# bhansconnect/burn-ppo

Measured on AMD Instinct MI355X. Metric: env-steps/sec (rollout+GAE+PPO update) at 1/2/4/8 MI355X; steps-to-475-return CartPole, higher is better.
Workload: dtype f32

## Files before the change

burn-ppo_amd/bppo/_lib.py:

```python
import ctypes as C
import os

import numpy as np

HERE = os.path.dirname(os.path.abspath(__file__))
LIB_PATH = os.environ.get("BPPO_LIB_PATH") or os.path.join(HERE, "libbppo.so")

OK, ERR_ARG, ERR_NONFINITE, ERR_EMPTY_MASK, ERR_HIP, ERR_COMM, ERR_UNSUPPORTED = range(7)
ENV_CARTPOLE, ENV_CONNECT_FOUR, ENV_LIARS_DICE = 0, 1, 2
ENV_SKULL = 3
ENV_KINDS = {"cartpole": ENV_CARTPOLE, "connect_four": ENV_CONNECT_FOUR, "liars_dice": ENV_LIARS_DICE,
             "skull": ENV_SKULL}
MAX_PLAYERS = 6


class BppoError(RuntimeError):
    def __init__(self, status, msg):
        super().__init__(f"bppo status {status}: {msg}")
        self.status = status


class Config(C.Structure):
    _fields_ = [("env_kind", C.c_int32), ("num_envs", C.c_int32), ("num_steps", C.c_int32),
                ("hidden_size", C.c_int32), ("num_hidden", C.c_int32), ("relu", C.c_int32),
                ("ctde", C.c_int32), ("critic_hidden_size", C.c_int32), ("critic_num_hidden", C.c_int32),
                ("num_epochs", C.c_int32), ("num_minibatches", C.c_int32),
                ("normalize_obs", C.c_int32), ("normalize_returns", C.c_int32), ("clip_value", C.c_int32),
                ("gamma", C.c_double), ("gae_lambda", C.c_double), ("clip_epsilon", C.c_double),
                ("value_coef", C.c_double), ("max_grad_norm", C.c_double), ("adam_epsilon", C.c_double),
                ("target_kl", C.c_double), ("return_clip", C.c_double),
                ("reward_shaping_coef", C.c_double), ("seed", C.c_uint64), ("env_seed_base", C.c_uint64),
                ("rng_stream", C.c_uint64),
                ("cnn", C.c_int32), ("num_conv_layers", C.c_int32), ("conv_channels", C.c_int32 * 4),
                ("kernel_size", C.c_int32), ("cnn_fc_hidden_size", C.c_int32), ("cnn_num_fc_layers", C.c_int32),
                ("normalize_values", C.c_int32), ("player_count", C.c_int32), ("split_networks", C.c_int32),
                ("shuffle_windows", C.c_int32)]


class Episode(C.Structure):
    _fields_ = [("total_reward", C.c_float * MAX_PLAYERS), ("length", C.c_int32), ("env_index", C.c_int32),
                ("step", C.c_int32), ("pad", C.c_int32)]


class RolloutInfo(C.Structure):
    _fields_ = [("episodes", C.c_int32), ("mean_return", C.c_float), ("mean_length", C.c_float),
                ("pad", C.c_int32), ("rng_word_pos", C.c_uint64)]


METRIC_NAMES = ("policy_loss", "value_loss", "entropy", "entropy_scaled", "approx_kl", "clip_fraction",
                "explained_variance", "total_loss", "value_mean", "returns_mean", "adv_mean_raw",
                "adv_std_raw", "adv_min_raw", "adv_max_raw", "value_error_mean", "value_error_std",
                "value_error_max", "avg_valid_actions", "entropy_valid_pct")


POPART_METRICS = ("value_norm_target_mean", "value_norm_target_std", "value_norm_rescale_mag")


class UpdateMetrics(C.Structure):
    _fields_ = [(n, C.c_float) for n in METRIC_NAMES] + [("num_updates", C.c_int32),
                                                          ("epochs_run", C.c_int32)] + \
        [(n, C.c_float) for n in POPART_METRICS]


ALLREDUCE_FN = C.CFUNCTYPE(C.c_int, C.c_void_p, C.c_size_t, C.c_void_p)

EXPORTS = (
    "bppo_create", "bppo_destroy", "bppo_last_error", "bppo_version", "bppo_num_params",
    "bppo_params_set", "bppo_params_get", "bppo_forward", "bppo_rng_get", "bppo_rng_set",
    "bppo_vecenv_reset", "bppo_vecenv_observe", "bppo_vecenv_step", "bppo_vecenv_set_step", "bppo_set_reward_shaping_schedule",
    "bppo_obs_norm_get", "bppo_obs_norm_set", "bppo_ret_norm_get", "bppo_ret_norm_set",
    "bppo_collect_rollouts", "bppo_rollout_episodes", "bppo_compute_gae", "bppo_ppo_update", "bppo_train_step", "bppo_train_steps",
    "bppo_set_allreduce", "bppo_set_allreduce_async", "bppo_get_stream", "bppo_opponents_set", "bppo_opponents_get_envs", "bppo_buffer_get", "bppo_buffer_set", "bppo_gae_device", "bppo_gae_rows_device",
    "bppo_gae_mp_device", "bppo_last_kernel_ms", "bppo_debug_libm", "bppo_debug_shuffle_chain", "bppo_debug_chain_walk2", "bppo_minibatch_rows",
    "bppo_debug_fisher_yates", "bppo_debug_gemm", "bppo_debug_shuffle_engine", "bppo_debug_sample",
    "bppo_rng_fill_bytes", "bppo_rng_from_seed", "bppo_rng_key_get", "bppo_num_param_tensors",
    "bppo_optimizer_get", "bppo_optimizer_set", "bppo_popart_get", "bppo_popart_set",
    "bppo_config_size", "bppo_update_metrics_size", "bppo_episode_size", "bppo_rollout_info_size",
    "bppo_set_explained_variance_mode", "bppo_set_minibatch_kernel", "bppo_set_rank",
    "bppo_debug_record_params",
)

STRUCT_SIZES = {"bppo_config_size": Config, "bppo_update_metrics_size": UpdateMetrics,
                "bppo_episode_size": Episode, "bppo_rollout_info_size": RolloutInfo}

_lib = None


def lib():
    global _lib
    if _lib is not None:
        return _lib
    try:
        import torch
    except ImportError:
        pass
    if not os.path.exists(LIB_PATH):
        raise RuntimeError(f"{LIB_PATH} is missing; build it with `make -C burn-ppo_amd` "
                           f"(or __graft_entry__.build())")
    L = C.CDLL(LIB_PATH)
    vp, u64, sz, i32 = C.c_void_p, C.c_uint64, C.c_size_t, C.c_int32
    fp = C.POINTER(C.c_float)
    dp = C.POINTER(C.c_double)
    sig = {
        "bppo_create": (i32, [C.POINTER(Config), C.c_int, vp, C.POINTER(vp)]),
        "bppo_destroy": (None, [vp]),
        "bppo_last_error": (C.c_char_p, [vp]),
        "bppo_version": (C.c_char_p, []),
        "bppo_num_params": (sz, [vp]),
        "bppo_params_set": (i32, [vp, vp, sz]),
        "bppo_params_get": (i32, [vp, vp, sz]),
        "bppo_forward": (i32, [vp, vp, vp, i32, vp, vp]),
        "bppo_rng_get": (i32, [vp, C.POINTER(u64)]),
        "bppo_rng_set": (i32, [vp, u64]),
        "bppo_vecenv_reset": (i32, [vp]),
        "bppo_vecenv_observe": (i32, [vp, vp, vp, vp, vp]),
        "bppo_vecenv_step": (i32, [vp, vp, vp, vp, vp, vp, i32, C.POINTER(i32)]),
        "bppo_vecenv_set_step": (i32, [vp, u64]),
        "bppo_set_reward_shaping_schedule": (i32, [vp, vp, vp, i32]),
        "bppo_obs_norm_get": (i32, [vp, vp, vp, dp]),
        "bppo_obs_norm_set": (i32, [vp, vp, vp, C.c_double]),
        "bppo_ret_norm_get": (i32, [vp, vp, vp]),
        "bppo_ret_norm_set": (i32, [vp, vp, vp]),
        "bppo_collect_rollouts": (i32, [vp, C.POINTER(RolloutInfo)]),
        "bppo_rollout_episodes": (i32, [vp, vp, i32, C.POINTER(i32)]),
        "bppo_compute_gae": (i32, [vp]),
        "bppo_ppo_update": (i32, [vp, C.c_double, C.c_double, C.POINTER(UpdateMetrics)]),
        "bppo_train_step": (i32, [vp, C.c_double, C.c_double, C.POINTER(RolloutInfo), C.POINTER(UpdateMetrics)]),
        "bppo_train_steps": (i32, [vp, i32, vp, vp, C.c_uint64, vp, vp, vp, i32, vp]),
        "bppo_set_allreduce": (i32, [vp, ALLREDUCE_FN, vp, i32]),
        "bppo_set_allreduce_async": (i32, [vp, ALLREDUCE_FN, vp, i32]),
        "bppo_set_rank": (i32, [vp, i32]),
        "bppo_get_stream": (i32, [vp, C.POINTER(vp)]),
        "bppo_opponents_set": (i32, [vp, i32, vp, vp, vp, vp, i32, vp, vp, vp]),
        "bppo_opponents_get_envs": (i32, [vp, vp, vp]),
        "bppo_buffer_get": (i32, [vp, C.c_char_p, vp, sz]),
        "bppo_buffer_set": (i32, [vp, C.c_char_p, vp, sz]),
        "bppo_gae_device": (i32, [vp, vp, vp, vp, i32, i32, C.c_float, C.c_float, vp, vp, vp]),
        "bppo_gae_rows_device": (i32, [vp, vp, vp, vp, i32, i32, C.c_float, C.c_float, vp, vp, vp, vp]),
        "bppo_gae_mp_device": (i32, [vp, vp, vp, vp, vp, i32, i32, i32, C.c_float, C.c_float, vp, vp,
                                     vp]),
        "bppo_last_kernel_ms": (i32, [vp, C.c_char_p, fp]),
        "bppo_debug_libm": (i32, [i32, i32, vp, vp, sz]),
        "bppo_debug_shuffle_chain": (i32, [u64, u64, u64, C.c_uint32, vp, C.POINTER(u64)]),
        "bppo_minibatch_rows": (i32, [vp, vp, i32, C.POINTER(i32)]),
        "bppo_debug_chain_walk2": (i32, [u64, u64, u64, u64, C.c_uint32, C.c_uint32, C.POINTER(u64), C.POINTER(u64)]),
        "bppo_debug_fisher_yates": (i32, [i32, vp, C.c_uint32, vp]),
        "bppo_debug_gemm": (i32, [i32, i32, i32, i32, vp, vp, vp, i32, vp, vp]),
        "bppo_debug_shuffle_engine": (i32, [u64, u64, u64, C.c_uint32, i32, u64, i32, i32, vp, vp, vp]),
        "bppo_debug_sample": (i32, [i32, i32, vp, vp, u64, u64, u64, vp, vp]),
        "bppo_rng_fill_bytes": (i32, [vp, vp, sz]),
        "bppo_rng_from_seed": (i32, [vp, vp]),
        "bppo_rng_key_get": (i32, [vp, vp]),
        "bppo_num_param_tensors": (sz, [vp]),
        "bppo_optimizer_get": (i32, [vp, vp, vp, vp, sz]),
        "bppo_optimizer_set": (i32, [vp, vp, vp, vp, sz]),
        "bppo_popart_get": (i32, [vp, vp]),
        "bppo_popart_set": (i32, [vp, vp]),
        "bppo_set_explained_variance_mode": (i32, [vp, i32]),
        "bppo_set_minibatch_kernel": (i32, [vp, i32]),
        "bppo_debug_record_params": (i32, [vp, vp, i32]),
    }
    for name in STRUCT_SIZES:
        sig[name] = (sz, [])
    for name, (res, args) in sig.items():
        f = getattr(L, name)
        f.restype = res
        f.argtypes = args
    for name, struct in STRUCT_SIZES.items():
        if getattr(L, name)() != C.sizeof(struct):
            raise RuntimeError(f"{LIB_PATH}: {name}() = {getattr(L, name)()} but ctypes {struct.__name__} is "
                               f"{C.sizeof(struct)} bytes (binding out of date with include/bppo.h)")
    _lib = L
    return L


def check(status, ctx=None):
    if status != OK:
        msg = lib().bppo_last_error(ctx).decode() if ctx else ""
        raise BppoError(status, msg)


def ptr(a):
    if a is None:
        return None
    if isinstance(a, np.ndarray):
        assert a.flags["C_CONTIGUOUS"]
        return a.ctypes.data
    return a.data_ptr()
```

burn-ppo_amd/csrc/bppo_api.hip:

```cpp
#include <algorithm>
#include <pthread.h>
#include <chrono>
#include <cmath>
#include <cstdio>
#include <cstdlib>
#include <cstring>
#include <new>
#include <thread>
#include <sys/prctl.h>
#include <x86intrin.h>
#include "bppo_internal.h"
#include "shuffle_host.h"
#include "bppo_wide.h"

using namespace bppo;

namespace bppo {
static double tsc_per_ms() {
    static double v = 0.0;
    if (v == 0.0) {
        const auto t0 = std::chrono::steady_clock::now();
        const uint64_t c0 = __rdtsc();
        std::this_thread::sleep_for(std::chrono::milliseconds(20));
        const uint64_t c1 = __rdtsc();
// ... 4 lines not shown


NetLayout make_layout(const bppo_config &c, int obs_dim, int priv_dim, int act_dim) {
    NetLayout L;
    const bool split = c.split_networks && !c.ctde;
    L.ctde = c.ctde || split; L.relu = c.relu;
    auto add = [&](int in, int out) {
        int i = L.n_layers++;
        L.in[i] = in; L.out[i] = out;
        return i;
    };
    int in = obs_dim;
    if (c.cnn) {
        L.H = 6; L.W = 7; L.C = 2;
        L.E = obs_dim - L.H * L.W * L.C;
        L.ksize = c.kernel_size;
        int cin = L.C;
        for (int l = 0; l < c.num_conv_layers; l++) {
            const int co = c.conv_channels[l < 4 ? l : 3];
            L.conv_cin[l] = cin;
            add(cin * L.ksize * L.ksize, co);
            cin = co;
        }
        L.n_conv = c.num_conv_layers;
        L.fdim = L.H * L.W * cin + L.E;
        in = L.fdim;
        for (int l = 0; l < c.cnn_num_fc_layers; l++) { add(in, c.cnn_fc_hidden_size); in = c.cnn_fc_hidden_size; }
        L.n_actor_hidden = L.n_conv + c.cnn_num_fc_layers;
    } else {
        for (int l = 0; l < c.num_hidden; l++) { add(in, c.hidden_size); in = c.hidden_size; }
        L.n_actor_hidden = c.num_hidden;
    }
    L.policy = add(in, act_dim);
    if (L.ctde && c.cnn) {
        L.critic_first = L.n_layers;
        for (int l = 0; l < L.n_conv; l++) add(L.in[l], L.out[l]);
        L.critic_fc0 = L.n_layers;
        int cin = L.fdim;
        for (int l = 0; l < c.cnn_num_fc_layers; l++) { add(cin, c.cnn_fc_hidden_size); cin = c.cnn_fc_hidden_size; }
        L.value = add(cin, 1);
    } else if (L.ctde) {
        int cin = split ? obs_dim : priv_dim + obs_dim;
        const int nc = split ? c.num_hidden : c.critic_num_hidden, wc = split ? c.hidden_size : c.critic_hidden_size;
        L.critic_first = L.critic_fc0 = L.n_layers;
        for (int l = 0; l < nc; l++) { add(cin, wc); cin = wc; }
        L.value = add(cin, 1);
    } else {
        L.value = add(in, 1);
    }
    int order[16], no = 0;
    for (int l = 0; l < L.n_layers; l++)
        if (!split || l < L.n_actor_hidden || (l >= L.critic_first && l < L.value)) order[no++] = l;
    if (split) { order[no++] = L.policy; order[no++] = L.value; }
    size_t off = 0;
    for (int r = 0; r < L.n_layers; r++) {
        const int l = order[r];
        L.rec[l] = r;
        L.w[l] = off; off += (size_t)L.in[l] * L.out[l];
        L.b[l] = off; off += L.out[l];
    }
    L.n_params = off;
    return L;
}

__global__ void k_libm(int which, const float *x, float *y, size_t n) {
    size_t i = blockIdx.x * (size_t)blockDim.x + threadIdx.x;
    if (i >= n) return;
    float v = x[i];
    switch (which) {
    case 0: y[i] = bppo_math::logf_glibc(v); break;
    case 1: y[i] = bppo_math::sinf_glibc(v); break;
    case 2: y[i] = bppo_math::cosf_glibc(v); break;
    case 3: y[i] = -bppo_math::logf_glibc(-bppo_math::logf_glibc(v)); break;
    case 5: y[i] = bppo_math::tanhf_glibc_bf(v); break;
    default: y[i] = bppo_math::expf_glibc(v); break;
    }
}

bppo_status launch_libm(int which, const float *d_x, float *d_y, size_t n) {
    hipLaunchKernelGGL(k_libm, dim3((unsigned)((n + 255) / 256)), dim3(256), 0, 0, which, d_x, d_y, n);
    return hipGetLastError() == hipSuccess ? BPPO_OK : BPPO_ERR_HIP;
}

}

static float powi_f32(float a, int b) {
    int recip = b < 0;
    float r = 1.0f;
    for (;;) {
        if (b & 1) r *= a;
        b /= 2;
        if (b == 0) break;
        a *= a;
    }
    return recip ? 1.0f / r : r;
}

template <class T>
static bppo_status dalloc(bppo_ctx *c, T **p, size_t n) {
    *p = nullptr;
    if (n == 0) return BPPO_OK;
    BPPO_HIP(c, hipMalloc((void **)p, n * sizeof(T)));
    BPPO_HIP(c, hipMemsetAsync(*p, 0, n * sizeof(T), c->stream));
    return BPPO_OK;
}

extern "C" size_t bppo_config_size(void) { return sizeof(bppo_config); }
extern "C" size_t bppo_update_metrics_size(void) { return sizeof(bppo_update_metrics); }
extern "C" size_t bppo_episode_size(void) { return sizeof(bppo_episode); }
extern "C" size_t bppo_rollout_info_size(void) { return sizeof(bppo_rollout_info); }

extern "C" const char *bppo_version(void) { return "bppo-mi355x 0.1 (gfx950)"; }

extern "C" const char *bppo_last_error(const bppo_ctx *c) { return c ? c->err.c_str() : "null ctx"; }

static hipError_t wait_event(bppo_ctx *c, hipEvent_t ev) {
    const auto t0 = std::chrono::steady_clock::now();
    hipError_t e = event_query(ev);
    if (e == hipErrorNotReady) {
        if (c->wait_est_us > 200.0)
            std::this_thread::sleep_for(std::chrono::microseconds((long)(0.7 * c->wait_est_us)));
        while ((e = event_query(ev)) == hipErrorNotReady) std::this_thread::sleep_for(std::chrono::microseconds(20));
    }
    const double ms = std::chrono::duration<double, std::milli>(std::chrono::steady_clock::now() - t0).count();
    c->wait_est_us = c->wait_est_us > 0.0 ? 0.5 * c->wait_est_us + 500.0 * ms : 1000.0 * ms;
    c->sync_wait_ms += ms;
    return e;
}

static hipError_t sync_stream(bppo_ctx *c) {
    const auto t0 = std::chrono::steady_clock::now();
    hipError_t e;
    if (!c->ev_block) e = hipStreamSynchronize(c->stream);
    else {
        static thread_local bool slack = false;
        if (!slack) { (void)prctl(PR_SET_TIMERSLACK, 1000UL, 0, 0, 0); slack = true; }
        e = hipEventRecord(c->ev_block, c->stream);
        while (e == hipSuccess && (e = event_query(c->ev_block)) == hipErrorNotReady) {
            std::this_thread::sleep_for(std::chrono::microseconds(20));
            e = hipSuccess;
        }
    }
    c->sync_wait_ms += std::chrono::duration<double, std::milli>(std::chrono::steady_clock::now() - t0).count();
    return e;
}

static bool cartpole_fused_net(const bppo_config &c) {
    return !c.split_networks && !c.cnn && !c.ctde && (c.hidden_size == 16 || c.hidden_size == 32 || c.hidden_size == 64) &&
           (c.num_hidden == 1 || c.num_hidden == 2);
}

static bppo_status ctx_init(bppo_ctx *c, const bppo_config *cfg, int dev, void *stream) {
    c->cfg = *cfg;
    c->dev = dev;
    if (cfg->num_envs <= 0 || cfg->num_steps <= 0 || cfg->num_epochs <= 0 || cfg->num_minibatches <= 0) {
        c->err = "num_envs, num_steps, num_epochs, num_minibatches must be positive";
        return BPPO_ERR_ARG;
    }
    c->N = cfg->num_envs; c->T = cfg->num_steps;
    switch (cfg->env_kind) {
    case BPPO_ENV_CARTPOLE: c->D = 5; c->A = 2; c->P = 1; c->G = 0; break;
    case BPPO_ENV_CONNECT_FOUR: c->D = 86; c->A = 7; c->P = 2; c->G = 0; break;
    case BPPO_ENV_LIARS_DICE: c->D = 270; c->A = 49; c->P = 4; c->G = cfg->ctde ? 120 : 0; break;
    case BPPO_ENV_SKULL: c->D = 135; c->A = 33; c->P = 6; c->G = cfg->ctde ? 200 : 0; break;
    default: c->err = "unknown env_kind"; return BPPO_ERR_ARG;
    }
    c->Pa = c->P;
    if (cfg->env_kind == BPPO_ENV_SKULL) {
        c->Pa = cfg->player_count ? cfg->player_count : 4;
        if (c->Pa < 2 || c->Pa > 6) { c->err = "Skull supports 2-6 players"; return BPPO_ERR_ARG; }
    }
    c->wide = cfg->env_kind != BPPO_ENV_CARTPOLE || !cartpole_fused_net(*cfg);
    if (c->wide && !cfg->ctde) c->G = 0;
    if (!cfg->cnn && (cfg->hidden_size < 1 || cfg->num_hidden < 1 ||
                      (cfg->ctde && (cfg->critic_hidden_size < 1 || cfg->critic_num_hidden < 1)))) {
        c->err = "hidden_size / num_hidden (critic_*) must be positive";
        return BPPO_ERR_ARG;
    }
    if (!(cfg->reward_shaping_coef >= 0.0)) { c->err = "reward_shaping_coef must be >= 0"; return BPPO_ERR_ARG; }
    if (cfg->cnn) {
        if (cfg->env_kind != BPPO_ENV_CONNECT_FOUR || cfg->ctde) { c->err = "CNN requires OBSERVATION_SHAPE (Connect Four)"; return BPPO_ERR_ARG; }
        if (cfg->num_conv_layers < 1 || cfg->num_conv_layers > 4 || cfg->kernel_size < 1 || cfg->kernel_size > 7 ||
            !(cfg->kernel_size & 1) || cfg->cnn_num_fc_layers < 1 || cfg->cnn_fc_hidden_size < 1) {
            c->err = "CNN: 1-4 conv layers, odd kernel_size <= 7 (same padding), >= 1 FC layer";
            return BPPO_ERR_UNSUPPORTED;
        }
        for (int l = 0; l < cfg->num_conv_layers; l++)
            if (cfg->conv_channels[l < 4 ? l : 3] < 1) { c->err = "conv_channels must be positive"; return BPPO_ERR_ARG; }
    }
    {
        const int split = cfg->split_networks && !cfg->ctde ? 2 : 1;
        const int layers = cfg->cnn ? split * (cfg->num_conv_layers + cfg->cnn_num_fc_layers) + 2
                         : cfg->ctde ? cfg->num_hidden + cfg->critic_num_hidden + 2
                                     : split * cfg->num_hidden + 2;
        if (layers > NetLayout::MAX_LAYERS) {
            c->err = "network: at most 16 layers in all (hidden / conv / FC layers + heads)";
            return BPPO_ERR_UNSUPPORTED;
        }
    }
    BPPO_HIP(c, hipSetDevice(dev));
    if (stream) { c->stream = (hipStream_t)stream; c->own_stream = false; }
    else {
        int lo = 0, hi = 0;
        BPPO_HIP(c, hipDeviceGetStreamPriorityRange(&lo, &hi));
        BPPO_HIP(c, hipStreamCreateWithPriority(&c->stream, hipStreamNonBlocking, hi));
        c->own_stream = true;
    }
    c->net = make_layout(*cfg, c->D, c->G, c->A);
    const size_t np = c->net.n_params;
    const size_t TN = (size_t)c->T * c->N;
    c->adam_t.assign(2 * c->net.n_layers, 0);
    TRY(dalloc(c, &c->d_params, np));
    TRY(dalloc(c, &c->d_m1, np));
    TRY(dalloc(c, &c->d_m2, np));
    TRY(dalloc(c, &c->d_grad, np + 64));
    c->slab_rows = 256 * 8;
    c->relu_mfma = cfg->relu ? 1 : 0;
    if (!c->wide) TRY(dalloc(c, &c->d_slab, c->slab_rows * (np + 64)));
    TRY(dalloc(c, &c->d_cp, (size_t)4 * c->N));
    TRY(dalloc(c, &c->d_steps, (size_t)c->N));
    TRY(dalloc(c, &c->d_env_pos, (size_t)c->N));
    TRY(dalloc(c, &c->d_ep_ret, (size_t)c->N * c->P));
    TRY(dalloc(c, &c->d_ep_len, (size_t)c->N));
    if (!c->wide) TRY(dalloc(c, &c->d_obs, TN * c->D));
    TRY(dalloc(c, &c->d_rew, TN));
    TRY(dalloc(c, &c->d_rew_raw, TN));
    TRY(dalloc(c, &c->d_done, TN));
    TRY(dalloc(c, &c->d_val, TN));
    TRY(dalloc(c, &c->d_logp, TN));
    TRY(dalloc(c, &c->d_adv, TN));
    TRY(dalloc(c, &c->d_ret, TN));
    TRY(dalloc(c, &c->d_act, TN));
    if (!c->wide || cfg->normalize_returns) TRY(dalloc(c, &c->d_X, TN));
    if (!c->wide && cfg->hidden_size == 64 && cfg->num_hidden == 2 && cfg->relu)
    {
        TRY(dalloc(c, &c->d_gumbel, TN * 2));
        TRY(dalloc(c, &c->d_rpool, (size_t)RPOOL_K * c->N));
        TRY(dalloc(c, &c->d_rpos, (size_t)RPOOL_K * c->N));
    }
    TRY(dalloc(c, &c->d_on, (size_t)2 * c->D + 1));
    if (!c->wide) TRY(dalloc(c, &c->d_obs_part, (size_t)c->N * 2 * c->D));
    if (!c->wide) {
        TRY(dalloc(c, &c->d_act_in, (size_t)c->N));
        TRY(dalloc(c, &c->d_scr_r, (size_t)c->N));
        TRY(dalloc(c, &c->d_bxc, (size_t)c->N * c->D));
        BPPO_HIP(c, hipMalloc((void **)&c->d_scr_d, (size_t)c->N));
    }
    TRY(dalloc(c, &c->d_rn_returns, (size_t)c->N * c->P));
    TRY(dalloc(c, &c->d_rn_stats, 4));
    TRY(dalloc(c, &c->d_scan_agg, (TN + 4095) / 4096 + 1));
    TRY(dalloc(c, &c->d_last_v, (size_t)c->N));
    c->eps_cap = (int)std::min<size_t>((size_t)c->T * c->N + 4096, (size_t)INT32_MAX / 2);
    TRY(dalloc(c, &c->d_eps, (size_t)c->eps_cap));
    TRY(dalloc(c, &c->d_ep_count, 1));
    TRY(dalloc(c, &c->d_ep_sum, ROLL_HOST_WORDS));
    TRY(dalloc(c, &c->d_err, 1));
    TRY(dalloc(c, &c->d_perm_base, TN));
    c->d_perm = c->d_perm_base;
    TRY(dalloc(c, &c->d_perm_ep, TN * (size_t)cfg->num_epochs));
    TRY(dalloc(c, &c->d_inv_ep, TN * (size_t)cfg->num_epochs));
    TRY(dalloc(c, &c->d_advpart, (size_t)ADV_STREAM_BLOCKS * ADV_STREAM_MAXM * 4));
    {
        c->fy_shared = getenv("BPPO_FY_ON_COPY") && atoi(getenv("BPPO_FY_ON_COPY")) == 1;
        if (!c->fy_shared) BPPO_HIP(c, make_side_stream(dev, &c->fy_stream));
        for (int e = 0; e < cfg->num_epochs && e < SHUF_MAX_EPOCHS; e++)
            BPPO_HIP(c, hipEventCreateWithFlags(&c->fy_ev[e], hipEventDisableTiming));
        if (getenv("BPPO_PREP_SIDE") && atoi(getenv("BPPO_PREP_SIDE")) == 1) {
            BPPO_HIP(c, make_side_stream(dev, &c->prep_stream));
            BPPO_HIP(c, hipEventCreateWithFlags(&c->ev_prep, hipEventDisableTiming));
        }
        BPPO_HIP(c, hipEventCreateWithFlags(&c->ev_env, hipEventDisableTiming));
    }
    TRY(dalloc(c, &c->d_fy, 4 * TN));
    TRY(dalloc(c, &c->d_scan, TN / 8192 + 2));
    BPPO_HIP(c, fy_ranges_init(c->fyr, (uint32_t)TN));
    TRY(dalloc(c, &c->d_red, 4 * 1024 + 64));
    TRY(dalloc(c, &c->d_mb_stats, (size_t)4 * std::max(cfg->num_minibatches, 2)));
    c->d_mb_cur = c->d_mb_stats;
    TRY(dalloc(c, &c->d_rows, (size_t)cfg->num_epochs * cfg->num_minibatches * (WM_COUNT + 4)));
    BPPO_HIP(c, hipHostMalloc((void **)&c->h_rows,
                              sizeof(float) * (size_t)cfg->num_epochs * cfg->num_minibatches * (WM_COUNT + 4),
                              hipHostMallocDefault));
    if (!c->wide && cfg->hidden_size == 64 && cfg->num_hidden == 2 && cfg->relu && c->D == 5)
    {
        BPPO_HIP(c, hipMalloc((void **)&c->d_rowA, sizeof(float4) * 2 * TN));
        BPPO_HIP(c, hipMalloc((void **)&c->d_rowB, sizeof(float2) * TN));
    }
    BPPO_HIP(c, hipHostMalloc((void **)&c->h_red, sizeof(double) * (4 * 1024 + 64 + 2 * ROLL_HOST_WORDS),
                              hipHostMallocDefault));
    BPPO_HIP(c, hipHostGetDevicePointer((void **)&c->hd_red, c->h_red, 0));
    BPPO_HIP(c, hipEventCreateWithFlags(&c->ev_upd, hipEventDisableTiming));
    BPPO_HIP(c, hipEventRecord(c->ev_upd, c->stream));
    BPPO_HIP(c, hipEventCreateWithFlags(&c->ev_block, hipEventDisableTiming | hipEventBlockingSync));
    for (int i = 0; i < TM_SLOTS; i++) {
        BPPO_HIP(c, hipEventCreate(&c->ev[i][0]));
        BPPO_HIP(c, hipEventCreate(&c->ev[i][1]));
    }
    for (int i = 0; i < bppo_ctx::MB_EV; i++) {
        BPPO_HIP(c, hipEventCreate(&c->mb_ev[i][0]));
        BPPO_HIP(c, hipEventCreate(&c->mb_ev[i][1]));
    }
    c->rng_key = seed_key(cfg->seed);
    c->rng_pos = 0;
    c->shuf.gate = c->ev_upd;
    TRY(c->shuf.init(dev, c->rng_key, cfg->rng_stream, (uint32_t)TN, cfg->num_epochs, TN * (uint64_t)c->A, c->err,
                     cfg->shuffle_windows != 0));
    if (c->fy_shared) c->fy_stream = c->shuf.copy;
    c->on_mean.assign(c->D, 0.0); c->on_m2.assign(c->D, 0.0); c->on_count = 0;
    c->u_ret = c->d_ret; c->u_val = c->d_val;
    c->shaping_v.assign(1, cfg->reward_shaping_coef); c->shaping_s.assign(1, 0);
    if (cfg->normalize_values) TRY(popart_alloc(c));
    if (c->wide) {
        TRY(wide_init(c));
        TRY(wide_reset(c));
        TRY(wide_pack(c));
    } else {
        TRY(launch_cartpole_reset(c));
    }
    BPPO_HIP(c, sync_stream(c));
    return BPPO_OK;
}

extern "C" bppo_status bppo_create(const bppo_config *cfg, int hip_device, void *hip_stream,
                                   bppo_ctx **out) {
    if (!cfg || !out) return BPPO_ERR_ARG;
    bppo_ctx *c = new bppo_ctx();
    bppo_status s = ctx_init(c, cfg, hip_device, hip_stream);
    *out = c;
    return s;
}

extern "C" void bppo_destroy(bppo_ctx *c) {
    if (!c) return;
    if (c->ev_thread.joinable()) c->ev_thread.join();
    if (c->ev_stream) { (void)hipStreamSynchronize(c->ev_stream); (void)hipStreamDestroy(c->ev_stream); }
    if (c->ev_gae) (void)hipEventDestroy(c->ev_gae);
    if (c->ev_copied) (void)hipEventDestroy(c->ev_copied);
    for (float *h : {c->h_ev_v, c->h_ev_r, c->h_ev_valid}) if (h) (void)hipHostFree(h);
    if (c->fy_stream) (void)hipStreamSynchronize(c->fy_stream);
    if (c->prep_stream) (void)hipStreamSynchronize(c->prep_stream);
    c->shuf.shutdown();
    if (c->stream) (void)hipStreamSynchronize(c->stream);
    wide_free(c);
    popart_free(c);
    void *ptrs[] = {c->d_params, c->d_m1, c->d_m2, c->d_grad, c->d_slab, c->d_cp, c->d_steps,
                    c->d_env_pos, c->d_ep_ret, c->d_ep_len, c->d_obs, c->d_rew, c->d_rew_raw,
                    c->d_done, c->d_val, c->d_logp, c->d_adv, c->d_ret, c->d_act, c->d_X, c->d_on,
                    c->d_obs_part, c->d_rn_returns, c->d_rn_stats, c->d_scan_agg, c->d_last_v,
                    c->d_eps, c->d_ep_count, c->d_ep_sum, c->d_err, c->d_perm_base, c->d_perm_ep, c->d_inv_ep, c->d_advpart, c->d_fy, c->d_scan,
                    c->d_red, c->d_mb_stats, c->d_gumbel, c->d_rpool, c->d_rpos, c->d_rows, c->d_rowA, c->d_rowB};
    for (void *p : ptrs) if (p) (void)hipFree(p);
    fy_ranges_free(c->fyr);
    if (c->h_red) (void)hipHostFree(c->h_red);
    if (c->h_rows) (void)hipHostFree(c->h_rows);
    if (c->ev_block) (void)hipEventDestroy(c->ev_block);
    if (c->ev_upd) (void)hipEventDestroy(c->ev_upd);
    for (int i = 0; i < TM_SLOTS; i++) {
        if (c->ev[i][0]) (void)hipEventDestroy(c->ev[i][0]);
        if (c->ev[i][1]) (void)hipEventDestroy(c->ev[i][1]);
    }
    for (auto &pr : c->mb_ev)
        for (hipEvent_t e : pr) if (e) (void)hipEventDestroy(e);
    if (c->fy_stream && !c->fy_shared) { (void)hipStreamSynchronize(c->fy_stream); (void)hipStreamDestroy(c->fy_stream); }
    for (hipEvent_t e : c->fy_ev) if (e) (void)hipEventDestroy(e);
    if (c->prep_stream) (void)hipStreamDestroy(c->prep_stream);
    for (hipEvent_t e : {c->ev_env, c->ev_prep}) if (e) (void)hipEventDestroy(e);
    if (c->own_stream && c->stream) (void)hipStreamDestroy(c->stream);
    delete c;
}

extern "C" size_t bppo_num_params(const bppo_ctx *c) { return c ? c->net.n_params : 0; }

static void drop_prefetch(bppo_ctx *c) {
    if (!c->prefetched) return;
    c->prefetched = false;
    c->collected = 0;
    c->gae_done = 0;
}

extern "C" bppo_status bppo_params_set(bppo_ctx *c, const float *h, size_t n) {
    if (!c || !h || n != c->net.n_params) { if (c) c->err = "params_set: size mismatch"; return BPPO_ERR_ARG; }
    drop_prefetch(c);
    BPPO_HIP(c, hipMemcpyAsync(c->d_params, h, n * 4, hipMemcpyHostToDevice, c->stream));
    if (c->wide) TRY(wide_pack(c));
    BPPO_HIP(c, sync_stream(c));
    return BPPO_OK;
}

extern "C" bppo_status bppo_params_get(bppo_ctx *c, float *h, size_t n) {
    if (!c || !h || n != c->net.n_params) { if (c) c->err = "params_get: size mismatch"; return BPPO_ERR_ARG; }
    BPPO_HIP(c, hipMemcpyAsync(h, c->d_params, n * 4, hipMemcpyDeviceToHost, c->stream));
    BPPO_HIP(c, sync_stream(c));
    return BPPO_OK;
}

extern "C" bppo_status bppo_forward(bppo_ctx *c, const float *obs, const float *priv, int32_t B,
                                    float *logits, float *values) {
    if (!c || !obs || B <= 0) return BPPO_ERR_ARG;
    if (c->wide) return wide_forward_host(c, obs, priv, B, logits, values);
    struct Scratch { float *p[3] = {nullptr, nullptr, nullptr}; ~Scratch() { for (float *q : p) (void)hipFree(q); } } t;
    BPPO_HIP(c, hipMalloc((void **)&t.p[0], sizeof(float) * (size_t)B * c->D));
    BPPO_HIP(c, hipMalloc((void **)&t.p[1], sizeof(float) * (size_t)B * c->A));
    BPPO_HIP(c, hipMalloc((void **)&t.p[2], sizeof(float) * (size_t)B));
    float *d_o = t.p[0], *d_l = t.p[1], *d_v = t.p[2];
    BPPO_HIP(c, hipMemcpyAsync(d_o, obs, sizeof(float) * (size_t)B * c->D, hipMemcpyHostToDevice, c->stream));
    bppo_status s = launch_forward_rows(c, d_o, B, d_l, d_v);
    if (s == BPPO_OK) {
        if (logits) BPPO_HIP(c, hipMemcpyAsync(logits, d_l, sizeof(float) * (size_t)B * c->A, hipMemcpyDeviceToHost, c->stream));
        if (values) BPPO_HIP(c, hipMemcpyAsync(values, d_v, sizeof(float) * (size_t)B, hipMemcpyDeviceToHost, c->stream));
    }
    const bppo_status ss = sync_stream(c) == hipSuccess ? BPPO_OK : BPPO_ERR_HIP;
    return s != BPPO_OK ? s : ss;
}

extern "C" bppo_status bppo_rng_get(bppo_ctx *c, uint64_t *p) {
    if (!c || !p) return BPPO_ERR_ARG;
    *p = c->rng_pos;
    return BPPO_OK;
}
extern "C" bppo_status bppo_rng_set(bppo_ctx *c, uint64_t p) {
    if (!c) return BPPO_ERR_ARG;
    drop_prefetch(c);
    c->shuf_slot = -1;
    c->fy_slot = -1; c->fy_done = 0;
    c->rng_pos = p;
    return BPPO_OK;
}

extern "C" bppo_status bppo_rng_fill_bytes(bppo_ctx *c, uint8_t *dst, size_t n) {
    if (!c || (!dst && n)) return BPPO_ERR_ARG;
    const size_t nw = (n + 3) / 4;
    uint32_t blk[16];
    uint64_t cached = ~0ull;
    for (size_t i = 0; i < nw; i++) {
        const uint64_t pos = c->rng_pos + i;
        if ((pos >> 4) != cached) { chacha12_block(c->rng_key, pos >> 4, c->cfg.rng_stream, blk); cached = pos >> 4; }
        const uint32_t w = blk[pos & 15];
        for (int b = 0; b < 4 && 4 * i + b < n; b++) dst[4 * i + b] = (uint8_t)(w >> (8 * b));
    }
    c->rng_pos += nw;
    c->shuf_slot = -1;
    c->fy_slot = -1; c->fy_done = 0;
    return BPPO_OK;
}

extern "C" bppo_status bppo_rng_from_seed(bppo_ctx *c, const uint8_t *seed) {
    if (!c || !seed) return BPPO_ERR_ARG;
    drop_prefetch(c);
    Key8 k;
    for (int i = 0; i < 8; i++)
        k.k[i] = (uint32_t)seed[4 * i] | ((uint32_t)seed[4 * i + 1] << 8) | ((uint32_t)seed[4 * i + 2] << 16) |
                 ((uint32_t)seed[4 * i + 3] << 24);
    BPPO_HIP(c, sync_stream(c));
    BPPO_HIP(c, hipStreamSynchronize(c->fy_stream));
    c->fy_slot = -1; c->fy_done = 0;
    c->shuf.shutdown();
    c->shuf.~ShuffleEngine();
    new (&c->shuf) ShuffleEngine();
    c->rng_key = k;
    c->rng_pos = 0;
    c->shuf_slot = -1;
    const size_t TN = (size_t)c->T * c->N;
    c->shuf.gate = c->ev_upd;
    TRY(c->shuf.init(c->dev, c->rng_key, c->cfg.rng_stream, (uint32_t)TN, c->cfg.num_epochs, TN * (uint64_t)c->A, c->err,
                     c->cfg.shuffle_windows != 0));
    if (c->fy_shared) c->fy_stream = c->shuf.copy;
    return BPPO_OK;
}

extern "C" bppo_status bppo_rng_key_get(bppo_ctx *c, uint32_t *key) {
    if (!c || !key) return BPPO_ERR_ARG;
    for (int i = 0; i < 8; i++) key[i] = c->rng_key.k[i];
    return BPPO_OK;
}

extern "C" bppo_status bppo_optimizer_get(bppo_ctx *c, float *m1, float *m2, int32_t *steps, size_t n) {
    if (!c || n != c->net.n_params) { if (c) c->err = "optimizer_get: size mismatch"; return BPPO_ERR_ARG; }
    if (m1) BPPO_HIP(c, hipMemcpyAsync(m1, c->d_m1, n * 4, hipMemcpyDeviceToHost, c->stream));
    if (m2) BPPO_HIP(c, hipMemcpyAsync(m2, c->d_m2, n * 4, hipMemcpyDeviceToHost, c->stream));
    BPPO_HIP(c, sync_stream(c));
    if (steps)
        for (int l = 0; l < c->net.n_layers; l++)
            for (int k = 0; k < 2; k++) steps[2 * c->net.rec[l] + k] = c->adam_t[2 * l + k];
    return BPPO_OK;
}

extern "C" bppo_status bppo_optimizer_set(bppo_ctx *c, const float *m1, const float *m2, const int32_t *steps,
                                          size_t n) {
    if (!c || !m1 || !m2 || !steps || n != c->net.n_params) {
        if (c) c->err = "optimizer_set: size mismatch";
        return BPPO_ERR_ARG;
    }
    BPPO_HIP(c, hipMemcpyAsync(c->d_m1, m1, n * 4, hipMemcpyHostToDevice, c->stream));
    BPPO_HIP(c, hipMemcpyAsync(c->d_m2, m2, n * 4, hipMemcpyHostToDevice, c->stream));
    BPPO_HIP(c, sync_stream(c));
    for (int l = 0; l < c->net.n_layers; l++)
        for (int k = 0; k < 2; k++) c->adam_t[2 * l + k] = steps[2 * c->net.rec[l] + k];
    return BPPO_OK;
}

extern "C" size_t bppo_num_param_tensors(const bppo_ctx *c) { return c ? c->adam_t.size() : 0; }

extern "C" bppo_status bppo_vecenv_reset(bppo_ctx *c) {
    if (!c) return BPPO_ERR_ARG;
    drop_prefetch(c);
    TRY(c->wide ? wide_reset(c) : launch_cartpole_reset(c));
    BPPO_HIP(c, sync_stream(c));
    return BPPO_OK;
}

extern "C" bppo_status bppo_vecenv_observe(bppo_ctx *c, float *obs, int32_t *players, uint8_t *masks,
                                           float *priv) {
    (void)priv; (void)masks;
    if (!c) return BPPO_ERR_ARG;
    if (c->wide) return wide_observe_host(c, obs, players, masks, priv);
    if (obs) {
        TRY(launch_cartpole_observe(c, c->d_bxc));
        BPPO_HIP(c, hipMemcpyAsync(obs, c->d_bxc, sizeof(float) * (size_t)c->N * c->D, hipMemcpyDeviceToHost, c->stream));
        BPPO_HIP(c, sync_stream(c));
    }
    if (players) std::fill(players, players + c->N, 0);
    return BPPO_OK;
}

extern "C" bppo_status bppo_vecenv_step(bppo_ctx *c, const int32_t *actions, float *obs, float *rewards,
                                        uint8_t *dones, bppo_episode *eps, int32_t cap, int32_t *n_eps) {
    if (!c || !actions) return BPPO_ERR_ARG;
    const int N = c->N;
    if (c->wide) {
        BPPO_HIP(c, hipMemsetAsync(c->d_ep_count, 0, 4, c->stream));
        int32_t cnt = 0;
        TRY(wide_step_host(c, actions, obs, rewards, dones, &cnt));
        if (n_eps) *n_eps = cnt;
        if (eps && cap > 0 && cnt > 0) {
            std::vector<EpisodeRec> recs(std::min(cnt, c->eps_cap));
            BPPO_HIP(c, hipMemcpy(recs.data(), c->d_eps, sizeof(EpisodeRec) * recs.size(), hipMemcpyDeviceToHost));
            std::sort(recs.begin(), recs.end(), [](const EpisodeRec &a, const EpisodeRec &b) {
                return a.env_index < b.env_index; });
            for (int i = 0; i < (int)recs.size() && i < cap; i++) {
                std::memcpy(eps[i].total_reward, recs[i].total_reward, sizeof(float) * BPPO_MAX_PLAYERS);
                eps[i].length = recs[i].length; eps[i].env_index = recs[i].env_index;
                eps[i].step = recs[i].step; eps[i].pad = 0;
            }
        }
        return BPPO_OK;
    }
    int32_t *d_a = c->d_act_in; float *d_r = c->d_scr_r, *d_o = c->d_bxc; uint8_t *d_d = c->d_scr_d;
    BPPO_HIP(c, hipMemcpyAsync(d_a, actions, sizeof(int32_t) * N, hipMemcpyHostToDevice, c->stream));
    BPPO_HIP(c, hipMemsetAsync(c->d_ep_count, 0, 4, c->stream));
    TRY(launch_cartpole_vecenv_step(c, d_a, d_r, d_d, d_o));
    if (rewards) BPPO_HIP(c, hipMemcpyAsync(rewards, d_r, sizeof(float) * N, hipMemcpyDeviceToHost, c->stream));
    if (dones) BPPO_HIP(c, hipMemcpyAsync(dones, d_d, N, hipMemcpyDeviceToHost, c->stream));
    if (obs) BPPO_HIP(c, hipMemcpyAsync(obs, d_o, sizeof(float) * (size_t)N * c->D, hipMemcpyDeviceToHost, c->stream));
    int32_t cnt = 0;
    BPPO_HIP(c, hipMemcpyAsync(&cnt, c->d_ep_count, 4, hipMemcpyDeviceToHost, c->stream));
    BPPO_HIP(c, sync_stream(c));
    if (n_eps) *n_eps = cnt;
    if (eps && cap > 0 && cnt > 0) {
        std::vector<EpisodeRec> recs(std::min(cnt, c->eps_cap));
        BPPO_HIP(c, hipMemcpy(recs.data(), c->d_eps, sizeof(EpisodeRec) * recs.size(), hipMemcpyDeviceToHost));
        std::sort(recs.begin(), recs.end(), [](const EpisodeRec &a, const EpisodeRec &b) {
            return a.env_index < b.env_index; });
        for (int i = 0; i < (int)recs.size() && i < cap; i++) {
            std::memcpy(eps[i].total_reward, recs[i].total_reward, sizeof(float) * BPPO_MAX_PLAYERS);
            eps[i].length = recs[i].length; eps[i].env_index = recs[i].env_index;
            eps[i].step = recs[i].step; eps[i].pad = 0;
        }
    }
    return BPPO_OK;
}

extern "C" bppo_status bppo_vecenv_set_step(bppo_ctx *c, uint64_t s) {
    if (!c) return BPPO_ERR_ARG;
    c->env_step = s;
    return BPPO_OK;
}

extern "C" bppo_status bppo_set_reward_shaping_schedule(bppo_ctx *c, const double *values, const uint64_t *steps,
                                                        int32_t n) {
    if (!c || n < 0 || (n > 0 && (!values || !steps))) return BPPO_ERR_ARG;
    std::vector<double> v(values, values + n);
    std::vector<uint64_t> s(steps, steps + n);
    if (bppo::schedule_get(v, s, 0) < 0.0) { c->err = "reward_shaping_coef must be >= 0"; return BPPO_ERR_ARG; }
    c->shaping_v = std::move(v); c->shaping_s = std::move(s);
    return BPPO_OK;
}

extern "C" bppo_status bppo_obs_norm_get(bppo_ctx *c, double *mean, double *m2, double *count) {
    if (!c) return BPPO_ERR_ARG;
    std::vector<double> h(2 * c->D + 1);
    BPPO_HIP(c, hipMemcpyAsync(h.data(), c->d_on, sizeof(double) * h.size(), hipMemcpyDeviceToHost, c->stream));
    BPPO_HIP(c, sync_stream(c));
    if (mean) std::memcpy(mean, h.data(), sizeof(double) * c->D);
    if (m2) std::memcpy(m2, h.data() + c->D, sizeof(double) * c->D);
    if (count) *count = h[2 * c->D];
    return BPPO_OK;
}

extern "C" bppo_status bppo_obs_norm_set(bppo_ctx *c, const double *mean, const double *m2, double count) {
    if (!c || !mean || !m2) return BPPO_ERR_ARG;
    drop_prefetch(c);
    std::vector<double> h(2 * c->D + 1);
    std::memcpy(h.data(), mean, sizeof(double) * c->D);
    std::memcpy(h.data() + c->D, m2, sizeof(double) * c->D);
    h[2 * c->D] = count;
    BPPO_HIP(c, hipMemcpyAsync(c->d_on, h.data(), sizeof(double) * h.size(), hipMemcpyHostToDevice, c->stream));
    BPPO_HIP(c, sync_stream(c));
    return BPPO_OK;
}

extern "C" bppo_status bppo_ret_norm_get(bppo_ctx *c, double *mvc, double *returns) {
    if (!c) return BPPO_ERR_ARG;
    if (mvc) BPPO_HIP(c, hipMemcpyAsync(mvc, c->d_rn_stats, sizeof(double) * 3, hipMemcpyDeviceToHost, c->stream));
    if (returns) BPPO_HIP(c, hipMemcpyAsync(returns, c->d_rn_returns, sizeof(double) * (size_t)c->N * c->P, hipMemcpyDeviceToHost, c->stream));
    BPPO_HIP(c, sync_stream(c));
    return BPPO_OK;
}

extern "C" bppo_status bppo_ret_norm_set(bppo_ctx *c, const double *mvc, const double *returns) {
    if (!c) return BPPO_ERR_ARG;
    drop_prefetch(c);
    if (mvc) BPPO_HIP(c, hipMemcpyAsync(c->d_rn_stats, mvc, sizeof(double) * 3, hipMemcpyHostToDevice, c->stream));
    if (returns) BPPO_HIP(c, hipMemcpyAsync(c->d_rn_returns, returns, sizeof(double) * (size_t)c->N * c->P, hipMemcpyHostToDevice, c->stream));
    BPPO_HIP(c, sync_stream(c));
    return BPPO_OK;
}

extern "C" bppo_status bppo_popart_get(bppo_ctx *c, double *st) {
    if (!c || !st) return BPPO_ERR_ARG;
    st[0] = c->pa_mean; st[1] = c->pa_m2; st[2] = c->pa_count; st[3] = c->pa_eps;
    return BPPO_OK;
}

extern "C" bppo_status bppo_popart_set(bppo_ctx *c, const double *st) {
    if (!c || !st) return BPPO_ERR_ARG;
    drop_prefetch(c);
    c->pa_mean = st[0]; c->pa_m2 = st[1]; c->pa_count = st[2]; c->pa_eps = st[3];
    return BPPO_OK;
}

static bppo_status tm_begin(bppo_ctx *c, int slot) {
    BPPO_HIP(c, hipEventRecord(c->ev[slot][0], c->stream));
    return BPPO_OK;
}
static bppo_status tm_end(bppo_ctx *c, int slot) {
    BPPO_HIP(c, hipEventRecord(c->ev[slot][1], c->stream));
    return BPPO_OK;
}
static void tm_read(bppo_ctx *c, int slot) {
    float ms = 0;
    if (event_ms(c->ev[slot][0], c->ev[slot][1], &ms)) c->last_ms[slot] = ms;
}

static bppo_status fy_enqueue_ready(bppo_ctx *c, int slot) {
    const size_t B = (size_t)c->T * c->N;
    if (slot != c->fy_slot) {
        c->fy_slot = slot; c->fy_done = 0;
        BPPO_HIP(c, hipStreamWaitEvent(c->fy_stream, c->ev_upd, 0));
    }
    if (c->shuf.failed(c->err)) return BPPO_ERR_HIP;
    while (c->fy_done < c->cfg.num_epochs && c->shuf.epoch_ready(slot, c->fy_done)) {
        const int e = c->fy_done;
        if (c->shuf.failed(c->err)) return BPPO_ERR_HIP;
        BPPO_HIP(c, hipStreamWaitEvent(c->fy_stream, c->shuf.ev[slot][e], 0));
        if (e > 0) BPPO_HIP(c, hipStreamWaitEvent(c->fy_stream, c->fy_ev[e - 1], 0));
        BPPO_HIP(c, hipEventRecord(c->ev[TM_SHUFFLE][0], c->fy_stream));
        BPPO_HIP(c, fisher_yates_device(c->shuf.d_J[slot] + (size_t)e * B, (uint32_t)B, c->d_fy, c->d_scan,
                                        c->d_perm_ep + (size_t)e * B, c->fy_stream, &c->fyr,
                                        c->d_inv_ep + (size_t)e * B));
        BPPO_HIP(c, hipEventRecord(c->ev[TM_SHUFFLE][1], c->fy_stream));
        BPPO_HIP(c, hipEventRecord(c->fy_ev[e], c->fy_stream));
        c->fy_done++;
    }
    return BPPO_OK;
}

static double *roll_host(bppo_ctx *c, int slot) { return c->h_red + 4 * 1024 + 64 + (size_t)slot * ROLL_HOST_WORDS; }

static bppo_status collect_enqueue(bppo_ctx *c, bool summary) {
    const size_t TN = (size_t)c->T * c->N;
    c->coll_slot ^= 1;
    const int tro = c->coll_slot ? TM_ROLLOUT_B : TM_ROLLOUT, trn = c->coll_slot ? TM_RETNORM_B : TM_RETNORM;
    if (c->wide) {
        BPPO_HIP(c, hipMemsetAsync(c->d_ep_count, 0, 4, c->stream));
        BPPO_HIP(c, hipMemsetAsync(c->d_err, 0, 4, c->stream));
    }
    const uint64_t base = c->rng_pos;
    TRY(tm_begin(c, tro));
    if (c->wide) TRY(wide_collect(c, base));
    else {
        TRY(launch_cartpole_rollout(c, base, nullptr, nullptr, c->cfg.normalize_obs));
        TRY(popart_denorm(c, c->d_val, TN));
    }
    TRY(tm_end(c, tro));
    if (!opp_active(c)) {
        c->shuf_slot = c->shuf.ensure(base + TN * (uint64_t)c->A);
        TRY(fy_enqueue_ready(c, c->shuf_slot));
    }
    if (opp_active(c)) {
        TRY(opp_rollout_end(c));
    } else {
        c->rng_pos = base + TN * (uint64_t)c->A;
        c->shuf_slot = c->shuf.ensure(c->rng_pos);
    }
    if (c->cfg.normalize_obs) TRY(launch_obs_norm_merge(c));
    TRY(tm_begin(c, trn));
    if (c->cfg.normalize_returns) TRY(launch_return_norm(c));
    else if (!c->wide) BPPO_HIP(c, hipMemcpyAsync(c->d_rew, c->d_rew_raw, TN * 4, hipMemcpyDeviceToDevice, c->stream));
    TRY(tm_end(c, trn));
    int32_t *hv = reinterpret_cast<int32_t *>(roll_host(c, c->coll_slot));
    if (summary) {
        if (zero_copy()) {
            TRY(launch_episode_summary(c, c->hd_red + (roll_host(c, c->coll_slot) - c->h_red)));
        } else {
            TRY(launch_episode_summary(c, c->d_ep_sum));
            BPPO_HIP(c, hipMemcpyAsync(hv, c->d_ep_sum, sizeof(double) * ROLL_HOST_WORDS, hipMemcpyDeviceToHost, c->stream));
        }
    } else {
        BPPO_HIP(c, hipMemcpyAsync(&hv[0], c->d_ep_count, 4, hipMemcpyDeviceToHost, c->stream));
        BPPO_HIP(c, hipMemcpyAsync(&hv[1], c->d_err, 4, hipMemcpyDeviceToHost, c->stream));
    }
    c->collected = 1; c->gae_done = 0;
    c->rollout_rng_pos[c->coll_slot] = c->rng_pos;
    return BPPO_OK;
}

static bppo_status collect_finish(bppo_ctx *c, bppo_rollout_info *info, int slot) {
    float ms = 0;
    const int tro = slot ? TM_ROLLOUT_B : TM_ROLLOUT, trn = slot ? TM_RETNORM_B : TM_RETNORM;
    if (event_ms(c->ev[tro][0], c->ev[tro][1], &ms)) c->last_ms[TM_ROLLOUT] = ms;
    if (event_ms(c->ev[trn][0], c->ev[trn][1], &ms)) c->last_ms[TM_RETNORM] = ms;
    const int32_t *hv = reinterpret_cast<const int32_t *>(roll_host(c, slot));
    const double *part = roll_host(c, slot) + 2;
    if (hv[1] & 2) { c->err = "Empty action mask: an env has no valid action"; return BPPO_ERR_EMPTY_MASK; }
    if (hv[1] & 1) { c->err = "NaN/Inf in log probs — model producing corrupt logits"; return BPPO_ERR_NONFINITE; }
    if (hv[1] & 4) { c->err = "opponent pool: pos_to_opp names a model index outside [0, n_models)"; return BPPO_ERR_ARG; }
    if (hv[1] & 8) { c->err = "Invalid action: outside the env's action mask"; return BPPO_ERR_ARG; }
    if (hv[1]) { c->err = "collect_rollouts: unknown device error flag"; return BPPO_ERR_HIP; }
    if (info) {
        info->episodes = hv[0];
        info->rng_word_pos = c->rollout_rng_pos[slot];
        info->mean_return = 0; info->mean_length = 0;
        const int n = std::min(hv[0], c->eps_cap);
        if (n > 0) {
            double sr = 0, sl = 0;
            for (int b = 0; b < EP_SUMMARY_BLOCKS; b++) { sr += part[2 * b]; sl += part[2 * b + 1]; }
            info->mean_return = (float)(sr / n); info->mean_length = (float)(sl / n);
        }
    }
    return BPPO_OK;
}

extern "C" bppo_status bppo_collect_rollouts(bppo_ctx *c, bppo_rollout_info *info) {
    if (!c) return BPPO_ERR_ARG;
    if (c->prefetched) c->prefetched = false;
    else TRY(collect_enqueue(c, info != nullptr));
    BPPO_HIP(c, sync_stream(c));
    return collect_finish(c, info, c->coll_slot);
}

extern "C" bppo_status bppo_rollout_episodes(bppo_ctx *c, bppo_episode *eps, int32_t cap, int32_t *n) {
    if (!c) return BPPO_ERR_ARG;
    int32_t cnt = 0;
    BPPO_HIP(c, hipMemcpyAsync(&cnt, c->d_ep_count, 4, hipMemcpyDeviceToHost, c->stream));
    BPPO_HIP(c, sync_stream(c));
    int m = std::min(cnt, c->eps_cap);
// ... 727 lines not shown
```

burn-ppo_amd/csrc/bppo_internal.h:

```cpp
#pragma once
#include <hip/hip_runtime.h>
#include <stdint.h>
#include <stddef.h>
#include <string>
#include <vector>
#include <thread>
#include <mutex>
#include <condition_variable>
#include <atomic>
#include <memory>
#include "../../include/bppo.h"
#include "bppo_device.h"

namespace bppo {

struct NetLayout {
    static constexpr int MAX_LAYERS = 16;
    int n_layers = 0;
    int in[MAX_LAYERS], out[MAX_LAYERS];
    size_t w[MAX_LAYERS], b[MAX_LAYERS];
    int n_actor_hidden = 0;
    int policy = 0, value = 0;
    int critic_first = -1;
    int critic_fc0 = -1;
    int ctde = 0, relu = 1;
    int rec[MAX_LAYERS];
    size_t n_params = 0;
    int n_conv = 0, ksize = 3, H = 0, W = 0, C = 0, E = 0, fdim = 0;
    int conv_cin[4] = {0, 0, 0, 0};
    int conv_base(int s) const { return s ? critic_first : 0; }
    bool is_conv(int l) const {
        return n_conv && (l < n_conv || (critic_fc0 > critic_first && l >= critic_first && l < critic_fc0));
    }
};
NetLayout make_layout(const bppo_config &c, int obs_dim, int priv_dim, int act_dim);

constexpr int EP_SUMMARY_BLOCKS = 128;
constexpr int WIDE_SPLIT_MIN_ROWS = 32768;
constexpr int RPOOL_K = 16;
constexpr int TM_SLOTS = 10;
constexpr int ROLL_HOST_WORDS = 2 + 2 * EP_SUMMARY_BLOCKS;
constexpr int ADV_STREAM_BLOCKS = 512, ADV_STREAM_MAXM = 16;
constexpr int GRAD_METRIC_SLOTS = 14, GRAD_VEMAX = 9, GRAD_VEMAX_LOCAL = GRAD_METRIC_SLOTS;

struct EpisodeRec {
    float total_reward[BPPO_MAX_PLAYERS];
    int32_t length, env_index, step, pad;
};

struct Welford { double n, mean, m2; };

constexpr int SHUF_MAX_EPOCHS = 32;
constexpr int SHUF_MAX_SPEC = 64;
constexpr uint64_t SHUF_CK = 1024;
constexpr uint64_t SHUF_CHUNK = (uint64_t)1 << 20;
__host__ __device__ constexpr uint64_t shuffle_window(uint64_t n) { return 2 * n + ((uint64_t)1 << 20); }

struct SpecWalk {
    uint64_t start = 0, end = 0, ck_base = 0;
    int wbuf = 0;
    std::vector<uint32_t> ck;
    std::atomic<int64_t> progress{-1};
    std::atomic<int> done{1};
    std::atomic<bool> stop{false};
    std::atomic<int> merged_to{-1};
    uint64_t merge_q = 0;
    uint64_t gen = 0;
    uint64_t job = 0;
    bool running = false;
};

struct WordBuf {
    uint32_t *d = nullptr, *h = nullptr;
    uint64_t cap = 0;
    struct Region { uint64_t base = 0, len = 0, off = 0; } reg[SHUF_MAX_EPOCHS];
    int nreg = 0;
    std::vector<hipEvent_t> ev;
    std::unique_ptr<std::atomic<int>[]> ok;
    uint32_t *hd = nullptr;
    bool gpu = false;
    uint64_t made_for = ~0ull;
};

struct FyRanges {
    uint32_t *x = nullptr;
    uint32_t *cb = nullptr;
    uint32_t *cursor = nullptr;
    uint2 *P = nullptr;
    uint32_t *flag = nullptr;
    int nb = 0, ncb = 0;
    uint32_t n = 0;
};

struct EpochSplit { uint32_t B, base, rem, M; };
__device__ __forceinline__ uint32_t mb_of(uint32_t i, const EpochSplit &s) {
    const uint32_t big = s.rem * (s.base + 1);
    return i < big ? i / (s.base + 1) : s.rem + (i - big) / s.base;
}
struct ShuffleEngine {
    int dev = 0;
    uint32_t n = 0;
    int epochs = 0;
    Key8 key{};
    uint64_t stream = 0;
    uint64_t gap = 0;
    uint64_t win = 0;
    bool keep_guess = true;
    bool pair = false;
    bool win_producers = false;
    bool win_gpu_words = false;
    hipStream_t d2h = nullptr;
    hipEvent_t words_made = nullptr;
    double Ew = 0.0, sigma = 0.0;
    int K = 0;
    int host_cpus = 16;
    WordBuf wb[2];
    SpecWalk spec[SHUF_MAX_SPEC];
    int nspec = 0, ncur = 0;
    int C = 1;
    int fr_depth = 0;
    int cont0 = 0;
    bool cont_valid[2] = {false, false};
    int cont_src0 = -1, cont_dst0 = -1, cont_wb = 0;
    uint64_t cont_seq = 0;
    std::vector<std::thread> workers;
    std::vector<std::thread> gens;
    std::vector<std::pair<uint64_t, size_t>> gen_order;
    WordBuf *gen_buf = nullptr;
    std::atomic<size_t> gen_next{0};
    uint64_t gen_job = 0;
    int gen_active = 0;
    void generator();
    uint64_t seq = 0;
    bool carry_valid[2] = {false, false};
    std::thread th;
    std::mutex mu;
    std::condition_variable cv;
    bool quit = false;
    bool slot_valid[2] = {false, false};
    uint64_t slot_start[2] = {0, 0};
    int pending = -1, running = -1;
    int consumer = -1;
    int chain_from = -1;
    uint64_t chain_start = 0;
    int last_slot = 1;
    hipEvent_t consumed[2] = {nullptr, nullptr};
    bool consumed_used[2] = {false, false};
    std::atomic<bool> cancel{false};
    int ready[2] = {0, 0};
    uint64_t end_pos[2][SHUF_MAX_EPOCHS];
    struct Seg { uint64_t pos0, pos1; uint32_t r0, pad; };
    int maxseg = 0;
    Seg *seg_host[2] = {nullptr, nullptr};
    Seg *d_seg[2] = {nullptr, nullptr};
    uint32_t *d_J[2] = {nullptr, nullptr};
    hipEvent_t ev[2][SHUF_MAX_EPOCHS] = {};
    bool ev_used[2][SHUF_MAX_EPOCHS] = {};
    hipStream_t copy = nullptr;
    hipEvent_t gate = nullptr;
    double walk_ms[2][SHUF_MAX_EPOCHS] = {};
    int coalesced[2][SHUF_MAX_EPOCHS] = {};
    std::atomic<uint64_t> spec_words{0}, true_words{0};
    std::atomic<uint64_t> tsc_walk{0}, tsc_words{0};
    bppo_status init(int device, const Key8 &key, uint64_t stream, uint32_t n_, int epochs_, uint64_t gap_,
                     std::string &err, bool windows = false);
    bool run_windowed(int slot, uint64_t start);
    void xj_gate_wait(int e);
    uint64_t job_end(int slot) const { return win ? slot_start[slot] + (uint64_t)epochs * win : end_pos[slot][epochs - 1]; }
    std::atomic<bool> hip_bad{false};
    std::mutex hip_mu;
    std::string hip_msg;
    void hip_note(hipError_t e, const char *what);
    bool failed(std::string &msg) const;
    int ensure(uint64_t start);
    hipError_t release(int slot, hipStream_t st);
    void wait_epoch(int slot, int e);
    bool epoch_ready(int slot, int e);
    void shutdown();
    void run();
    void worker(int i);
    void launch_walk(int i, uint64_t start, int wbuf);
    void stop_walks(int lo, int hi);
    const uint32_t *words(int b, uint64_t pos, uint64_t len, std::vector<uint32_t> &scratch, bool true_walk = false);
    int alt_b = -1;
    WordBuf::Region alt_reg;
    struct WalkStats { uint64_t words = 0, tsc_walk = 0, tsc_words = 0; };
    void walk_pair(int i, WalkStats &st);
    uint64_t walk_piece(int b, uint64_t pos, uint32_t *r, std::vector<uint32_t> &scratch, WalkStats &st,
                        bool true_walk = false);
    void flush(WalkStats &st, std::atomic<uint64_t> &words_ctr);
    int peek(int i, uint64_t q, uint32_t *r);
};
uint64_t shuffle_walk_host(const Key8 &key, uint64_t stream, uint64_t pos, uint32_t n, uint32_t *J);
hipError_t make_side_stream(int device, hipStream_t *st);

struct Timers {
    hipEvent_t a = nullptr, b = nullptr;
};

}

struct bppo_ctx {
    bppo_config cfg;
    int dev = 0;
    hipStream_t stream = nullptr;
    bool own_stream = false;
    std::string err;
    int N = 0, T = 0, D = 0, A = 0, P = 1, G = 0;
    int Pa = 1;
    bppo::NetLayout net;
    float *d_params = nullptr, *d_m1 = nullptr, *d_m2 = nullptr;
    std::vector<int32_t> adam_t;
    float *d_grad = nullptr;
    double *d_grad64 = nullptr;
    float *d_slab = nullptr;
    size_t slab_rows = 0;
    int slab_used = 0;
    int relu_mfma = 1;
    int mb_kernel = 0;
    float *dbg_params = nullptr;
    int dbg_params_max = 0;
    float *d_cp = nullptr;
    int32_t *d_steps = nullptr;
    uint64_t *d_env_pos = nullptr;
    float *d_ep_ret = nullptr;
    int32_t *d_ep_len = nullptr;
    uint64_t env_step = 0;
    std::vector<double> shaping_v;
    std::vector<uint64_t> shaping_s;
    float *d_obs = nullptr, *d_rew = nullptr, *d_rew_raw = nullptr, *d_done = nullptr;
    float *d_val = nullptr, *d_logp = nullptr, *d_adv = nullptr, *d_ret = nullptr;
    int32_t *d_act = nullptr;
    double *d_X = nullptr;
    float *d_gumbel = nullptr;
    float4 *d_rpool = nullptr;
    uint64_t *d_rpos = nullptr;
    double *d_on = nullptr;
    std::vector<double> on_mean, on_m2;
    double on_count = 0;
    double *d_obs_part = nullptr;
    double *d_rn_returns = nullptr;
    double *d_rn_stats = nullptr;
    bppo::Welford *d_scan_agg = nullptr;
    float *d_last_v = nullptr;
    bppo::EpisodeRec *d_eps = nullptr;
    int32_t *d_ep_count = nullptr;
    int32_t eps_cap = 0;
    double *d_ep_sum = nullptr;
    int32_t *d_err = nullptr;
    bppo::Key8 rng_key{};
    uint64_t rng_pos = 0;
    bppo::ShuffleEngine shuf;
    uint32_t *d_perm = nullptr;
    uint32_t *d_perm_base = nullptr;
    uint32_t *d_perm_ep = nullptr;
    uint32_t *d_inv_ep = nullptr;
    double *d_advpart = nullptr;
    hipStream_t fy_stream = nullptr;
    bool fy_shared = false;
    hipEvent_t fy_ev[bppo::SHUF_MAX_EPOCHS] = {};
    hipStream_t prep_stream = nullptr;
    hipEvent_t ev_env = nullptr, ev_prep = nullptr;
    int fy_slot = -1, fy_done = 0;
    uint32_t *d_fy = nullptr;
    uint32_t *d_scan = nullptr;
    bppo::FyRanges fyr;
    int shuf_slot = -1;
    double *d_red = nullptr;
    double *h_red = nullptr;
    double *hd_red = nullptr;
    float *h_rows = nullptr;
    float *d_mb_stats = nullptr;
    float *d_mb_cur = nullptr;
    float *d_rows = nullptr;
    std::vector<float> last_rows;
    float4 *d_rowA = nullptr;
    float2 *d_rowB = nullptr;
    bppo_allreduce_fn allreduce = nullptr;
    void *allreduce_user = nullptr;
    int world = 1;
    int rank = -1;
    float *d_pa_gather = nullptr;
    int allreduce_async = 0;
    int wide = 0;
    int L = 0;
    int rows_max = 0;
    void *d_wstate = nullptr;
    float *d_xc = nullptr;
    float *d_obs_raw = nullptr;
    int opp_K = 0, n_opp = 0;
    float *d_opp_params = nullptr;
    double *d_opp_on = nullptr;
    std::vector<int> opp_has_norm;
    int32_t *d_lpos = nullptr, *d_p2o = nullptr, *d_curopp = nullptr;
    int32_t *d_group = nullptr, *d_gpos = nullptr;
    float *d_valid = nullptr;
    uint64_t *d_rngpos = nullptr;
    float *d_oraw = nullptr, *d_oxc = nullptr, *d_ologits = nullptr;
    uint32_t *d_vidx = nullptr, *d_Jopp = nullptr;
    uint32_t *d_nvalid = nullptr;
    uint32_t n_valid = 0;
    int32_t *d_gbase = nullptr, *h_gbase = nullptr;
    double *d_obsw_part = nullptr;
    size_t obsw_part_n = 0;
    uint8_t *d_mask = nullptr;
    int32_t *d_players = nullptr;
    float *d_allr = nullptr;
    float *d_lvpp = nullptr;
    float *d_hbuf = nullptr;
    size_t hoff[16] = {};
    float *d_logits = nullptr, *d_values = nullptr;
    float *d_xcg = nullptr;
    float *d_dout = nullptr;
    float *d_dz[2] = {nullptr, nullptr};
    float *d_heads = nullptr, *d_heads_b = nullptr;
    float *d_part = nullptr, *d_colsum = nullptr;
    double *d_mpart = nullptr;
    float *d_cnn_y[2][4] = {};
    float *d_cnn_f[2] = {nullptr, nullptr};
    float *d_cnn_dy[2] = {nullptr, nullptr};
    float *d_cnn_wt = nullptr, *d_cnn_wd = nullptr, *d_cnn_owt = nullptr, *d_cnn_dwt = nullptr;
    size_t cnn_wt_off[2][4] = {};
    size_t cnn_wd_off[2][4] = {};
    int cnn_stacks = 1;
    double pa_mean = 0.0, pa_m2 = 0.0, pa_count = 0.0, pa_eps = 1e-4;
    float pa_rescale_mag = 0.0f;
    double pa_tsum = 0.0, pa_tsq = 0.0, pa_tcount = 0.0;
    float *d_ret_n = nullptr, *d_val_n = nullptr;
    double *d_pa_part = nullptr;
    const float *u_ret = nullptr, *u_val = nullptr;
    float *d_bxc = nullptr;
    uint8_t *d_bmask = nullptr;
    int32_t *d_bplayers = nullptr;
    int32_t *d_act_in = nullptr;
    float *d_scr_r = nullptr;
    uint8_t *d_scr_d = nullptr;
    hipEvent_t ev[bppo::TM_SLOTS][2] = {};
    hipEvent_t ev_block = nullptr;
    float last_ms[8] = {0};
    double last_walk_ms = 0.0, last_wait_ms = 0.0;
    double sync_wait_ms = 0.0, last_host_ms = 0.0, last_sync_ms = 0.0;
    double wait_est_us = 0.0;
    static constexpr int MB_EV = 64;
    hipEvent_t mb_ev[MB_EV][2] = {};
    int mb_ev_n = 0;
    int mb_launch = 0;
    float mb_k_mean = 0.0f, mb_k_min = 0.0f, mb_k_max = 0.0f;
    bool mb_ev_split[MB_EV] = {};
    float mb_k_split = 0.0f, mb_k_exact = 0.0f;
    double last_spec_mwords = 0.0, last_true_mwords = 0.0;
    double last_walk_cpu_ms = 0.0, last_words_cpu_ms = 0.0;
    int last_met = 0;
    int collected = 0, gae_done = 0;
    hipEvent_t ev_upd = nullptr;
    int coll_slot = 1;
    uint64_t rollout_rng_pos[2] = {0, 0};
    bool prefetch_next = false, prefetched = false;
    bool rows_from_rollout = false, rows_packed = false;
    uint64_t prefetch_env_step = 0;
    int ev_mode = 0;
    hipStream_t ev_stream = nullptr;
    hipEvent_t ev_gae = nullptr, ev_copied = nullptr;
    float *h_ev_v = nullptr, *h_ev_r = nullptr, *h_ev_valid = nullptr;
    std::thread ev_thread;
    float ev_ref = 0.0f;
};

namespace bppo {
enum { TM_ROLLOUT = 0, TM_GAE = 1, TM_UPDATE = 2, TM_FWDBWD = 3, TM_RETNORM = 4, TM_SHUFFLE = 5,
       TM_ADAM = 6, TM_BOOT = 7 };
enum { TM_ROLLOUT_B = 8, TM_RETNORM_B = 9 };

bppo_status launch_cartpole_reset(bppo_ctx *c);
bppo_status launch_cartpole_rollout(bppo_ctx *c, uint64_t base_pos, const double *mean,
                                    const double *sd, int norm_on);
bppo_status launch_cartpole_vecenv_step(bppo_ctx *c, const int32_t *d_actions, float *d_rew,
                                        uint8_t *d_done, float *d_obs_out);
bppo_status launch_cartpole_observe(bppo_ctx *c, float *d_obs_out);
bppo_status launch_obs_norm_merge(bppo_ctx *c);
bppo_status launch_episode_summary(bppo_ctx *c, double *host_slot);
inline bool zero_copy() {
    static const bool z = getenv("BPPO_ZERO_COPY") && atoi(getenv("BPPO_ZERO_COPY")) == 1;
    return z;
}
bppo_status launch_obs_norm_rows(bppo_ctx *c, int rows, float *x, int ld, float *raw);
bppo_status launch_obs_norm_rows_on(bppo_ctx *c, int rows, float *x, int ld, float *raw, const double *on);
bppo_status launch_bootstrap(bppo_ctx *c, const double *mean, const double *sd, int norm_on);
bppo_status launch_forward_rows(bppo_ctx *c, const float *d_obs, int B, float *d_logits,
                                float *d_values);
bppo_status launch_gae_1p(const float *r, const float *d, const float *v, const float *lv, int T,
                          int N, float gamma, float lambda, float *adv, float *ret, hipStream_t s,
                          float2 *pairs = nullptr, bool *pairs_done = nullptr, hipError_t *herr = nullptr);
bppo_status launch_gae_mp(const float *ar, const int32_t *pl, const float *d, const float *v,
                          const float *lvpp, int T, int N, int P, float gamma, float lambda,
                          float *adv, float *ret, hipStream_t s, hipError_t *herr = nullptr);
bppo_status launch_return_norm(bppo_ctx *c);
bppo_status launch_fisher_yates(bppo_ctx *c, const uint32_t *d_J, uint32_t n);
hipError_t fisher_yates_device(const uint32_t *d_J, uint32_t n, uint32_t *scratch, uint32_t *scan, uint32_t *perm,
                               hipStream_t st, const FyRanges *rg, uint32_t *inv = nullptr);
hipError_t fy_ranges_init(FyRanges &r, uint32_t n);
void fy_ranges_free(FyRanges &r);
bppo_status launch_epoch_adv_stats(bppo_ctx *c, uint32_t B, int M, const uint32_t *inv = nullptr);
bppo_status launch_minibatch(bppo_ctx *c, uint32_t start, uint32_t n, float ent_coef, bool exact);
bppo_status launch_adam(bppo_ctx *c, float lr, const float *c1, const float *c2, float *metric_dst = nullptr,
                        int nm = 0);
bppo_status launch_metric_row(bppo_ctx *c, float *dst, int nm);
bppo_status launch_pack_rows(bppo_ctx *c);
bppo_status launch_explained_variance(bppo_ctx *c, const float *valid);
void explained_variance_sums(bppo_ctx *c, double *out4);
bppo_status wide_init(bppo_ctx *c);
void wide_free(bppo_ctx *c);
bppo_status wide_reset(bppo_ctx *c);
bppo_status wide_pack(bppo_ctx *c);
bppo_status wide_forward(bppo_ctx *c, int rows, const float *xc, int ldxc, float *logits, float *values,
                         int split = 0);
bppo_status wide_forward_actor(bppo_ctx *c, int rows, const float *xc, int ldxc, const float *params, float *logits);
bppo_status cnn_alloc(bppo_ctx *c);
void cnn_free(bppo_ctx *c);
bppo_status cnn_pack(bppo_ctx *c, const float *params, float *wt, float *wd);
bppo_status cnn_features(bppo_ctx *c, int s, int rows, const float *x, int ldx, const float *params, const float *wt);
bppo_status cnn_backward(bppo_ctx *c, int s, int rows, const float *x, int ldx, float *dF, float *grad, int exact);
inline int wide_exact_grad(const bppo_ctx *c) {
    if (c->mb_kernel == 1) return 2;
    return c->mb_kernel == 0 ? 1 : 0;
}
bool opp_active(const bppo_ctx *c);
bppo_status opp_alloc(bppo_ctx *c);
void opp_free(bppo_ctx *c);
bppo_status opp_rollout_begin(bppo_ctx *c, uint64_t base);
bppo_status opp_step_group(bppo_ctx *c, int t);
bppo_status opp_step_forwards(bppo_ctx *c);
bppo_status opp_step_seats(bppo_ctx *c, int t);
bppo_status opp_rollout_end(bppo_ctx *c);
bppo_status opp_compact_valid(bppo_ctx *c);
bppo_status opp_map_perm(bppo_ctx *c, uint32_t n);
bppo_status wide_collect(bppo_ctx *c, uint64_t base);
bppo_status wide_bootstrap_gae(bppo_ctx *c);
bppo_status wide_minibatch(bppo_ctx *c, uint32_t start, uint32_t n, double ent_coef, bool first);
bppo_status wide_observe_host(bppo_ctx *c, float *obs, int32_t *players, uint8_t *masks, float *priv);
bppo_status wide_step_host(bppo_ctx *c, const int32_t *actions, float *obs, float *rewards, uint8_t *dones,
                           int32_t *n_eps);
bppo_status wide_forward_host(bppo_ctx *c, const float *obs, const float *priv, int B, float *logits,
                              float *values);
bppo_status wide_buffer_get(bppo_ctx *c, const char *name, void *host, size_t bytes, bool *handled);
double popart_std(const bppo_ctx *c);

inline double schedule_get(const std::vector<double> &v, const std::vector<uint64_t> &s, uint64_t step) {
    const size_t n = v.size();
    if (n == 0) return 0.0;
    if (n == 1 || step <= s[0]) return v[0];
    for (size_t i = 0; i + 1 < n; i++)
        if (step >= s[i] && step < s[i + 1]) {
            const double t = (double)(step - s[i]) / (double)(s[i + 1] - s[i]);
            return v[i] + (v[i + 1] - v[i]) * t;
        }
    return v[n - 1];
}
inline float shaping_coef(const bppo_ctx *c) { return (float)schedule_get(c->shaping_v, c->shaping_s, c->env_step); }
bppo_status popart_alloc(bppo_ctx *c);
void popart_free(bppo_ctx *c);
bppo_status popart_denorm(bppo_ctx *c, float *v, size_t n);
bppo_status popart_update_begin(bppo_ctx *c, const float *valid);
bppo_status popart_target_stats(bppo_ctx *c, int full_epochs, size_t rows_done, const float *valid);
bppo_status launch_libm(int which, const float *d_x, float *d_y, size_t n);

inline bppo_status hip_fail(bppo_ctx *c, hipError_t e, const char *what) {
    if (c) c->err = std::string(what) + ": " + hipGetErrorString(e);
    return BPPO_ERR_HIP;
}
inline bppo_status launch_check(bppo_ctx *c, const char *kernel) {
    const hipError_t e = hipGetLastError();
    return e == hipSuccess ? BPPO_OK : hip_fail(c, e, kernel);
}
inline hipError_t event_query(hipEvent_t ev) {
    const hipError_t e = hipEventQuery(ev);
    if (e != hipSuccess) (void)hipGetLastError();
    return e;
}
inline bool event_ms(hipEvent_t a, hipEvent_t b, float *ms) {
    const hipError_t e = hipEventElapsedTime(ms, a, b);
    if (e != hipSuccess) (void)hipGetLastError();
    return e == hipSuccess;
}
}

#define TRY(x)                                 \
    do {                                       \
        bppo_status _s = (x);                  \
        if (_s != BPPO_OK) return _s;          \
    } while (0)

#define BPPO_HIP(c, expr)                                                   \
    do {                                                                    \
        hipError_t _e = (expr);                                             \
// ... 3 lines not shown
```

burn-ppo_amd/csrc/shuffle_engine.hip:

```cpp
#include <algorithm>
#include <chrono>
#include <cmath>
#include <cstdlib>
#include <cstdio>
#include <cstring>
#include <pthread.h>
#include <x86intrin.h>
#include <sys/mman.h>
#include <sys/prctl.h>
#include <sys/resource.h>
#include <sys/syscall.h>
#include <unistd.h>
#include "bppo_internal.h"
#include "shuffle_host.h"

namespace bppo {

static bool shuf_debug() {
    static int v = -1;
    if (v < 0) v = getenv("BPPO_SHUFFLE_DEBUG") ? 1 : 0;
    return v == 1;
}
static double shuf_t_ms() {
    static const auto t0 = std::chrono::steady_clock::now();
    return std::chrono::duration<double, std::milli>(std::chrono::steady_clock::now() - t0).count();
}
#define SHUF_LOG(...)                                        \
    do {                                                     \
        if (shuf_debug()) { fprintf(stderr, "%9.3f ", shuf_t_ms()); fprintf(stderr, __VA_ARGS__); fflush(stderr); } \
    } while (0)

__global__ void k_chacha_words(Key8 key, uint64_t stream, uint64_t base, uint64_t len, uint32_t *out) {
    const uint64_t b = blockIdx.x * (uint64_t)blockDim.x + threadIdx.x;
    if (b * 16 >= len) return;
    uint32_t blk[16];
    chacha12_block(key, (base >> 4) + b, stream, blk);
    uint4 *o = reinterpret_cast<uint4 *>(out + b * 16);
    o[0] = make_uint4(blk[0], blk[1], blk[2], blk[3]);
    o[1] = make_uint4(blk[4], blk[5], blk[6], blk[7]);
    o[2] = make_uint4(blk[8], blk[9], blk[10], blk[11]);
    o[3] = make_uint4(blk[12], blk[13], blk[14], blk[15]);
}

struct WordRegions {
    const uint32_t *ptr[4];
    uint64_t base[4], len[4];
    int n;
};
constexpr int XJ_WAVES = 4;
constexpr int XJ_H = 16;

__device__ __forceinline__ uint32_t xj_word(const Key8 &key, uint64_t stream, const WordRegions &wr, uint64_t q) {
    for (int k = 0; k < wr.n; k++)
        if (q >= wr.base[k] && q < wr.base[k] + wr.len[k]) return wr.ptr[k][q - wr.base[k]];
    uint32_t blk[16];
    chacha12_block(key, q >> 4, stream, blk);
    uint32_t v = blk[0];
#pragma unroll
    for (int i = 1; i < 16; i++) v = (int)(q & 15) == i ? blk[i] : v;
    return v;
}

__global__ void __launch_bounds__(64 * XJ_WAVES) k_expand_J(Key8 key, uint64_t stream, const ShuffleEngine::Seg *segs,
                                                          int ns, WordRegions wr, uint32_t *J) {
    const int lane = threadIdx.x & 63;
    const int si = blockIdx.x * XJ_WAVES + (threadIdx.x >> 6);
    if (si == 0 && lane == 0) J[0] = 0;
    if (si >= ns) return;
    const ShuffleEngine::Seg g = segs[si];
    uint32_t r = g.r0;
    uint64_t q = g.pos0;
    uint32_t avail = q < g.pos1 ? (uint32_t)min((uint64_t)64, g.pos1 - q) : 0u;
    uint32_t w = lane < (int)avail ? xj_word(key, stream, wr, q + lane) : 0u;
    while (q < g.pos1 && r >= 2) {
        const uint64_t qn = q + 64;
        const uint32_t availn = qn < g.pos1 ? (uint32_t)min((uint64_t)64, g.pos1 - qn) : 0u;
        const uint32_t wn = lane < (int)availn ? xj_word(key, stream, wr, qn + lane) : 0u;
        const int lz = __clz(r);
        const uint32_t lowr = 1u << (31 - lz);
        if (r >= lowr + 64 && r >= 66) {
            const uint32_t s = 1u << lz;
            const uint32_t rj = r - (uint32_t)lane;
            uint32_t lo = w * rj, z = (rj << lz) - 1u;
            const uint64_t valid = avail >= 64 ? ~0ull : ((1ull << avail) - 1ull);
            uint64_t rejm = 0;
            uint32_t b = avail;
            uint32_t nrej = 0;
            uint64_t from = 0;
            bool open = true;
#pragma unroll
            for (int h = 0; h < XJ_H; h++) {
                const uint64_t acc = __ballot(lo <= z);
                lo += w;
                z += s;
                if (open) {
                    const uint64_t rem = ~acc & valid & ~from;
                    if (rem == 0) { open = false; continue; }
                    const int jh = __builtin_ctzll(rem);
                    rejm |= 1ull << jh;
                    nrej++;
                    from = jh == 63 ? ~0ull : ((2ull << jh) - 1ull);
                    if (h == XJ_H - 1) b = (uint32_t)jh + 1;
                }
            }
            const uint32_t below = (uint32_t)__builtin_amdgcn_mbcnt_hi((uint32_t)(rejm >> 32),
                                                                      __builtin_amdgcn_mbcnt_lo((uint32_t)rejm, 0u));
            if ((uint32_t)lane < b && !((rejm >> lane) & 1ull)) {
                const uint32_t rr = r - (uint32_t)lane + below;
                J[rr - 1] = __umulhi(w, rr);
            }
            r -= b - nrej;
            q += b;
        } else {
            uint32_t rr = r, used = 0;
            if (lane == 0) {
                int lz1 = __clz(rr);
                uint32_t lowr1 = 1u << (31 - lz1), sh = 1u << lz1, z = (rr << lz1) - 1u;
                for (uint32_t j = 0; j < avail && rr >= 2; j++) {
                    const uint32_t wj = xj_word(key, stream, wr, q + j);
                    const uint64_t m = (uint64_t)wj * rr;
                    used = j + 1;
                    if ((uint32_t)m <= z) {
                        J[rr - 1] = (uint32_t)(m >> 32);
                        rr--;
                        z -= sh;
                        if (rr < lowr1 && rr >= 1) { lz1 = __clz(rr); lowr1 = 1u << (31 - lz1); sh = 1u << lz1; z = (rr << lz1) - 1u; }
                    }
                }
            }
            r = __shfl(rr, 0, 64);
            q += __shfl(used, 0, 64);
        }
        if (q == qn) {
            w = wn;
            avail = availn;
        } else if (q < g.pos1) {
            avail = (uint32_t)min((uint64_t)64, g.pos1 - q);
            w = lane < (int)avail ? xj_word(key, stream, wr, q + lane) : 0u;
        }
    }
}

void ShuffleEngine::xj_gate_wait(int e) {
    static const int mode = getenv("BPPO_XJ_GATE") ? atoi(getenv("BPPO_XJ_GATE")) : 0;
    if (gate && (mode == 1 || (mode == 2 && e > 0))) hip_note(hipStreamWaitEvent(copy, gate, 0), "hipStreamWaitEvent");
}

static void shuffle_word_stats(uint32_t n, double &mean, double &sd) {
    double m = 0.0, v = 0.0;
    for (uint32_t R = n; R >= 2; R--) {
        const double a = (double)(R << __builtin_clz(R)) / 4294967296.0;
        m += 1.0 / a;
        v += (1.0 - a) / (a * a);
    }
    mean = m;
    sd = std::sqrt(v);
}

static uint32_t *host_words_alloc(uint64_t words) {
    const size_t bytes = (size_t)words * 4;
    const size_t huge = (size_t)2 << 20, sz = (bytes + huge - 1) / huge * huge;
    void *p = mmap(nullptr, sz, PROT_READ | PROT_WRITE, MAP_PRIVATE | MAP_ANONYMOUS, -1, 0);
    if (p == MAP_FAILED) return nullptr;
    (void)madvise(p, sz, MADV_HUGEPAGE);
    memset(p, 0, sz);
    return static_cast<uint32_t *>(p);
}
static void host_words_free(uint32_t *h, uint64_t words) {
    const size_t huge = (size_t)2 << 20, bytes = (size_t)words * 4;
    (void)munmap(h, (bytes + huge - 1) / huge * huge);
}

bppo_status ShuffleEngine::init(int device, const Key8 &k, uint64_t strm, uint32_t n_, int epochs_, uint64_t gap_,
                                std::string &err, bool windows) {
    dev = device; n = n_; epochs = epochs_; key = k; stream = strm; gap = gap_;
    if (epochs > SHUF_MAX_EPOCHS) { err = "num_epochs > 32 not supported by the shuffle engine"; return BPPO_ERR_UNSUPPORTED; }
    shuffle_word_stats(n, Ew, sigma);
    win = windows ? shuffle_window(n) : 0;
    host_cpus = 16;
    if (const char *e = getenv("BPPO_HOST_THREADS")) host_cpus = std::max(1, atoi(e));
    K = std::max(1, std::min(6, (6 * host_cpus + 8) / 16));
    if (const char *e = getenv("BPPO_SHUFFLE_SPEC")) K = std::max(0, atoi(e));
    C = std::min(2, std::max(epochs, 1));
    fr_depth = getenv("BPPO_SHUFFLE_FRONTIER") ? atoi(getenv("BPPO_SHUFFLE_FRONTIER")) : (host_cpus >= 8 ? 2 : 1);
    if (fr_depth > 0 && epochs >= 3 && K > 0) {
        C = std::min(fr_depth + 1, epochs - 1);
        fr_depth = C - 1;
        if (!getenv("BPPO_SHUFFLE_SPEC")) K = std::max(1, std::min(fr_depth >= 2 ? 4 : 5, (5 * host_cpus + 8) / 16));
    } else {
        fr_depth = 0;
    }
    if (win) { K = 1; C = 0; fr_depth = 0; }
    keep_guess = !(getenv("BPPO_SHUFFLE_KEEP_GUESS") && atoi(getenv("BPPO_SHUFFLE_KEEP_GUESS")) == 0);
    pair = win && host_cpus < epochs;
    if (const char *e = getenv("BPPO_SHUFFLE_PAIR")) pair = win && atoi(e) != 0;
    win_producers = win && getenv("BPPO_SHUFFLE_WIN_PRODUCERS") && atoi(getenv("BPPO_SHUFFLE_WIN_PRODUCERS")) == 1;
    win_gpu_words = win && !win_producers && getenv("BPPO_SHUFFLE_GPU_WORDS") &&
                    atoi(getenv("BPPO_SHUFFLE_GPU_WORDS")) == 1;
    const bool cont_on = !win && epochs - 1 >= C;
    K = std::min(K, SHUF_MAX_SPEC / (std::max(epochs - C, 0) + 2 * C + (cont_on ? 2 : 0)));
    ncur = K * std::max(epochs - C, 0);
    nspec = ncur + 2 * C * K;
    if (cont_on && K > 0) {
        cont0 = nspec;
        nspec += 2 * K;
    }
    const size_t bytes = sizeof(uint32_t) * (size_t)n * epochs;
    maxseg = (int)((Ew + 48.0 * sigma) / SHUF_CK) + 16;
    const size_t sbytes = sizeof(Seg) * (size_t)maxseg * epochs;
    for (int s = 0; s < 2; s++) {
        if (hipHostMalloc((void **)&seg_host[s], sbytes, hipHostMallocDefault) != hipSuccess ||
            hipMalloc((void **)&d_seg[s], sbytes) != hipSuccess ||
            hipMalloc((void **)&d_J[s], bytes) != hipSuccess) {
            err = "shuffle buffers: allocation failed";
            return BPPO_ERR_HIP;
        }
        for (int e = 0; e < epochs; e++)
            if (hipEventCreateWithFlags(&ev[s][e], hipEventDisableTiming | hipEventBlockingSync) != hipSuccess) {
                err = "shuffle events: creation failed";
                return BPPO_ERR_HIP;
            }
    }
    for (int s = 0; s < 2; s++)
        if (hipEventCreateWithFlags(&consumed[s], hipEventDisableTiming | hipEventBlockingSync) != hipSuccess) {
            err = "shuffle events: creation failed";
            return BPPO_ERR_HIP;
        }
    if (win && getenv("BPPO_SHUFFLE_GPU_WORDS") && atoi(getenv("BPPO_SHUFFLE_GPU_WORDS")) == 1 &&
        (hipStreamCreateWithFlags(&d2h, hipStreamNonBlocking) != hipSuccess ||
         hipEventCreateWithFlags(&words_made, hipEventDisableTiming) != hipSuccess)) {
        err = "shuffle word copies: stream creation failed";
        return BPPO_ERR_HIP;
    }
    if (make_side_stream(dev, &copy) != hipSuccess) {
        err = "shuffle copy stream: creation failed";
        return BPPO_ERR_HIP;
    }
    auto chunks = [](double w) { return ((uint64_t)std::max(w, 1.0) + SHUF_CHUNK - 1) / SHUF_CHUNK * SHUF_CHUNK; };
    const double sE = sigma * std::sqrt((double)std::max(epochs, 1));
    const uint64_t cap0 = chunks(epochs * Ew + 12.0 * sE + 4.0 * SHUF_CK) + SHUF_CHUNK;
    const double sC = sigma * std::sqrt((double)(epochs + C));
    const uint64_t cap1 = K && !win ? chunks(C * Ew + 8.0 * sC + 12.0 * sigma + 8.0 * SHUF_CK) + SHUF_CHUNK : 0;
    const uint64_t capw = (uint64_t)epochs * chunks(Ew + 10.0 * sigma + 4.0 * SHUF_CK);
    for (int b = 0; b < 2; b++) {
        WordBuf &w = wb[b];
        w.cap = win ? capw : cap0 + cap1;
        if (hipMalloc((void **)&w.d, w.cap * 4) != hipSuccess ||
            !(w.h = host_words_alloc(w.cap))) {
            err = "shuffle word buffers: allocation failed";
            return BPPO_ERR_HIP;
        }
        if (win_gpu_words) {
            const size_t huge = (size_t)2 << 20, sz = ((size_t)w.cap * 4 + huge - 1) / huge * huge;
            if (hipHostRegister(w.h, sz, hipHostRegisterDefault) != hipSuccess) {
                (void)hipGetLastError();
                w.gpu = false;
            } else {
                w.hd = w.h;
                w.gpu = true;
            }
        }
        const size_t nch = w.cap / SHUF_CHUNK;
        w.ev.assign(nch, nullptr);
        w.ok.reset(new std::atomic<int>[nch]);
        for (size_t c = 0; c < nch; c++) {
            w.ok[c] = 0;
            if (hipEventCreateWithFlags(&w.ev[c], w.gpu ? hipEventDisableTiming
                                                         : hipEventDisableTiming | hipEventBlockingSync) != hipSuccess) {
                err = "shuffle chunk events: creation failed";
                return BPPO_ERR_HIP;
            }
        }
    }
    const uint64_t nck = (uint64_t)((Ew + 24.0 * sigma) / SHUF_CK) + 4;
    for (int i = 0; i < nspec; i++) spec[i].ck.assign(nck, 0xFFFFFFFFu);
    for (int i = 0; i < nspec; i++) workers.emplace_back([this, i]() { worker(i); });
    const int ngen = win && !win_producers ? 0 : std::max(1, std::min(4, host_cpus / 4));
    for (int i = 0; i < ngen; i++) gens.emplace_back([this]() { generator(); });
    th = std::thread([this]() { run(); });
    return BPPO_OK;
}

int ShuffleEngine::ensure(uint64_t start) {
    std::unique_lock<std::mutex> lk(mu);
    for (int sl = 0; sl < 2; sl++)
        if (slot_valid[sl] && slot_start[sl] == start) {
            consumer = sl;
            lk.unlock();
            cv.notify_all();
            return sl;
        }
    if (running >= 0 || pending >= 0) {
        cancel = true;
        pending = -1;
        cv.notify_all();
        cv.wait(lk, [&] { return running < 0; });
        cancel = false;
    }
    chain_from = -1;
    slot_valid[0] = slot_valid[1] = false;
    const int sl = last_slot ^ 1;
    last_slot = sl;
    slot_start[sl] = start;
    slot_valid[sl] = true;
    ready[sl] = 0;
    pending = sl;
    consumer = sl;
    lk.unlock();
    cv.notify_all();
    return sl;
}

void ShuffleEngine::wait_epoch(int slot, int e) {
    std::unique_lock<std::mutex> lk(mu);
    const bool had = ready[slot] > e;
    cv.wait(lk, [&] { return ready[slot] > e || !slot_valid[slot]; });
    SHUF_LOG("[shuf] consumer epoch %d %s\n", e, had ? "ready" : "waited");
}

bool ShuffleEngine::epoch_ready(int slot, int e) {
    std::lock_guard<std::mutex> lk(mu);
    return slot_valid[slot] && ready[slot] > e;
}

hipError_t ShuffleEngine::release(int slot, hipStream_t st) {
    const hipError_t e = hipEventRecord(consumed[slot], st);
    if (e != hipSuccess) return e;
    std::lock_guard<std::mutex> lk(mu);
    consumed_used[slot] = true;
    return hipSuccess;
}

void ShuffleEngine::hip_note(hipError_t e, const char *what) {
    if (e == hipSuccess) return;
    (void)hipGetLastError();
    std::lock_guard<std::mutex> lk(hip_mu);
    if (hip_bad.load(std::memory_order_relaxed)) return;
    hip_msg = std::string("shuffle engine: ") + what + ": " + hipGetErrorString(e);
    hip_bad.store(true, std::memory_order_release);
}

bool ShuffleEngine::failed(std::string &msg) const {
    if (!hip_bad.load(std::memory_order_acquire)) return false;
    msg = hip_msg;
    return true;
}


const uint32_t *ShuffleEngine::words(int b, uint64_t pos, uint64_t len, std::vector<uint32_t> &scratch, bool true_walk) {
    if (true_walk && alt_b >= 0 && pos >= alt_reg.base && pos + len <= alt_reg.base + alt_reg.len) {
        WordBuf &a = wb[alt_b];
        const uint64_t o = alt_reg.off + (pos - alt_reg.base);
        if (a.ok[(size_t)(o / SHUF_CHUNK)].load(std::memory_order_acquire)) return a.h + o;
    }
    WordBuf &w = wb[b];
    for (int g = 0; g < w.nreg; g++) {
        const WordBuf::Region &R = w.reg[g];
        if (pos >= R.base && pos + len <= R.base + R.len) {
            const uint64_t o = R.off + (pos - R.base);
            const size_t c = (size_t)(o / SHUF_CHUNK);
            if (w.ok[c].load(std::memory_order_acquire)) return w.h + o;
            if (w.gpu && event_query(w.ev[c]) == hipSuccess) {
                w.ok[c].store(1, std::memory_order_release);
                return w.h + o;
            }
            break;
        }
    }
    scratch.resize(len);
    bppo_host::chacha12_words(key.k, stream, pos, scratch.data(), len);
    return scratch.data();
}

uint64_t ShuffleEngine::walk_piece(int b, uint64_t pos, uint32_t *r, std::vector<uint32_t> &scratch, WalkStats &st,
                                   bool true_walk) {
    const uint64_t q = (pos / SHUF_CK + 1) * SHUF_CK;
    const uint64_t t0 = __rdtsc();
    const uint32_t *w = words(b, pos, q - pos, scratch, true_walk);
    const uint64_t t1 = __rdtsc();
    const uint64_t used = bppo_host::chain_walk_nj(w, (size_t)(q - pos), r);
    st.tsc_words += t1 - t0;
    st.tsc_walk += __rdtsc() - t1;
    st.words += used;
    return pos + used;
}
void ShuffleEngine::flush(WalkStats &st, std::atomic<uint64_t> &words_ctr) {
    words_ctr.fetch_add(st.words, std::memory_order_relaxed);
    tsc_walk.fetch_add(st.tsc_walk, std::memory_order_relaxed);
    tsc_words.fetch_add(st.tsc_words, std::memory_order_relaxed);
    st = WalkStats{};
}

void ShuffleEngine::launch_walk(int i, uint64_t start, int wbuf) {
    SpecWalk &s = spec[i];
    s.start = start;
    s.ck_base = start / SHUF_CK * SHUF_CK;
    s.wbuf = wbuf;
    s.end = 0;
    std::fill(s.ck.begin(), s.ck.end(), 0xFFFFFFFFu);
    s.progress.store(-1, std::memory_order_relaxed);
    s.stop.store(false, std::memory_order_relaxed);
    s.merged_to.store(-1, std::memory_order_relaxed);
    s.merge_q = 0;
    s.done.store(0, std::memory_order_release);
    s.running = true;
    s.job = seq;
    s.gen++;
}

void ShuffleEngine::stop_walks(int lo, int hi) {
    std::unique_lock<std::mutex> lk(mu);
    for (int i = lo; i < hi; i++) spec[i].stop.store(true, std::memory_order_relaxed);
    cv.notify_all();
    cv.wait(lk, [&] {
        if (quit) return true;
        for (int i = lo; i < hi; i++) if (spec[i].running) return false;
        return true;
    });
}

int ShuffleEngine::peek(int i, uint64_t q, uint32_t *r) {
    for (;;) {
        SpecWalk &t = spec[i];
        if (q <= t.start) return -1;
        const int mt = t.merged_to.load(std::memory_order_acquire);
        if (mt >= 0 && q >= t.merge_q) { i = mt; continue; }
        const int64_t c = (int64_t)((q - t.ck_base) / SHUF_CK);
        if (c >= (int64_t)t.ck.size()) return -1;
        if (t.progress.load(std::memory_order_acquire) >= c) { *r = t.ck[c]; return 1; }
        if (t.done.load(std::memory_order_acquire) && t.merged_to.load(std::memory_order_acquire) < 0) return -1;
        return 0;
    }
}

void ShuffleEngine::worker(int i) {
    (void)pthread_setname_np(pthread_self(), "bppo-spec");
    (void)hipSetDevice(dev);
    {
        const int g = i < ncur ? i / std::max(K, 1) : std::max(epochs - C, 0);
        const int nv = (fr_depth > 0 || win) ? 1 : 3 * g;
        if (nv > 0) (void)setpriority(PRIO_PROCESS, (id_t)syscall(SYS_gettid), std::min(19, nv));
    }
    std::vector<uint32_t> scratch;
    WalkStats wst;
    uint64_t seen = 0;
    SpecWalk &s = spec[i];
    for (;;) {
        {
            std::unique_lock<std::mutex> lk(mu);
            cv.wait(lk, [&] { return quit || s.gen != seen; });
            if (quit) { s.running = false; cv.notify_all(); return; }
            seen = s.gen;
        }
        if (pair && i < nspec - (nspec & 1)) {
            if (i & 1) continue;
            walk_pair(i, wst);
            continue;
        }
        uint64_t pos = s.start;
        uint32_t r = n;
        while (r >= 2 && !s.stop.load(std::memory_order_relaxed)) {
            const uint64_t q = (pos / SHUF_CK + 1) * SHUF_CK;
            pos = walk_piece(s.wbuf, pos, &r, scratch, wst);
            if (pos == q) {
                const int64_t c = (int64_t)((q - s.ck_base) / SHUF_CK);
                if (c < (int64_t)s.ck.size()) {
                    s.ck[c] = r;
                    s.progress.store(c, std::memory_order_release);
                }
                uint32_t rl;
                if (i % K != 0 && peek(i - 1, q, &rl) == 1 && rl == r) {
                    s.merge_q = q;
                    s.merged_to.store(i - 1, std::memory_order_release);
                    break;
                }
            }
        }
        s.end = pos;
        flush(wst, spec_words);
        {
            std::lock_guard<std::mutex> lk(mu);
            s.done.store(1, std::memory_order_release);
            s.running = false;
            if (cont_dst0 >= 0 && s.job == cont_seq && i >= cont_src0 && i < cont_src0 + K && r < 2 &&
                !s.stop.load(std::memory_order_relaxed) && s.merged_to.load(std::memory_order_relaxed) < 0 &&
                !quit && !cancel.load(std::memory_order_relaxed))
                launch_walk(cont_dst0 + (i - cont_src0), pos + gap, cont_wb);
        }
        cv.notify_all();
    }
}

void ShuffleEngine::walk_pair(int i, WalkStats &st) {
    struct Chain {
        SpecWalk *s;
        uint64_t pos;
        uint32_t r;
        const uint32_t *w;
        size_t left;
        std::vector<uint32_t> scratch;
        bool live;
    } ch[2];
    {
        std::unique_lock<std::mutex> lk(mu);
        cv.wait(lk, [&] { return quit || spec[i + 1].running; });
        if (quit) return;
    }
    auto refill = [&](Chain &c) {
        const uint64_t q = (c.pos / SHUF_CK + 1) * SHUF_CK;
        const uint64_t t0 = __rdtsc();
        c.w = words(c.s->wbuf, c.pos, q - c.pos, c.scratch);
        st.tsc_words += __rdtsc() - t0;
        c.left = (size_t)(q - c.pos);
    };
    auto finish = [&](Chain &c) {
        c.live = false;
        c.s->end = c.pos;
        std::lock_guard<std::mutex> lk(mu);
        c.s->done.store(1, std::memory_order_release);
        c.s->running = false;
    };
    auto advance = [&](Chain &c, size_t used) {
        c.w += used;
        c.left -= used;
        c.pos += used;
        st.words += used;
        if (c.r < 2) { finish(c); cv.notify_all(); return; }
        if (c.left == 0) {
            const int64_t k = (int64_t)((c.pos - c.s->ck_base) / SHUF_CK);
            if (k < (int64_t)c.s->ck.size()) {
                c.s->ck[k] = c.r;
                c.s->progress.store(k, std::memory_order_release);
            }
            if (c.s->stop.load(std::memory_order_relaxed)) { finish(c); cv.notify_all(); return; }
            refill(c);
        }
    };
    for (int k = 0; k < 2; k++) {
        Chain &c = ch[k];
        c.s = &spec[i + k];
        c.pos = c.s->start;
        c.r = n;
        c.live = n >= 2;
        if (c.live) refill(c);
        else finish(c);
    }
    while (ch[0].live && ch[1].live) {
        size_t u0 = 0, u1 = 0;
        const uint64_t t0 = __rdtsc();
        bppo_host::chain_walk2_nj(ch[0].w, ch[0].left, &ch[0].r, &u0, ch[1].w, ch[1].left, &ch[1].r, &u1);
        st.tsc_walk += __rdtsc() - t0;
        advance(ch[0], u0);
        advance(ch[1], u1);
    }
    for (int k = 0; k < 2; k++) {
        Chain &c = ch[k];
        while (c.live) {
            const uint64_t t0 = __rdtsc();
            const size_t u = bppo_host::chain_walk_nj(c.w, c.left, &c.r);
            st.tsc_walk += __rdtsc() - t0;
            advance(c, u);
        }
    }
    flush(st, spec_words);
    cv.notify_all();
}

void ShuffleEngine::generator() {
    (void)pthread_setname_np(pthread_self(), "bppo-words");
    uint64_t seen = 0;
    for (;;) {
        WordBuf *W;
        {
            std::unique_lock<std::mutex> lk(mu);
            cv.wait(lk, [&] { return quit || gen_job != seen; });
            if (quit) return;
            seen = gen_job;
            W = gen_buf;
            gen_active++;
        }
        for (;;) {
            const size_t k = gen_next.fetch_add(1, std::memory_order_relaxed);
            if (k >= gen_order.size()) break;
            const auto pc = gen_order[k];
            bppo_host::chacha12_words(key.k, stream, pc.first, W->h + pc.second * SHUF_CHUNK, SHUF_CHUNK);
            W->ok[pc.second].store(1, std::memory_order_release);
        }
        {
            std::lock_guard<std::mutex> lk(mu);
            gen_active--;
        }
        cv.notify_all();
    }
}

void ShuffleEngine::run() {
    (void)pthread_setname_np(pthread_self(), "bppo-true");
    (void)prctl(PR_SET_TIMERSLACK, 1000UL, 0, 0, 0);
    (void)hipSetDevice(dev);
    std::vector<uint32_t> scratch;
    for (;;) {
        uint64_t start;
        int slot;
        bool wait_consumed = false;
        {
            std::unique_lock<std::mutex> lk(mu);
            cv.wait(lk, [&] { return quit || pending >= 0 || (chain_from >= 0 && consumer == chain_from); });
            if (quit) return;
            if (pending < 0) {
                slot = chain_from ^ 1;
                chain_from = -1;
                last_slot = slot;
                slot_start[slot] = chain_start;
                slot_valid[slot] = true;
                ready[slot] = 0;
            } else {
                slot = pending;
                pending = -1;
            }
            running = slot;
            start = slot_start[slot];
            wait_consumed = consumed_used[slot];
        }
        if (wait_consumed) hip_note(hipStreamWaitEvent(copy, consumed[slot], 0), "hipStreamWaitEvent");
        seq++;
        if (win) {
            const bool ok = run_windowed(slot, start);
            if (!ok) stop_walks(0, nspec);
            {
                std::lock_guard<std::mutex> lk(mu);
                running = -1;
                if (!ok) {
                    slot_valid[slot] = false;
                } else {
                    chain_from = slot;
                    chain_start = job_end(slot) + gap;
                }
            }
            cv.notify_all();
            continue;
        }
        const int b = (int)(seq & 1);
        const int cs = 1 - b;
        const int cur0 = 0, cur1 = ncur;
        const int cn0 = ncur + b * C * K, cn1 = cn0 + C * K;
        const int cp0 = ncur + cs * C * K;
        SHUF_LOG("[shuf] job %llu start=%llu slot=%d carry=%d\n", (unsigned long long)seq, (unsigned long long)start,
                 slot, (int)carry_valid[cs]);
        stop_walks(cn0, cn1);
        const int ccn0 = cont0 ? cont0 + b * K : 0, ccp0 = cont0 ? cont0 + cs * K : 0;
        if (cont0) {
            stop_walks(ccn0, ccn0 + K);
            std::lock_guard<std::mutex> lk(mu);
            for (int i = ccn0; i < ccn0 + K; i++) {
                spec[i].start = ~0ull;
                spec[i].merged_to.store(-1, std::memory_order_relaxed);
            }
            cont_src0 = cur0 + (epochs - 1 - C) * K;
            cont_dst0 = ccn0;
            cont_wb = b;
            cont_seq = seq;
            cont_valid[b] = K > 0;
        }
        WordBuf &W = wb[b];
        const double sE = sigma * std::sqrt((double)std::max(epochs, 1));
        {
            auto chunks = [](double w) { return ((uint64_t)std::max(w, 1.0) + SHUF_CHUNK - 1) / SHUF_CHUNK * SHUF_CHUNK; };
            const uint64_t s0 = start / SHUF_CK * SHUF_CK;
            const uint64_t end0 = s0 + chunks((double)(start - s0) + epochs * Ew + 10.0 * sE + 4.0 * SHUF_CK);
            const WordBuf &Pv = wb[b ^ 1];
            alt_b = -1;
            uint64_t base0 = s0;
            static const bool reuse = !(getenv("BPPO_SHUFFLE_CARRY_REUSE") && atoi(getenv("BPPO_SHUFFLE_CARRY_REUSE")) == 0);
            if (reuse && seq > 1 && Pv.nreg == 2 && Pv.reg[1].len > 0 && Pv.reg[1].base <= s0 &&
                Pv.reg[1].base + Pv.reg[1].len > s0 && Pv.reg[1].base + Pv.reg[1].len < end0) {
                alt_b = b ^ 1;
                alt_reg = Pv.reg[1];
                base0 = alt_reg.base + alt_reg.len;
            }
            W.nreg = 1;
            W.reg[0].base = base0;
            W.reg[0].off = 0;
            W.reg[0].len = std::min(W.cap, chunks((double)(end0 - base0)));
            if (K > 0) {
                const double sC = sigma * std::sqrt((double)(epochs + C));
                const double lo = (double)start + epochs * Ew + (double)gap - 4.0 * sC - 4.0 * SHUF_CK;
                uint64_t b1 = (uint64_t)std::max(lo, 0.0) / SHUF_CK * SHUF_CK;
                b1 = std::max(b1, W.reg[0].base + W.reg[0].len);
                const uint64_t len1 = std::min(W.cap - W.reg[0].len, chunks(C * Ew + 8.0 * sC + 12.0 * sigma + 8.0 * SHUF_CK));
                if (len1 > 0) {
                    W.reg[1].base = b1; W.reg[1].off = W.reg[0].len; W.reg[1].len = len1;
                    W.nreg = 2;
                }
            }
        }
        std::vector<std::pair<double, size_t>> order;
        for (int g = 0; g < W.nreg; g++) {
            const WordBuf::Region &R = W.reg[g];
            hipLaunchKernelGGL(k_chacha_words, dim3((unsigned)((R.len / 16 + 255) / 256)), dim3(256), 0, copy, key,
                               stream, R.base, R.len, W.d + R.off);
            hip_note(hipGetLastError(), "k_chacha_words launch");
            for (uint64_t o = 0; o < R.len; o += SHUF_CHUNK) {
                const size_t c = (size_t)((R.off + o) / SHUF_CHUNK);
                W.ok[c] = 0;
                const double p = (double)(R.base + o);
                const double org = g == 0 ? (double)start : (double)start + epochs * Ew + (double)gap;
                const double key_t = std::fmod(std::max(0.0, p - org + 4.0 * sE), std::max(Ew, 1.0));
                order.push_back({key_t, c});
            }
        }
        std::sort(order.begin(), order.end());
        {
            std::unique_lock<std::mutex> lk(mu);
            cv.wait(lk, [&] { return gen_active == 0 || quit; });
            gen_order.clear();
            for (auto &oc : order) {
                const size_t c = oc.second;
                const WordBuf::Region *R = nullptr;
                for (int g = 0; g < W.nreg; g++)
                    if (c * SHUF_CHUNK >= W.reg[g].off && c * SHUF_CHUNK < W.reg[g].off + W.reg[g].len) R = &W.reg[g];
                if (R) gen_order.push_back({R->base + (c * SHUF_CHUNK - R->off), c});
            }
            gen_buf = &W;
            gen_next.store(0, std::memory_order_relaxed);
            gen_job++;
        }
        cv.notify_all();
        const double spread = 2.0;
        auto guess = [&](double centre, double sd, int k) {
            return (uint64_t)std::max((double)start, std::floor(centre + ((k + 0.5) / K - 0.5) * 2.0 * spread * sd));
        };
        if (fr_depth > 0) {
            std::lock_guard<std::mutex> lk(mu);
            for (int i = cur0; i < cur1; i++) { spec[i].start = ~0ull; spec[i].merged_to.store(-1, std::memory_order_relaxed); }
            for (int i = cn0; i < cn1; i++) { spec[i].start = ~0ull; spec[i].merged_to.store(-1, std::memory_order_relaxed); }
            carry_valid[b] = K > 0;
        } else {
            std::lock_guard<std::mutex> lk(mu);
            for (int e = C; e < epochs; e++)
                for (int k = 0; k < K; k++)
                    launch_walk(cur0 + (e - C) * K + k, guess((double)start + e * Ew, sigma * std::sqrt((double)e), k), b);
            for (int c = 0; c < C; c++)
                for (int k = 0; k < K; k++)
                    launch_walk(cn0 + c * K + k, guess((double)start + (epochs + c) * Ew + (double)gap,
                                                       sigma * std::sqrt((double)(epochs + c)), k), b);
            carry_valid[b] = K > 0;
        }
        cv.notify_all();
        uint64_t pos = start;
        bool cancelled = false;
        WalkStats tst;
        std::vector<std::pair<uint64_t, uint32_t>> tck;
        for (int e = 0; e < epochs && !cancelled; e++) {
            auto t0 = std::chrono::steady_clock::now();
            if (ev_used[slot][e]) hip_note(hipEventSynchronize(ev[slot][e]), "hipEventSynchronize");
            uint32_t r = n;
            int met = -1, walked = 0;
            int s0 = 0, s1 = 0;
            if (e < C) { if (carry_valid[cs]) { s0 = cp0 + e * K; s1 = s0 + K; } }
            else { s0 = cur0 + (e - C) * K; s1 = s0 + K; }
            int c0 = 0, c1 = 0;
            if (e == 0 && cont0 && cont_valid[cs]) { c0 = ccp0; c1 = ccp0 + K; }
            tck.clear();
            tck.push_back({pos, r});
            int fin = -1;
            uint64_t endp = 0, chain_front = 0;
            auto frontier = [&](int i) -> uint64_t {
                for (int mt; (mt = spec[i].merged_to.load(std::memory_order_acquire)) >= 0;) i = mt;
                const int64_t pr = spec[i].progress.load(std::memory_order_acquire);
                return pr < 0 ? 0 : spec[i].ck_base + (uint64_t)pr * SHUF_CK;
            };
            auto try_switch = [&](uint64_t q, uint32_t rq) -> bool {
                int best = met;
                uint64_t bf = met >= 0 ? frontier(met) : 0;
                for (int g = 0; g < 2; g++)
                    for (int i = g ? s0 : c0; i < (g ? s1 : c1); i++) {
                        uint32_t rs = 0;
                        if (i == met || peek(i, q, &rs) != 1 || rs != rq) continue;
                        const uint64_t f = frontier(i);
                        if (best < 0 || f > bf) { best = i; bf = f; }
                    }
                if (best == met) return false;
                met = best;
                const bool on_cont = met >= c0 && met < c1;
                bool keep[SHUF_MAX_SPEC] = {};
                for (int i = met; i >= 0; i = spec[i].merged_to.load(std::memory_order_acquire)) keep[i] = true;
                for (int g = 0; g < 2; g++)
                    for (int i = g ? s0 : c0; i < (g ? s1 : c1); i++)
                        if (!keep[i] && !(on_cont && g == 1 && keep_guess))
                            spec[i].stop.store(true, std::memory_order_relaxed);
                return true;
            };
            while (r >= 2) {
                if (met >= 0) {
                    if (cancel.load(std::memory_order_relaxed) || quit) { cancelled = true; break; }
                    int f = met;
                    for (int mt; (mt = spec[f].merged_to.load(std::memory_order_acquire)) >= 0;) f = mt;
                    const bool chain_done = spec[f].done.load(std::memory_order_acquire) != 0 &&
                                            spec[f].merged_to.load(std::memory_order_acquire) < 0;
                    uint32_t rr = 0;
                    const bool recheck = keep_guess && s1 > s0 && met >= c0 && met < c1;
                    for (uint64_t q = (pos / SHUF_CK + 1) * SHUF_CK; r >= 2 && peek(met, q, &rr) == 1; q += SHUF_CK) {
                        tck.push_back({q, rr});
                        pos = q;
                        r = rr;
                        if (recheck && try_switch(q, rr)) break;
                    }
                    if (r < 2) break;
                    if (chain_done && spec[f].end > pos && spec[f].end - pos <= SHUF_CK) {
                        fin = f;
                        endp = spec[f].end;
                        break;
                    }
                    if (fr_depth > 0 && !chain_done && pos > chain_front) {
                        chain_front = pos;
                        std::this_thread::sleep_for(std::chrono::microseconds(10));
                        continue;
                    }
                }
                const uint64_t q = (pos / SHUF_CK + 1) * SHUF_CK;
                pos = walk_piece(b, pos, &r, scratch, tst, true);
                if (cancel.load(std::memory_order_relaxed)) { cancelled = true; break; }
                if (pos != q || r < 2) continue;
                tck.push_back({q, r});
                if (s0 == s1 && c0 == c1) continue;
                if (met < 0) walked++;
                try_switch(q, r);
            }
            flush(tst, true_words);
            if (cancelled) break;
            Seg *S = seg_host[slot] + (size_t)e * maxseg;
            int ns = 0;
            bool overflow = false;
            auto add = [&](uint64_t p0, uint64_t p1, uint32_t r0) {
                if (p1 <= p0 || r0 < 2) return;
                if (ns >= maxseg) { overflow = true; return; }
                S[ns++] = Seg{p0, p1, r0, 0};
            };
            for (size_t i = 0; i + 1 < tck.size(); i++) add(tck[i].first, tck[i + 1].first, tck[i].second);
            if (fin >= 0) pos = endp;
            add(tck.back().first, pos, tck.back().second);
            coalesced[slot][e] = met >= 0 ? walked : -1;
            auto prune = [&](int g0, int g1, uint64_t x) {
                int lo = -1, hi = -1, exact = -1;
                for (int i = g0; i < g1; i++) {
                    const uint64_t st = spec[i].start;
                    if (st == ~0ull) continue;
                    if (st == x) exact = i;
                    if (st <= x && (lo < 0 || st > spec[lo].start)) lo = i;
                    if (st > x && (hi < 0 || st < spec[hi].start)) hi = i;
                }
                bool keep[SHUF_MAX_SPEC] = {};
                for (int k0 : {exact >= 0 ? exact : lo, exact >= 0 ? -1 : hi})
                    for (int i = k0; i >= 0; i = spec[i].merged_to.load(std::memory_order_acquire)) keep[i] = true;
                for (int i = g0; i < g1; i++)
                    if (!keep[i]) spec[i].stop.store(true, std::memory_order_relaxed);
                return exact;
            };
            if (K > 0 && !cancelled) {
                std::lock_guard<std::mutex> lk(mu);
                if (e + 1 < epochs) {
                    if (e + 1 < C) { if (carry_valid[cs]) prune(cp0 + (e + 1) * K, cp0 + (e + 2) * K, pos); }
                    else prune(cur0 + (e + 1 - C) * K, cur0 + (e + 2 - C) * K, pos);
                } else {
                    const uint64_t x = pos + gap;
                    const int ex = cont0 ? prune(ccn0, ccn0 + K, x) : -1;
                    if (ex >= 0 && !keep_guess) for (int i = cn0; i < cn0 + K; i++) spec[i].stop.store(true, std::memory_order_relaxed);
                    else prune(cn0, cn0 + K, x);
                }
            }
            if (fr_depth > 0 && !cancelled) {
                std::lock_guard<std::mutex> lk(mu);
                const int t = e + 1 + fr_depth;
                int g0 = -1;
                if (t < epochs) g0 = cur0 + (t - C) * K;
                else if (t - epochs < C) g0 = cn0 + (t - epochs) * K;
                if (g0 >= 0) {
                    const double centre = (double)pos + fr_depth * Ew + (t >= epochs ? (double)gap : 0.0);
                    const double sd = sigma * std::sqrt((double)fr_depth);
                    for (int k = 0; k < K; k++) launch_walk(g0 + k, guess(centre, sd, k), b);
                }
                cv.notify_all();
            }
            if (overflow) {
                std::vector<uint32_t> Jh(n);
                const uint64_t e0 = shuffle_walk_host(key, stream, tck.front().first, n, Jh.data());
                hip_note(hipMemcpyAsync(d_J[slot] + (size_t)e * n, Jh.data(), 4ull * n, hipMemcpyHostToDevice, copy), "hipMemcpyAsync");
                hip_note(hipStreamSynchronize(copy), "hipStreamSynchronize");
                pos = e0;
            } else {
                WordRegions wr{};
                for (int bb = 0; bb < 2; bb++)
                    for (int g = 0; g < wb[bb].nreg; g++) {
                        wr.ptr[wr.n] = wb[bb].d + wb[bb].reg[g].off;
                        wr.base[wr.n] = wb[bb].reg[g].base;
                        wr.len[wr.n] = wb[bb].reg[g].len;
                        wr.n++;
                    }
                Seg *dS = d_seg[slot] + (size_t)e * maxseg;
                hip_note(hipMemcpyAsync(dS, S, sizeof(Seg) * (size_t)std::max(ns, 1), hipMemcpyHostToDevice, copy), "hipMemcpyAsync");
                xj_gate_wait(e);
                hipLaunchKernelGGL(k_expand_J, dim3((unsigned)((std::max(ns, 1) + XJ_WAVES - 1) / XJ_WAVES)),
                                   dim3(64 * XJ_WAVES), 0, copy, key, stream, (const Seg *)dS, ns, wr,
                                   d_J[slot] + (size_t)e * n);
                hip_note(hipGetLastError(), "k_expand_J launch");
            }
            end_pos[slot][e] = pos;
            hip_note(hipEventRecord(ev[slot][e], copy), "hipEventRecord");
            ev_used[slot][e] = true;
            walk_ms[slot][e] = std::chrono::duration<double, std::milli>(std::chrono::steady_clock::now() - t0).count();
            SHUF_LOG("[shuf] epoch %d end=%llu met=%d segs=%d (%.2f ms)\n", e, (unsigned long long)pos,
                     coalesced[slot][e], ns, walk_ms[slot][e]);
            {
                std::lock_guard<std::mutex> lk(mu);
                ready[slot] = e + 1;
            }
            cv.notify_all();
            if (K > 0) stop_walks(s0, s1);
            if (c1 > c0) { stop_walks(c0, c1); cont_valid[cs] = false; }
            if (e == C - 1) carry_valid[cs] = false;
        }
        SHUF_LOG("[shuf] job done cancelled=%d\n", (int)cancelled);
        stop_walks(cur0, cur1);
        if (cancelled) {
            stop_walks(0, nspec);
            carry_valid[0] = carry_valid[1] = false;
            cont_valid[0] = cont_valid[1] = false;
        }
        {
            std::lock_guard<std::mutex> lk(mu);
            running = -1;
            if (cancelled) {
                slot_valid[slot] = false;
            } else {
                chain_from = slot;
                chain_start = end_pos[slot][epochs - 1] + gap;
            }
        }
        cv.notify_all();
    }
}

bool ShuffleEngine::run_windowed(int slot, uint64_t start) {
    const int b = (int)(seq & 1);
    WordBuf &W = wb[b];
    auto chunks = [](double w) { return ((uint64_t)std::max(w, 1.0) + SHUF_CHUNK - 1) / SHUF_CHUNK * SHUF_CHUNK; };
    const uint64_t rlen = std::min(W.cap / (uint64_t)epochs, chunks(Ew + 10.0 * sigma + 4.0 * SHUF_CK));
    auto regions = [&](WordBuf &B, uint64_t s0, std::vector<size_t> &order) {
        std::vector<std::pair<double, size_t>> ord;
        B.nreg = epochs;
        for (int e = 0; e < epochs; e++) {
            WordBuf::Region &R = B.reg[e];
            R.base = (s0 + (uint64_t)e * win) / SHUF_CK * SHUF_CK;
            R.off = (uint64_t)e * rlen;
            R.len = rlen;
            for (uint64_t o = 0; o < R.len; o += SHUF_CHUNK) {
                const size_t c = (size_t)((R.off + o) / SHUF_CHUNK);
                B.ok[c] = 0;
                ord.push_back({(double)o + 0.25 * e, c});
            }
        }
        std::sort(ord.begin(), ord.end());
        order.clear();
        for (auto &oc : ord) order.push_back(oc.second);
    };
    auto make_words = [&](WordBuf &B, uint64_t s0, std::vector<size_t> &order) {
        regions(B, s0, order);
        for (int e = 0; e < epochs; e++)
            hipLaunchKernelGGL(k_chacha_words, dim3((unsigned)((B.reg[e].len / 16 + 255) / 256)), dim3(256), 0, copy,
                               key, stream, B.reg[e].base, B.reg[e].len, B.d + B.reg[e].off);
        hip_note(hipGetLastError(), "k_chacha_words launch");
        if (B.gpu) {
            hip_note(hipEventRecord(words_made, copy), "hipEventRecord");
            hip_note(hipStreamWaitEvent(d2h, words_made, 0), "hipStreamWaitEvent");
            for (size_t c : order) {
                const uint64_t o = c * SHUF_CHUNK;
                hip_note(hipMemcpyAsync(B.h + o, B.d + o, SHUF_CHUNK * 4, hipMemcpyDeviceToHost, d2h), "hipMemcpyAsync");
                hip_note(hipEventRecord(B.ev[c], d2h), "hipEventRecord");
            }
        }
        B.made_for = s0;
    };
    std::vector<size_t> order, next_order;
    if (!(W.gpu && W.made_for == start)) make_words(W, start, order);
    else regions(W, start, order);
    if (W.gpu) make_words(wb[b ^ 1], start + (uint64_t)epochs * win + gap, next_order);
    {
        std::unique_lock<std::mutex> lk(mu);
        cv.wait(lk, [&] { return gen_active == 0 || quit; });
        gen_order.clear();
        if (win_producers)
            for (size_t c : order) {
                const WordBuf::Region &R = W.reg[c * SHUF_CHUNK / rlen];
                gen_order.push_back({R.base + (c * SHUF_CHUNK - R.off), c});
            }
        gen_buf = &W;
        gen_next.store(0, std::memory_order_relaxed);
        gen_job++;
        for (int e = 0; e < epochs; e++) launch_walk(e, start + (uint64_t)e * win, b);
    }
    cv.notify_all();
    for (int e = 0; e < epochs; e++) {
        const auto t0 = std::chrono::steady_clock::now();
        if (ev_used[slot][e]) hip_note(hipEventSynchronize(ev[slot][e]), "hipEventSynchronize");
        SpecWalk &w = spec[e];
        {
            std::unique_lock<std::mutex> lk(mu);
            cv.wait(lk, [&] { return quit || cancel.load(std::memory_order_relaxed) ||
                                     (!w.running && w.done.load(std::memory_order_acquire)); });
            if (quit || cancel.load(std::memory_order_relaxed)) return false;
        }
        const uint64_t p0 = start + (uint64_t)e * win, pend = w.end;
        Seg *S = seg_host[slot] + (size_t)e * maxseg;
        int ns = 0;
        bool overflow = false;
        auto add = [&](uint64_t a, uint64_t z, uint32_t r0) {
            if (z <= a || r0 < 2) return;
            if (ns >= maxseg) { overflow = true; return; }
            S[ns++] = Seg{a, z, r0, 0};
        };
        uint64_t q = w.ck_base + SHUF_CK;
        add(p0, std::min(q, pend), n);
        for (size_t c = 1; q < pend; c++, q += SHUF_CK) {
            if (c >= w.ck.size()) { overflow = true; break; }
            add(q, std::min(q + SHUF_CK, pend), w.ck[c]);
        }
        if (overflow) {
            std::vector<uint32_t> Jh(n);
            (void)shuffle_walk_host(key, stream, p0, n, Jh.data());
            hip_note(hipMemcpyAsync(d_J[slot] + (size_t)e * n, Jh.data(), 4ull * n, hipMemcpyHostToDevice, copy), "hipMemcpyAsync");
            hip_note(hipStreamSynchronize(copy), "hipStreamSynchronize");
        } else {
            WordRegions wr{};
            wr.ptr[0] = W.d + W.reg[e].off; wr.base[0] = W.reg[e].base; wr.len[0] = W.reg[e].len; wr.n = 1;
            Seg *dS = d_seg[slot] + (size_t)e * maxseg;
            hip_note(hipMemcpyAsync(dS, S, sizeof(Seg) * (size_t)std::max(ns, 1), hipMemcpyHostToDevice, copy), "hipMemcpyAsync");
            xj_gate_wait(e);
            hipLaunchKernelGGL(k_expand_J, dim3((unsigned)((std::max(ns, 1) + XJ_WAVES - 1) / XJ_WAVES)),
                               dim3(64 * XJ_WAVES), 0, copy, key, stream, (const Seg *)dS, ns, wr,
                               d_J[slot] + (size_t)e * n);
            hip_note(hipGetLastError(), "k_expand_J launch");
        }
        end_pos[slot][e] = pend;
        coalesced[slot][e] = -1;
        hip_note(hipEventRecord(ev[slot][e], copy), "hipEventRecord");
        ev_used[slot][e] = true;
        walk_ms[slot][e] = std::chrono::duration<double, std::milli>(std::chrono::steady_clock::now() - t0).count();
        {
            std::lock_guard<std::mutex> lk(mu);
            ready[slot] = e + 1;
        }
        cv.notify_all();
    }
    return true;
}

void ShuffleEngine::shutdown() {
    if (th.joinable()) {
        {
            std::lock_guard<std::mutex> lk(mu);
            quit = true;
            cancel = true;
            for (int i = 0; i < nspec; i++) spec[i].stop = true;
        }
        cv.notify_all();
        th.join();
        for (auto &w : workers) w.join();
        workers.clear();
        for (auto &g : gens) g.join();
        gens.clear();
    }
    if (copy) { (void)hipStreamSynchronize(copy); (void)hipStreamDestroy(copy); copy = nullptr; }
    if (d2h) { (void)hipStreamSynchronize(d2h); (void)hipStreamDestroy(d2h); d2h = nullptr; }
    if (words_made) { (void)hipEventDestroy(words_made); words_made = nullptr; }
    for (int s = 0; s < 2; s++) {
        if (consumed[s]) { (void)hipEventDestroy(consumed[s]); consumed[s] = nullptr; }
        for (int e = 0; e < epochs; e++) if (ev[s][e]) { (void)hipEventDestroy(ev[s][e]); ev[s][e] = nullptr; }
        if (seg_host[s]) { (void)hipHostFree(seg_host[s]); seg_host[s] = nullptr; }
        if (d_seg[s]) { (void)hipFree(d_seg[s]); d_seg[s] = nullptr; }
        if (d_J[s]) { (void)hipFree(d_J[s]); d_J[s] = nullptr; }
    }
    for (int b = 0; b < 2; b++) {
        for (auto &e : wb[b].ev) if (e) (void)hipEventDestroy(e);
        wb[b].ev.clear();
        if (wb[b].d) { (void)hipFree(wb[b].d); wb[b].d = nullptr; }
        if (wb[b].h && wb[b].hd) (void)hipHostUnregister(wb[b].h);
        wb[b].hd = nullptr;
        if (wb[b].h) { host_words_free(wb[b].h, wb[b].cap); wb[b].h = nullptr; }
    }
}

hipError_t make_side_stream(int device, hipStream_t *st) {
    (void)device;
    int lo = 0, hi = 0;
    (void)hipDeviceGetStreamPriorityRange(&lo, &hi);
    static const bool normal = getenv("BPPO_SIDE_PRIO") && std::string(getenv("BPPO_SIDE_PRIO")) == "normal";
    if (normal) return hipStreamCreateWithFlags(st, hipStreamNonBlocking);
    return hipStreamCreateWithPriority(st, hipStreamNonBlocking, lo);
}

uint64_t shuffle_walk_host(const Key8 &key, uint64_t stream, uint64_t pos, uint32_t n, uint32_t *J) {
    const size_t C = (size_t)1 << 18;
    std::vector<uint32_t> w(C);
    uint32_t r = n;
    while (r >= 2) {
        bppo_host::chacha12_words(key.k, stream, pos, w.data(), C);
        pos += bppo_host::chain_walk(w.data(), C, &r, J);
    }
    if (n) J[0] = 0;
    return pos;
}

}
```

burn-ppo_amd/csrc/shuffle_host.cpp:

```cpp
#include "shuffle_host.h"

#include <immintrin.h>
#include <cstdlib>
#include <string.h>

namespace bppo_host {

typedef uint32_t u32;
typedef uint64_t u64;

static inline u32 rotl(u32 v, int n) { return (v << n) | (v >> (32 - n)); }

static void chacha12_block_scalar(const u32 key[8], u64 ctr, u64 stream, u32 out[16]) {
    u32 x[16] = {0x61707865u, 0x3320646eu, 0x79622d32u, 0x6b206574u, key[0], key[1], key[2], key[3],
                 key[4], key[5], key[6], key[7], (u32)ctr, (u32)(ctr >> 32), (u32)stream,
                 (u32)(stream >> 32)};
    u32 s[16];
    memcpy(s, x, sizeof s);
#define QR(a, b, c, d)                              \
    x[a] += x[b]; x[d] = rotl(x[d] ^ x[a], 16);     \
    x[c] += x[d]; x[b] = rotl(x[b] ^ x[c], 12);     \
    x[a] += x[b]; x[d] = rotl(x[d] ^ x[a], 8);      \
    x[c] += x[d]; x[b] = rotl(x[b] ^ x[c], 7);
    for (int r = 0; r < 6; r++) {
        QR(0, 4, 8, 12) QR(1, 5, 9, 13) QR(2, 6, 10, 14) QR(3, 7, 11, 15)
        QR(0, 5, 10, 15) QR(1, 6, 11, 12) QR(2, 7, 8, 13) QR(3, 4, 9, 14)
    }
#undef QR
    for (int i = 0; i < 16; i++) out[i] = x[i] + s[i];
}

__attribute__((target("avx2"))) static void chacha12_8blocks_avx2(const u32 key[8], u64 ctr, u64 stream,
                                                                  u32 *out) {
    __m256i x[16], s[16];
    x[0] = _mm256_set1_epi32(0x61707865); x[1] = _mm256_set1_epi32(0x3320646e);
    x[2] = _mm256_set1_epi32(0x79622d32); x[3] = _mm256_set1_epi32(0x6b206574);
    for (int i = 0; i < 8; i++) x[4 + i] = _mm256_set1_epi32((int)key[i]);
    u32 lo[8], hi[8];
    for (int l = 0; l < 8; l++) { u64 c = ctr + (u64)l; lo[l] = (u32)c; hi[l] = (u32)(c >> 32); }
    x[12] = _mm256_loadu_si256((const __m256i *)lo);
    x[13] = _mm256_loadu_si256((const __m256i *)hi);
    x[14] = _mm256_set1_epi32((int)(u32)stream);
    x[15] = _mm256_set1_epi32((int)(u32)(stream >> 32));
    for (int i = 0; i < 16; i++) s[i] = x[i];
    const __m256i r16 = _mm256_setr_epi8(2, 3, 0, 1, 6, 7, 4, 5, 10, 11, 8, 9, 14, 15, 12, 13,
                                         2, 3, 0, 1, 6, 7, 4, 5, 10, 11, 8, 9, 14, 15, 12, 13);
    const __m256i r8 = _mm256_setr_epi8(3, 0, 1, 2, 7, 4, 5, 6, 11, 8, 9, 10, 15, 12, 13, 14,
                                        3, 0, 1, 2, 7, 4, 5, 6, 11, 8, 9, 10, 15, 12, 13, 14);
#define ROTV(v, n) _mm256_or_si256(_mm256_slli_epi32(v, n), _mm256_srli_epi32(v, 32 - n))
#define QRV(a, b, c, d)                                                                   \
    x[a] = _mm256_add_epi32(x[a], x[b]); x[d] = _mm256_shuffle_epi8(_mm256_xor_si256(x[d], x[a]), r16); \
    x[c] = _mm256_add_epi32(x[c], x[d]); x[b] = ROTV(_mm256_xor_si256(x[b], x[c]), 12);              \
    x[a] = _mm256_add_epi32(x[a], x[b]); x[d] = _mm256_shuffle_epi8(_mm256_xor_si256(x[d], x[a]), r8);  \
    x[c] = _mm256_add_epi32(x[c], x[d]); x[b] = ROTV(_mm256_xor_si256(x[b], x[c]), 7);
    for (int r = 0; r < 6; r++) {
        QRV(0, 4, 8, 12) QRV(1, 5, 9, 13) QRV(2, 6, 10, 14) QRV(3, 7, 11, 15)
        QRV(0, 5, 10, 15) QRV(1, 6, 11, 12) QRV(2, 7, 8, 13) QRV(3, 4, 9, 14)
    }
#undef QRV
#undef ROTV
    for (int i = 0; i < 16; i++) x[i] = _mm256_add_epi32(x[i], s[i]);
    alignas(32) u32 t[16][8];
    for (int i = 0; i < 16; i++) _mm256_store_si256((__m256i *)t[i], x[i]);
    for (int l = 0; l < 8; l++)
        for (int i = 0; i < 16; i++) out[l * 16 + i] = t[i][l];
}

__attribute__((target("avx512f"))) static void chacha12_16blocks_avx512(const u32 key[8], u64 ctr, u64 stream,
                                                                       u32 *out) {
    __m512i x[16], s[16];
    x[0] = _mm512_set1_epi32(0x61707865); x[1] = _mm512_set1_epi32(0x3320646e);
    x[2] = _mm512_set1_epi32(0x79622d32); x[3] = _mm512_set1_epi32(0x6b206574);
    for (int i = 0; i < 8; i++) x[4 + i] = _mm512_set1_epi32((int)key[i]);
    u32 lo[16], hi[16];
    for (int l = 0; l < 16; l++) { u64 c = ctr + (u64)l; lo[l] = (u32)c; hi[l] = (u32)(c >> 32); }
    x[12] = _mm512_loadu_si512((const void *)lo);
    x[13] = _mm512_loadu_si512((const void *)hi);
    x[14] = _mm512_set1_epi32((int)(u32)stream);
    x[15] = _mm512_set1_epi32((int)(u32)(stream >> 32));
    for (int i = 0; i < 16; i++) s[i] = x[i];
#define QRZ(a, b, c, d)                                                                     \
    x[a] = _mm512_add_epi32(x[a], x[b]); x[d] = _mm512_rol_epi32(_mm512_xor_si512(x[d], x[a]), 16); \
    x[c] = _mm512_add_epi32(x[c], x[d]); x[b] = _mm512_rol_epi32(_mm512_xor_si512(x[b], x[c]), 12); \
    x[a] = _mm512_add_epi32(x[a], x[b]); x[d] = _mm512_rol_epi32(_mm512_xor_si512(x[d], x[a]), 8);  \
    x[c] = _mm512_add_epi32(x[c], x[d]); x[b] = _mm512_rol_epi32(_mm512_xor_si512(x[b], x[c]), 7);
    for (int r = 0; r < 6; r++) {
        QRZ(0, 4, 8, 12) QRZ(1, 5, 9, 13) QRZ(2, 6, 10, 14) QRZ(3, 7, 11, 15)
        QRZ(0, 5, 10, 15) QRZ(1, 6, 11, 12) QRZ(2, 7, 8, 13) QRZ(3, 4, 9, 14)
    }
#undef QRZ
    alignas(64) u32 t[16][16];
    for (int i = 0; i < 16; i++) _mm512_store_si512((void *)t[i], _mm512_add_epi32(x[i], s[i]));
    for (int l = 0; l < 16; l++)
        for (int i = 0; i < 16; i++) out[l * 16 + i] = t[i][l];
}

static bool have_avx512() {
    static int v = -1;
    if (v < 0) { __builtin_cpu_init(); v = __builtin_cpu_supports("avx512f") ? 1 : 0; }
    return v == 1;
}

static bool have_avx2() {
    static int v = -1;
    if (v < 0) { __builtin_cpu_init(); v = __builtin_cpu_supports("avx2") ? 1 : 0; }
    return v == 1;
}

void chacha12_words(const u32 key[8], u64 stream, u64 pos, u32 *out, size_t n) {
    size_t o = 0;
    u32 blk[128];
    if (pos & 15) {
        chacha12_block_scalar(key, pos >> 4, stream, blk);
        for (u64 w = pos & 15; w < 16 && o < n; w++) out[o++] = blk[w];
    }
    u64 b = (pos + o) >> 4;
    if (have_avx512()) {
        while (n - o >= 256) {
            chacha12_16blocks_avx512(key, b, stream, out + o);
            o += 256; b += 16;
        }
    }
    const bool v8 = have_avx2();
    while (n - o >= 128 && v8) {
        chacha12_8blocks_avx2(key, b, stream, out + o);
        o += 128; b += 8;
    }
    while (o < n) {
        chacha12_block_scalar(key, b, stream, blk);
        for (int w = 0; w < 16 && o < n; w++) out[o++] = blk[w];
        b++;
    }
}

static inline size_t walk_scalar(const u32 *w, size_t nw, u32 *rp, u32 *J) {
    u32 r = *rp;
    size_t p = 0;
    while (r >= 2 && p < nw) {
        const int lz = __builtin_clz(r);
        const u32 lowr = 1u << (31 - lz), s = 1u << lz;
        u32 z = (r << lz) - 1u;
        while (r >= lowr && r >= 2 && p < nw) {
            const u64 m = (u64)w[p++] * r;
            J[r - 1] = (u32)(m >> 32);
            const u32 acc = (u32)m <= z;
            r -= acc;
            z -= acc ? s : 0u;
        }
    }
    *rp = r;
    return p;
}

__attribute__((target("avx512f,avx512bw,avx512vl,avx512dq,bmi,bmi2,popcnt")))
static size_t walk_avx512(const u32 *w, size_t nw, u32 *rp, u32 *J) {
    u32 r = *rp;
    size_t p = 0;
    const __m512i kidx = _mm512_setr_epi32(0, 1, 2, 3, 4, 5, 6, 7, 8, 9, 10, 11, 12, 13, 14, 15);
    const __m512i rev = _mm512_setr_epi32(15, 14, 13, 12, 11, 10, 9, 8, 7, 6, 5, 4, 3, 2, 1, 0);
    while (r >= 2 && p < nw) {
        const int lz = __builtin_clz(r);
        const u32 lowr = 1u << (31 - lz), s = 1u << lz;
        while (r >= lowr + 24 && p + 16 <= nw) {
            const u32 z = (r << lz) - 1u;
            const __m512i wv = _mm512_loadu_si512((const void *)(w + p));
            const __m512i rk = _mm512_sub_epi32(_mm512_set1_epi32((int)r), kidx);
            __m512i lo = _mm512_mullo_epi32(wv, rk);
            __m512i zz = _mm512_sub_epi32(_mm512_set1_epi32((int)z), _mm512_slli_epi32(kidx, lz));
            const __m512i sv = _mm512_set1_epi32((int)s);
            u64 M[8];
            for (int j = 0; j < 8; j++) {
                M[j] = (u64)_mm512_cmple_epu32_mask(lo, zz);
                lo = _mm512_add_epi32(lo, wv);
                zz = _mm512_add_epi32(zz, sv);
            }
            u64 k = 0, rejmask = 0;
            for (int j = 0; j < 8; j++) {
                const u64 rej = ((~M[j]) & 0xFFFFull & (~0ull << k)) | (1ull << 16);
                const u64 kz = (u64)__builtin_ctzll(rej);
                rejmask |= 1ull << kz;
                k = kz + 1;
            }
            const u32 stop = k > 16 ? 16u : (u32)k;
            const u32 valid = (u32)((1u << stop) - 1u);
            const u32 am = (~(u32)rejmask) & valid;
            const u32 acc = (u32)__builtin_popcount(am);
            const __m512i wc = _mm512_maskz_compress_epi32((__mmask16)am, wv);
            const __m512i pe = _mm512_mul_epu32(wc, rk);
            const __m512i po = _mm512_mul_epu32(_mm512_srli_epi64(wc, 32), _mm512_srli_epi64(rk, 32));
            const __m512i hi = _mm512_mask_blend_epi32((__mmask16)0xAAAA, _mm512_srli_epi64(pe, 32), po);
            const __m512i hr = _mm512_permutexvar_epi32(rev, hi);
            const __mmask16 sm = (__mmask16)(0xFFFFu & ~((1u << (16 - acc)) - 1u));
            _mm512_mask_storeu_epi32((void *)(J + r - 16), sm, hr);
            r -= acc;
            p += stop;
        }
        u32 z = (r << lz) - 1u;
        while (r >= lowr && r >= 2 && p < nw) {
            const u64 m = (u64)w[p++] * r;
            J[r - 1] = (u32)(m >> 32);
            const u32 a = (u32)m <= z;
            r -= a;
            z -= a ? s : 0u;
            if (r >= lowr + 24 && p + 16 <= nw) break;
        }
    }
    *rp = r;
    return p;
}

static inline size_t walk_scalar_nj(const u32 *w, size_t nw, u32 *rp) {
    u32 r = *rp;
    size_t p = 0;
    while (r >= 2 && p < nw) {
        const int lz = __builtin_clz(r);
        const u32 lowr = 1u << (31 - lz), s = 1u << lz;
        u32 z = (r << lz) - 1u;
        while (r >= lowr && r >= 2 && p < nw) {
            const u32 lo = w[p++] * r;
            const u32 acc = lo <= z;
            r -= acc;
            z -= acc ? s : 0u;
        }
    }
    *rp = r;
    return p;
}

template <int NH>
__attribute__((target("avx512f,avx512bw,avx512vl,avx512dq,bmi,bmi2,popcnt")))
static size_t walk_avx512_nj_t(const u32 *w, size_t nw, u32 *rp) {
    u32 r = *rp;
    size_t p = 0;
    const __m512i kidx = _mm512_setr_epi32(0, 1, 2, 3, 4, 5, 6, 7, 8, 9, 10, 11, 12, 13, 14, 15);
    const __m512i kidx16 = _mm512_add_epi32(kidx, _mm512_set1_epi32(16));
    while (r >= 2 && p < nw) {
        const int lz = __builtin_clz(r);
        const u32 lowr = 1u << (31 - lz), s = 1u << lz;
        const __m512i sv = _mm512_set1_epi32((int)s);
        const __m512i kz = _mm512_slli_epi32(kidx, lz), kz16 = _mm512_slli_epi32(kidx16, lz);
        while (r >= lowr + 48 && p + 32 <= nw) {
            const u32 z = (r << lz) - 1u;
            const __m512i w0 = _mm512_loadu_si512((const void *)(w + p));
            const __m512i w1 = _mm512_loadu_si512((const void *)(w + p + 16));
            const __m512i rv = _mm512_set1_epi32((int)r), zv = _mm512_set1_epi32((int)z);
            __m512i lo0 = _mm512_mullo_epi32(w0, _mm512_sub_epi32(rv, kidx));
            __m512i lo1 = _mm512_mullo_epi32(w1, _mm512_sub_epi32(rv, kidx16));
            __m512i zz0 = _mm512_sub_epi32(zv, kz), zz1 = _mm512_sub_epi32(zv, kz16);
            u64 Z[NH];
            for (int j = 0; j < NH; j++) {
                const __mmask32 m = _mm512_kunpackw(_mm512_cmple_epu32_mask(lo1, zz1), _mm512_cmple_epu32_mask(lo0, zz0));
                Z[j] = (u64)(u32)~_cvtmask32_u32(m) | 0xFFFFFFFF00000000ull;
                lo0 = _mm512_add_epi32(lo0, w0); lo1 = _mm512_add_epi32(lo1, w1);
                zz0 = _mm512_add_epi32(zz0, sv); zz1 = _mm512_add_epi32(zz1, sv);
            }
            u64 L = 0;
            for (int j = 0; j < NH; j++) L = _blsmsk_u64(Z[j] & ~L);
            const u32 P = (u32)__builtin_popcountll(L);
            r -= P - NH;
            p += P < 32 ? P : 32;
        }
        u32 z = (r << lz) - 1u;
        while (r >= lowr && r >= 2 && p < nw) {
            const u32 lo = w[p++] * r;
            const u32 a = lo <= z;
            r -= a;
            z -= a ? s : 0u;
            if (r >= lowr + 48 && p + 32 <= nw) break;
        }
    }
    *rp = r;
    return p;
}
static size_t walk_avx512_nj(const u32 *w, size_t nw, u32 *rp) { return walk_avx512_nj_t<10>(w, nw, rp); }

template <int NH>
__attribute__((target("avx512f,avx512bw,avx512vl,avx512dq,bmi,bmi2,popcnt"), always_inline))
static inline u32 block32(const u32 *w, u32 &r) {
    const int lz = __builtin_clz(r);
    const u32 z = (r << lz) - 1u;
    const __m512i kidx = _mm512_setr_epi32(0, 1, 2, 3, 4, 5, 6, 7, 8, 9, 10, 11, 12, 13, 14, 15);
    const __m512i kidx16 = _mm512_add_epi32(kidx, _mm512_set1_epi32(16));
    const __m512i sv = _mm512_set1_epi32((int)(1u << lz));
    const __m512i w0 = _mm512_loadu_si512((const void *)w);
    const __m512i w1 = _mm512_loadu_si512((const void *)(w + 16));
    const __m512i rv = _mm512_set1_epi32((int)r), zv = _mm512_set1_epi32((int)z);
    __m512i lo0 = _mm512_mullo_epi32(w0, _mm512_sub_epi32(rv, kidx));
    __m512i lo1 = _mm512_mullo_epi32(w1, _mm512_sub_epi32(rv, kidx16));
    __m512i zz0 = _mm512_sub_epi32(zv, _mm512_slli_epi32(kidx, lz));
    __m512i zz1 = _mm512_sub_epi32(zv, _mm512_slli_epi32(kidx16, lz));
    u64 Z[NH];
    for (int j = 0; j < NH; j++) {
        const __mmask32 m = _mm512_kunpackw(_mm512_cmple_epu32_mask(lo1, zz1), _mm512_cmple_epu32_mask(lo0, zz0));
        Z[j] = (u64)(u32)~_cvtmask32_u32(m) | 0xFFFFFFFF00000000ull;
        lo0 = _mm512_add_epi32(lo0, w0); lo1 = _mm512_add_epi32(lo1, w1);
        zz0 = _mm512_add_epi32(zz0, sv); zz1 = _mm512_add_epi32(zz1, sv);
    }
    u64 L = 0;
    for (int j = 0; j < NH; j++) L = _blsmsk_u64(Z[j] & ~L);
    const u32 P = (u32)__builtin_popcountll(L);
    r -= P - NH;
    return P < 32 ? P : 32;
}

static inline bool block_ok(u32 r, size_t p, size_t nw) {
    const u32 lowr = 1u << (31 - __builtin_clz(r));
    return r >= lowr + 48 && p + 32 <= nw;
}

static inline void steps_until_block(const u32 *w, size_t nw, size_t &p, u32 &r) {
    while (r >= 2 && p < nw) {
        if (r >= 2 && block_ok(r, p, nw)) return;
        const int lz = __builtin_clz(r);
        const u32 lo = w[p++] * r;
        r -= lo <= (r << lz) - 1u;
    }
}

__attribute__((target("avx512f,avx512bw,avx512vl,avx512dq,bmi,bmi2,popcnt")))
static void walk2_avx512_nj(const u32 *wa, size_t na, u32 *rap, size_t *ua, const u32 *wb, size_t nb, u32 *rbp,
                            size_t *ub) {
    u32 ra = *rap, rb = *rbp;
    size_t pa = 0, pb = 0;
    for (;;) {
        while (block_ok(ra, pa, na) && block_ok(rb, pb, nb)) {
            pa += block32<10>(wa + pa, ra);
            pb += block32<10>(wb + pb, rb);
        }
        steps_until_block(wa, na, pa, ra);
        steps_until_block(wb, nb, pb, rb);
        const bool da = ra < 2 || pa >= na || !block_ok(ra, pa, na);
        const bool db = rb < 2 || pb >= nb || !block_ok(rb, pb, nb);
        if (da || db) break;
    }
    *rap = ra; *rbp = rb; *ua = pa; *ub = pb;
}

static int isa_level() {
    static int v = -1;
    if (v < 0) {
        __builtin_cpu_init();
        v = (__builtin_cpu_supports("avx512f") && __builtin_cpu_supports("avx512bw") &&
             __builtin_cpu_supports("avx512vl") && __builtin_cpu_supports("avx512dq")) ? 2 : 1;
    }
    return v;
}

int chain_walk_isa() { return isa_level(); }

size_t chain_walk_nj(const u32 *w, size_t nw, u32 *r) {
    if (isa_level() == 2) return walk_avx512_nj(w, nw, r);
    return walk_scalar_nj(w, nw, r);
}

void chain_walk2_nj(const u32 *wa, size_t na, u32 *ra, size_t *ua, const u32 *wb, size_t nb, u32 *rb, size_t *ub) {
    if (isa_level() == 2) return walk2_avx512_nj(wa, na, ra, ua, wb, nb, rb, ub);
    *ua = walk_scalar_nj(wa, na, ra);
    *ub = walk_scalar_nj(wb, nb, rb);
}

size_t chain_walk(const u32 *w, size_t nw, u32 *r, u32 *J) {
    if (isa_level() == 2) return walk_avx512(w, nw, r, J);
    return walk_scalar(w, nw, r, J);
}

}
```

burn-ppo_amd/csrc/shuffle_host.h:

```cpp
#pragma once
#include <stddef.h>
#include <stdint.h>

namespace bppo_host {

void chacha12_words(const uint32_t key[8], uint64_t stream, uint64_t pos, uint32_t *out, size_t n);

size_t chain_walk(const uint32_t *w, size_t nw, uint32_t *r, uint32_t *J);

size_t chain_walk_nj(const uint32_t *w, size_t nw, uint32_t *r);

void chain_walk2_nj(const uint32_t *wa, size_t na, uint32_t *ra, size_t *ua,
                    const uint32_t *wb, size_t nb, uint32_t *rb, size_t *ub);

int chain_walk_isa();

}
```

include/bppo.h:

```cpp
#ifndef BPPO_H
#define BPPO_H

#include <stddef.h>
#include <stdint.h>

#ifdef __cplusplus
extern "C" {
#endif

typedef enum {
    BPPO_OK = 0,
    BPPO_ERR_ARG = 1,
    BPPO_ERR_NONFINITE = 2,
    BPPO_ERR_EMPTY_MASK = 3,
    BPPO_ERR_HIP = 4,
    BPPO_ERR_COMM = 5,
    BPPO_ERR_UNSUPPORTED = 6
} bppo_status;

typedef enum { BPPO_ENV_CARTPOLE = 0, BPPO_ENV_CONNECT_FOUR = 1, BPPO_ENV_LIARS_DICE = 2, BPPO_ENV_SKULL = 3 } bppo_env_kind;
#define BPPO_MAX_PLAYERS 6

typedef struct {
    int32_t env_kind;
    int32_t num_envs;
    int32_t num_steps;
    int32_t hidden_size, num_hidden, relu;
    int32_t ctde, critic_hidden_size, critic_num_hidden;
    int32_t num_epochs, num_minibatches;
    int32_t normalize_obs, normalize_returns, clip_value;
    double gamma, gae_lambda, clip_epsilon, value_coef, max_grad_norm, adam_epsilon;
    double target_kl;
    double return_clip;
    double reward_shaping_coef;
    uint64_t seed;
    uint64_t env_seed_base;
    uint64_t rng_stream;
    int32_t cnn, num_conv_layers, conv_channels[4], kernel_size, cnn_fc_hidden_size, cnn_num_fc_layers;
    int32_t normalize_values;
    int32_t player_count;
    int32_t split_networks;
    int32_t shuffle_windows;
} bppo_config;

typedef struct {
    float total_reward[BPPO_MAX_PLAYERS];
    int32_t length;
    int32_t env_index;
    int32_t step;
    int32_t pad;
} bppo_episode;

typedef struct {
    int32_t episodes;
    float mean_return;
    float mean_length;
    int32_t pad;
    uint64_t rng_word_pos;
} bppo_rollout_info;

typedef struct {
    float policy_loss, value_loss, entropy, entropy_scaled, approx_kl, clip_fraction;
    float explained_variance, total_loss, value_mean, returns_mean;
    float adv_mean_raw, adv_std_raw, adv_min_raw, adv_max_raw;
    float value_error_mean, value_error_std, value_error_max;
    float avg_valid_actions, entropy_valid_pct;
    int32_t num_updates, epochs_run;
    float value_norm_target_mean, value_norm_target_std, value_norm_rescale_mag;
} bppo_update_metrics;

typedef struct bppo_ctx bppo_ctx;

bppo_status bppo_create(const bppo_config *cfg, int hip_device, void *hip_stream, bppo_ctx **out);
void bppo_destroy(bppo_ctx *ctx);
const char *bppo_last_error(const bppo_ctx *ctx);
const char *bppo_version(void);
size_t bppo_config_size(void);
size_t bppo_update_metrics_size(void);
size_t bppo_episode_size(void);
size_t bppo_rollout_info_size(void);

size_t bppo_num_params(const bppo_ctx *ctx);
bppo_status bppo_params_set(bppo_ctx *ctx, const float *host, size_t n);
bppo_status bppo_params_get(bppo_ctx *ctx, float *host, size_t n);
bppo_status bppo_forward(bppo_ctx *ctx, const float *obs, const float *priv, int32_t B,
                         float *logits, float *values);

bppo_status bppo_rng_get(bppo_ctx *ctx, uint64_t *word_pos);
bppo_status bppo_rng_set(bppo_ctx *ctx, uint64_t word_pos);
bppo_status bppo_rng_fill_bytes(bppo_ctx *ctx, uint8_t *dst, size_t n);
bppo_status bppo_rng_from_seed(bppo_ctx *ctx, const uint8_t *seed);
bppo_status bppo_rng_key_get(bppo_ctx *ctx, uint32_t key[8]);

size_t bppo_num_param_tensors(const bppo_ctx *ctx);
bppo_status bppo_optimizer_get(bppo_ctx *ctx, float *m1, float *m2, int32_t *steps, size_t n);
bppo_status bppo_optimizer_set(bppo_ctx *ctx, const float *m1, const float *m2, const int32_t *steps, size_t n);

bppo_status bppo_vecenv_reset(bppo_ctx *ctx);
bppo_status bppo_vecenv_observe(bppo_ctx *ctx, float *obs, int32_t *players, uint8_t *masks,
                                float *priv);
bppo_status bppo_vecenv_step(bppo_ctx *ctx, const int32_t *actions, float *obs, float *rewards,
                             uint8_t *dones, bppo_episode *eps, int32_t cap, int32_t *n_eps);
bppo_status bppo_vecenv_set_step(bppo_ctx *ctx, uint64_t global_step);
bppo_status bppo_set_reward_shaping_schedule(bppo_ctx *ctx, const double *values, const uint64_t *steps,
                                             int32_t n);

bppo_status bppo_obs_norm_get(bppo_ctx *ctx, double *mean, double *m2, double *count);
bppo_status bppo_obs_norm_set(bppo_ctx *ctx, const double *mean, const double *m2, double count);
bppo_status bppo_ret_norm_get(bppo_ctx *ctx, double *mvc, double *returns);
bppo_status bppo_ret_norm_set(bppo_ctx *ctx, const double *mvc, const double *returns);
bppo_status bppo_popart_get(bppo_ctx *ctx, double *state4);
bppo_status bppo_popart_set(bppo_ctx *ctx, const double *state4);

bppo_status bppo_collect_rollouts(bppo_ctx *ctx, bppo_rollout_info *info);
bppo_status bppo_rollout_episodes(bppo_ctx *ctx, bppo_episode *eps, int32_t cap, int32_t *n);
bppo_status bppo_compute_gae(bppo_ctx *ctx);
bppo_status bppo_ppo_update(bppo_ctx *ctx, double lr, double ent_coef, bppo_update_metrics *m);
bppo_status bppo_train_step(bppo_ctx *ctx, double lr, double ent_coef, bppo_rollout_info *info,
                            bppo_update_metrics *m);
bppo_status bppo_train_steps(bppo_ctx *ctx, int32_t n, const double *lr, const double *ent_coef,
                             uint64_t global_step0, bppo_rollout_info *infos, bppo_update_metrics *ms,
                             const char *const *phase_keys, int32_t nkeys, float *phase_sums);

typedef int (*bppo_allreduce_fn)(float *device_buf, size_t n, void *user);
bppo_status bppo_set_allreduce(bppo_ctx *ctx, bppo_allreduce_fn fn, void *user, int32_t world_size);
bppo_status bppo_set_rank(bppo_ctx *ctx, int32_t rank);

bppo_status bppo_set_allreduce_async(bppo_ctx *ctx, bppo_allreduce_fn fn, void *user, int32_t world_size);
bppo_status bppo_get_stream(bppo_ctx *ctx, void **hip_stream);

bppo_status bppo_opponents_set(bppo_ctx *ctx, int32_t n_models, const float *params, const double *norm_mean,
                               const double *norm_m2, const double *norm_count, int32_t num_opponent_envs,
                               const int32_t *learner_pos, const int32_t *pos_to_opp, const int32_t *current_opp);
bppo_status bppo_opponents_get_envs(bppo_ctx *ctx, int32_t *learner_pos, int32_t *pos_to_opp);

int32_t bppo_minibatch_rows(bppo_ctx *ctx, float *out, int32_t max_rows, int32_t *row_width);
bppo_status bppo_buffer_get(bppo_ctx *ctx, const char *name, void *host, size_t bytes);
bppo_status bppo_buffer_set(bppo_ctx *ctx, const char *name, const void *host, size_t bytes);

bppo_status bppo_gae_device(const float *rewards, const float *dones, const float *values,
                            const float *last_values, int32_t T, int32_t N, float gamma,
                            float lambda, float *advantages, float *returns, void *hip_stream);
bppo_status bppo_gae_rows_device(const float *rewards, const float *dones, const float *values,
                                 const float *last_values, int32_t T, int32_t N, float gamma,
                                 float lambda, float *advantages, float *returns, float *pairs,
                                 void *hip_stream);
bppo_status bppo_gae_mp_device(const float *all_rewards, const int32_t *players,
                               const float *dones, const float *values, const float *last_v_pp,
                               int32_t T, int32_t N, int32_t P, float gamma, float lambda,
                               float *advantages, float *returns, void *hip_stream);

bppo_status bppo_set_explained_variance_mode(bppo_ctx *ctx, int32_t mode);

bppo_status bppo_set_minibatch_kernel(bppo_ctx *ctx, int32_t mode);

bppo_status bppo_debug_record_params(bppo_ctx *ctx, float *host, int32_t max_minibatches);

bppo_status bppo_last_kernel_ms(bppo_ctx *ctx, const char *kernel, float *ms);

bppo_status bppo_debug_libm(int32_t which, int32_t device, const float *x, float *y, size_t n);

bppo_status bppo_debug_shuffle_chain(uint64_t seed, uint64_t stream, uint64_t word_pos, uint32_t n,
                                     uint32_t *J, uint64_t *end_pos);
bppo_status bppo_debug_fisher_yates(int32_t device, const uint32_t *J, uint32_t n, uint32_t *perm);
bppo_status bppo_debug_chain_walk2(uint64_t seed, uint64_t stream, uint64_t pos_a, uint64_t pos_b, uint32_t n,
                                   uint32_t piece, uint64_t *end_a, uint64_t *end_b);
bppo_status bppo_debug_shuffle_engine(uint64_t seed, uint64_t stream, uint64_t start, uint32_t n, int32_t epochs,
                                      uint64_t gap, int32_t jobs, int32_t windows, uint32_t *J, uint64_t *ends,
                                      int32_t *met);

bppo_status bppo_debug_sample(int32_t A, int32_t B, const float *logits, const uint8_t *masks, uint64_t seed,
                              uint64_t stream, uint64_t word_pos, int32_t *actions, float *log_probs);

bppo_status bppo_debug_gemm(int32_t mode, int32_t M, int32_t N, int32_t K, const float *A, const float *B,
                            const float *bias_or_H, int32_t act, float *out, float *out2);

#ifdef __cplusplus
}
#endif
#endif
```

Before: 654.5 million.

## Record rejection bitmasks during host chain walk to simplify GPU J expansion

The host-side shuffle chain walk now records, per chunk, a bitmask of which random words were accepted. The GPU expand kernel then uses these masks to place each accepted word directly, instead of re-running the rejection-sampling walk with wave ballots. This is meant to cut GPU expand cost and serial per-segment work. In exchange it adds host bit bookkeeping, extra pinned and device buffers and copies, and it removes the optional event gate on the copy stream.

```diff
diff --git a/burn-ppo_amd/bppo/_lib.py b/burn-ppo_amd/bppo/_lib.py
--- a/burn-ppo_amd/bppo/_lib.py
+++ b/burn-ppo_amd/bppo/_lib.py
@@ -77,7 +77,7 @@
     "bppo_optimizer_get", "bppo_optimizer_set", "bppo_popart_get", "bppo_popart_set",
     "bppo_config_size", "bppo_update_metrics_size", "bppo_episode_size", "bppo_rollout_info_size",
     "bppo_set_explained_variance_mode", "bppo_set_minibatch_kernel", "bppo_set_rank",
-    "bppo_debug_record_params",
+    "bppo_debug_record_params", "bppo_debug_walk_bits", "bppo_debug_walk2_bits", "bppo_debug_expand_bits",
 )
 
 STRUCT_SIZES = {"bppo_config_size": Config, "bppo_update_metrics_size": UpdateMetrics,
@@ -159,6 +159,9 @@
         "bppo_set_explained_variance_mode": (i32, [vp, i32]),
         "bppo_set_minibatch_kernel": (i32, [vp, i32]),
         "bppo_debug_record_params": (i32, [vp, vp, i32]),
+        "bppo_debug_walk_bits": (i32, [vp, sz, vp, vp, u64, i32, C.POINTER(sz)]),
+        "bppo_debug_walk2_bits": (i32, [vp, sz, vp, vp, u64, C.POINTER(sz), vp, sz, vp, vp, u64, C.POINTER(sz), i32]),
+        "bppo_debug_expand_bits": (i32, [i32, vp, u64, sz, vp, vp, vp, vp, i32, C.c_uint32, vp]),
     }
     for name in STRUCT_SIZES:
         sig[name] = (sz, [])
diff --git a/burn-ppo_amd/csrc/bppo_api.hip b/burn-ppo_amd/csrc/bppo_api.hip
--- a/burn-ppo_amd/csrc/bppo_api.hip
+++ b/burn-ppo_amd/csrc/bppo_api.hip
@@ -330,7 +330,6 @@
     }
     c->rng_key = seed_key(cfg->seed);
     c->rng_pos = 0;
-    c->shuf.gate = c->ev_upd;
     TRY(c->shuf.init(dev, c->rng_key, cfg->rng_stream, (uint32_t)TN, cfg->num_epochs, TN * (uint64_t)c->A, c->err,
                      cfg->shuffle_windows != 0));
     if (c->fy_shared) c->fy_stream = c->shuf.copy;
@@ -489,7 +488,6 @@
     c->rng_pos = 0;
     c->shuf_slot = -1;
     const size_t TN = (size_t)c->T * c->N;
-    c->shuf.gate = c->ev_upd;
     TRY(c->shuf.init(c->dev, c->rng_key, c->cfg.rng_stream, (uint32_t)TN, c->cfg.num_epochs, TN * (uint64_t)c->A, c->err,
                      c->cfg.shuffle_windows != 0));
     if (c->fy_shared) c->fy_stream = c->shuf.copy;
diff --git a/burn-ppo_amd/csrc/bppo_internal.h b/burn-ppo_amd/csrc/bppo_internal.h
--- a/burn-ppo_amd/csrc/bppo_internal.h
+++ b/burn-ppo_amd/csrc/bppo_internal.h
@@ -60,6 +60,11 @@
     uint64_t start = 0, end = 0, ck_base = 0;
     int wbuf = 0;
     std::vector<uint32_t> ck;
+    uint64_t *bits = nullptr;
+    uint64_t bits_cap = 0;
+    uint64_t *bits_own = nullptr;
+    uint64_t bits_own_cap = 0;
+    hipEvent_t bits_ev = nullptr;
     std::atomic<int64_t> progress{-1};
     std::atomic<int> done{1};
     std::atomic<bool> stop{false};
@@ -150,14 +155,17 @@
     int ready[2] = {0, 0};
     uint64_t end_pos[2][SHUF_MAX_EPOCHS];
     struct Seg { uint64_t pos0, pos1; uint32_t r0, pad; };
+    static constexpr int SEG_BITW = (int)(SHUF_CK / 64);
     int maxseg = 0;
     Seg *seg_host[2] = {nullptr, nullptr};
     Seg *d_seg[2] = {nullptr, nullptr};
+    uint64_t *bits_host[2] = {nullptr, nullptr};
+    uint64_t *spec_bits = nullptr;
+    uint64_t *d_bits[2] = {nullptr, nullptr};
     uint32_t *d_J[2] = {nullptr, nullptr};
     hipEvent_t ev[2][SHUF_MAX_EPOCHS] = {};
     bool ev_used[2][SHUF_MAX_EPOCHS] = {};
     hipStream_t copy = nullptr;
-    hipEvent_t gate = nullptr;
     double walk_ms[2][SHUF_MAX_EPOCHS] = {};
     int coalesced[2][SHUF_MAX_EPOCHS] = {};
     std::atomic<uint64_t> spec_words{0}, true_words{0};
@@ -165,7 +173,6 @@
     bppo_status init(int device, const Key8 &key, uint64_t stream, uint32_t n_, int epochs_, uint64_t gap_,
                      std::string &err, bool windows = false);
     bool run_windowed(int slot, uint64_t start);
-    void xj_gate_wait(int e);
     uint64_t job_end(int slot) const { return win ? slot_start[slot] + (uint64_t)epochs * win : end_pos[slot][epochs - 1]; }
     std::atomic<bool> hip_bad{false};
     std::mutex hip_mu;
@@ -179,7 +186,7 @@
     void shutdown();
     void run();
     void worker(int i);
-    void launch_walk(int i, uint64_t start, int wbuf);
+    void launch_walk(int i, uint64_t start, int wbuf, uint64_t *bits = nullptr, uint64_t bits_cap = 0);
     void stop_walks(int lo, int hi);
     const uint32_t *words(int b, uint64_t pos, uint64_t len, std::vector<uint32_t> &scratch, bool true_walk = false);
     int alt_b = -1;
@@ -187,9 +194,9 @@
     struct WalkStats { uint64_t words = 0, tsc_walk = 0, tsc_words = 0; };
     void walk_pair(int i, WalkStats &st);
     uint64_t walk_piece(int b, uint64_t pos, uint32_t *r, std::vector<uint32_t> &scratch, WalkStats &st,
-                        bool true_walk = false);
+                        bool true_walk, uint64_t *bits, uint64_t bits_base, uint64_t bits_cap);
     void flush(WalkStats &st, std::atomic<uint64_t> &words_ctr);
-    int peek(int i, uint64_t q, uint32_t *r);
+    int peek(int i, uint64_t q, uint32_t *r, int *src = nullptr);
 };
 uint64_t shuffle_walk_host(const Key8 &key, uint64_t stream, uint64_t pos, uint32_t n, uint32_t *J);
 hipError_t make_side_stream(int device, hipStream_t *st);
diff --git a/burn-ppo_amd/csrc/shuffle_engine.hip b/burn-ppo_amd/csrc/shuffle_engine.hip
--- a/burn-ppo_amd/csrc/shuffle_engine.hip
+++ b/burn-ppo_amd/csrc/shuffle_engine.hip
@@ -48,7 +48,6 @@
     int n;
 };
 constexpr int XJ_WAVES = 4;
-constexpr int XJ_H = 16;
 
 __device__ __forceinline__ uint32_t xj_word(const Key8 &key, uint64_t stream, const WordRegions &wr, uint64_t q) {
     for (int k = 0; k < wr.n; k++)
@@ -61,89 +60,39 @@
     return v;
 }
 
-__global__ void __launch_bounds__(64 * XJ_WAVES) k_expand_J(Key8 key, uint64_t stream, const ShuffleEngine::Seg *segs,
-                                                          int ns, WordRegions wr, uint32_t *J) {
+__global__ void __launch_bounds__(64 * XJ_WAVES) k_expand_bits(Key8 key, uint64_t stream, const ShuffleEngine::Seg *segs,
+                                                             const uint64_t *bits, int ns, WordRegions wr, uint32_t n,
+                                                             uint32_t *J) {
+    constexpr int BW = ShuffleEngine::SEG_BITW;
     const int lane = threadIdx.x & 63;
     const int si = blockIdx.x * XJ_WAVES + (threadIdx.x >> 6);
-    if (si == 0 && lane == 0) J[0] = 0;
+    if (si == 0 && lane == 0 && n) J[0] = 0;
     if (si >= ns) return;
     const ShuffleEngine::Seg g = segs[si];
-    uint32_t r = g.r0;
-    uint64_t q = g.pos0;
-    uint32_t avail = q < g.pos1 ? (uint32_t)min((uint64_t)64, g.pos1 - q) : 0u;
-    uint32_t w = lane < (int)avail ? xj_word(key, stream, wr, q + lane) : 0u;
-    while (q < g.pos1 && r >= 2) {
-        const uint64_t qn = q + 64;
-        const uint32_t availn = qn < g.pos1 ? (uint32_t)min((uint64_t)64, g.pos1 - qn) : 0u;
-        const uint32_t wn = lane < (int)availn ? xj_word(key, stream, wr, qn + lane) : 0u;
-        const int lz = __clz(r);
-        const uint32_t lowr = 1u << (31 - lz);
-        if (r >= lowr + 64 && r >= 66) {
-            const uint32_t s = 1u << lz;
-            const uint32_t rj = r - (uint32_t)lane;
-            uint32_t lo = w * rj, z = (rj << lz) - 1u;
-            const uint64_t valid = avail >= 64 ? ~0ull : ((1ull << avail) - 1ull);
-            uint64_t rejm = 0;
-            uint32_t b = avail;
-            uint32_t nrej = 0;
-            uint64_t from = 0;
-            bool open = true;
-#pragma unroll
-            for (int h = 0; h < XJ_H; h++) {
-                const uint64_t acc = __ballot(lo <= z);
-                lo += w;
-                z += s;
-                if (open) {
-                    const uint64_t rem = ~acc & valid & ~from;
-                    if (rem == 0) { open = false; continue; }
-                    const int jh = __builtin_ctzll(rem);
-                    rejm |= 1ull << jh;
-                    nrej++;
-                    from = jh == 63 ? ~0ull : ((2ull << jh) - 1ull);
-                    if (h == XJ_H - 1) b = (uint32_t)jh + 1;
-                }
-            }
-            const uint32_t below = (uint32_t)__builtin_amdgcn_mbcnt_hi((uint32_t)(rejm >> 32),
-                                                                      __builtin_amdgcn_mbcnt_lo((uint32_t)rejm, 0u));
-            if ((uint32_t)lane < b && !((rejm >> lane) & 1ull)) {
-                const uint32_t rr = r - (uint32_t)lane + below;
-                J[rr - 1] = __umulhi(w, rr);
-            }
-            r -= b - nrej;
-            q += b;
-        } else {
-            uint32_t rr = r, used = 0;
-            if (lane == 0) {
-                int lz1 = __clz(rr);
-                uint32_t lowr1 = 1u << (31 - lz1), sh = 1u << lz1, z = (rr << lz1) - 1u;
-                for (uint32_t j = 0; j < avail && rr >= 2; j++) {
-                    const uint32_t wj = xj_word(key, stream, wr, q + j);
-                    const uint64_t m = (uint64_t)wj * rr;
-                    used = j + 1;
-                    if ((uint32_t)m <= z) {
-                        J[rr - 1] = (uint32_t)(m >> 32);
-                        rr--;
-                        z -= sh;
-                        if (rr < lowr1 && rr >= 1) { lz1 = __clz(rr); lowr1 = 1u << (31 - lz1); sh = 1u << lz1; z = (rr << lz1) - 1u; }
-                    }
-                }
-            }
-            r = __shfl(rr, 0, 64);
-            q += __shfl(used, 0, 64);
-        }
-        if (q == qn) {
-            w = wn;
-            avail = availn;
-        } else if (q < g.pos1) {
-            avail = (uint32_t)min((uint64_t)64, g.pos1 - q);
-            w = lane < (int)avail ? xj_word(key, stream, wr, q + lane) : 0u;
-        }
-    }
-}
-
-void ShuffleEngine::xj_gate_wait(int e) {
-    static const int mode = getenv("BPPO_XJ_GATE") ? atoi(getenv("BPPO_XJ_GATE")) : 0;
-    if (gate && (mode == 1 || (mode == 2 && e > 0))) hip_note(hipStreamWaitEvent(copy, gate, 0), "hipStreamWaitEvent");
+    const uint64_t base = g.pos0 & ~(SHUF_CK - 1);
+    if (g.pos1 <= g.pos0 || g.pos1 > base + SHUF_CK) return;
+    const int a = (int)(g.pos0 - base), b = (int)(g.pos1 - base);
+    uint64_t m = 0;
+    if (lane < BW) {
+        const int f = min(max(a - 64 * lane, 0), 64), t = min(max(b - 64 * lane, 0), 64);
+        const uint64_t below_t = t >= 64 ? ~0ull : ((1ull << t) - 1ull);
+        const uint64_t below_f = f >= 64 ? ~0ull : ((1ull << f) - 1ull);
+        m = bits[(size_t)si * BW + lane] & below_t & ~below_f;
+    }
+    uint32_t before = 0;
+#pragma unroll 4
+    for (int s = 0; s < BW; s++) {
+        const uint32_t mlo = (uint32_t)__shfl((int)(uint32_t)m, s, 64);
+        const uint32_t mhi = (uint32_t)__shfl((int)(uint32_t)(m >> 32), s, 64);
+        const uint64_t ms = ((uint64_t)mhi << 32) | mlo;
+        if ((ms >> lane) & 1ull) {
+            const uint32_t below = (uint32_t)__builtin_amdgcn_mbcnt_hi(mhi, __builtin_amdgcn_mbcnt_lo(mlo, 0u));
+            const uint32_t rr = g.r0 - before - below;
+            const uint32_t w = xj_word(key, stream, wr, base + (uint64_t)(64 * s + lane));
+            if (rr >= 2 && rr <= g.r0 && rr <= n) J[rr - 1] = __umulhi(w, rr);
+        }
+        before += (uint32_t)__popcll(ms);
+    }
 }
 
 static void shuffle_word_stats(uint32_t n, double &mean, double &sd) {
@@ -208,9 +157,12 @@
     const size_t bytes = sizeof(uint32_t) * (size_t)n * epochs;
     maxseg = (int)((Ew + 48.0 * sigma) / SHUF_CK) + 16;
     const size_t sbytes = sizeof(Seg) * (size_t)maxseg * epochs;
+    const size_t bbytes = sizeof(uint64_t) * SEG_BITW * (size_t)maxseg * epochs;
     for (int s = 0; s < 2; s++) {
         if (hipHostMalloc((void **)&seg_host[s], sbytes, hipHostMallocDefault) != hipSuccess ||
             hipMalloc((void **)&d_seg[s], sbytes) != hipSuccess ||
+            hipHostMalloc((void **)&bits_host[s], bbytes, hipHostMallocDefault) != hipSuccess ||
+            hipMalloc((void **)&d_bits[s], bbytes) != hipSuccess ||
             hipMalloc((void **)&d_J[s], bytes) != hipSuccess) {
             err = "shuffle buffers: allocation failed";
             return BPPO_ERR_HIP;
@@ -274,6 +226,13 @@
     }
     const uint64_t nck = (uint64_t)((Ew + 24.0 * sigma) / SHUF_CK) + 4;
     for (int i = 0; i < nspec; i++) spec[i].ck.assign(nck, 0xFFFFFFFFu);
+    if (!win && nspec > 0) {
+        if (hipHostMalloc((void **)&spec_bits, sizeof(uint64_t) * SEG_BITW * nck * (size_t)nspec, hipHostMallocDefault) != hipSuccess) {
+            err = "shuffle bit buffers: allocation failed";
+            return BPPO_ERR_HIP;
+        }
+        for (int i = 0; i < nspec; i++) { spec[i].bits_own = spec_bits + (size_t)i * nck * SEG_BITW; spec[i].bits_own_cap = nck; }
+    }
     for (int i = 0; i < nspec; i++) workers.emplace_back([this, i]() { worker(i); });
     const int ngen = win && !win_producers ? 0 : std::max(1, std::min(4, host_cpus / 4));
     for (int i = 0; i < ngen; i++) gens.emplace_back([this]() { generator(); });
@@ -373,12 +332,14 @@
 }
 
 uint64_t ShuffleEngine::walk_piece(int b, uint64_t pos, uint32_t *r, std::vector<uint32_t> &scratch, WalkStats &st,
-                                   bool true_walk) {
+                                   bool true_walk, uint64_t *bits, uint64_t bits_base, uint64_t bits_cap) {
     const uint64_t q = (pos / SHUF_CK + 1) * SHUF_CK;
     const uint64_t t0 = __rdtsc();
     const uint32_t *w = words(b, pos, q - pos, scratch, true_walk);
     const uint64_t t1 = __rdtsc();
-    const uint64_t used = bppo_host::chain_walk_nj(w, (size_t)(q - pos), r);
+    const bool rec = bits && pos >= bits_base && (pos - bits_base) / SHUF_CK < bits_cap;
+    const uint64_t used = rec ? bppo_host::chain_walk_bits(w, (size_t)(q - pos), r, bits, pos - bits_base)
+                              : bppo_host::chain_walk_nj(w, (size_t)(q - pos), r);
     st.tsc_words += t1 - t0;
     st.tsc_walk += __rdtsc() - t1;
     st.words += used;
@@ -391,11 +352,14 @@
     st = WalkStats{};
 }
 
-void ShuffleEngine::launch_walk(int i, uint64_t start, int wbuf) {
+void ShuffleEngine::launch_walk(int i, uint64_t start, int wbuf, uint64_t *bits, uint64_t bits_cap) {
     SpecWalk &s = spec[i];
     s.start = start;
     s.ck_base = start / SHUF_CK * SHUF_CK;
     s.wbuf = wbuf;
+    if (s.bits_ev) { hip_note(hipEventSynchronize(s.bits_ev), "hipEventSynchronize"); s.bits_ev = nullptr; }
+    s.bits = bits ? bits : s.bits_own;
+    s.bits_cap = bits ? bits_cap : s.bits_own_cap;
     s.end = 0;
     std::fill(s.ck.begin(), s.ck.end(), 0xFFFFFFFFu);
     s.progress.store(-1, std::memory_order_relaxed);
@@ -419,15 +383,15 @@
     });
 }
 
-int ShuffleEngine::peek(int i, uint64_t q, uint32_t *r) {
+int ShuffleEngine::peek(int i, uint64_t q, uint32_t *r, int *src) {
     for (;;) {
         SpecWalk &t = spec[i];
         if (q <= t.start) return -1;
         const int mt = t.merged_to.load(std::memory_order_acquire);
-        if (mt >= 0 && q >= t.merge_q) { i = mt; continue; }
+        if (mt >= 0 && q > t.merge_q) { i = mt; continue; }
         const int64_t c = (int64_t)((q - t.ck_base) / SHUF_CK);
         if (c >= (int64_t)t.ck.size()) return -1;
-        if (t.progress.load(std::memory_order_acquire) >= c) { *r = t.ck[c]; return 1; }
+        if (t.progress.load(std::memory_order_acquire) >= c) { *r = t.ck[c]; if (src) *src = i; return 1; }
         if (t.done.load(std::memory_order_acquire) && t.merged_to.load(std::memory_order_acquire) < 0) return -1;
         return 0;
     }
@@ -461,7 +425,7 @@
         uint32_t r = n;
         while (r >= 2 && !s.stop.load(std::memory_order_relaxed)) {
             const uint64_t q = (pos / SHUF_CK + 1) * SHUF_CK;
-            pos = walk_piece(s.wbuf, pos, &r, scratch, wst);
+            pos = walk_piece(s.wbuf, pos, &r, scratch, wst, false, s.bits, s.ck_base, s.bits_cap);
             if (pos == q) {
                 const int64_t c = (int64_t)((q - s.ck_base) / SHUF_CK);
                 if (c < (int64_t)s.ck.size()) {
@@ -513,6 +477,7 @@
         st.tsc_words += __rdtsc() - t0;
         c.left = (size_t)(q - c.pos);
     };
+    auto rec = [&](const Chain &c) { return c.s->bits && (c.pos - c.s->ck_base) / SHUF_CK < c.s->bits_cap; };
     auto finish = [&](Chain &c) {
         c.live = false;
         c.s->end = c.pos;
@@ -548,7 +513,11 @@
     while (ch[0].live && ch[1].live) {
         size_t u0 = 0, u1 = 0;
         const uint64_t t0 = __rdtsc();
-        bppo_host::chain_walk2_nj(ch[0].w, ch[0].left, &ch[0].r, &u0, ch[1].w, ch[1].left, &ch[1].r, &u1);
+        if (rec(ch[0]) && rec(ch[1]))
+            bppo_host::chain_walk2_bits(ch[0].w, ch[0].left, &ch[0].r, &u0, ch[0].s->bits, ch[0].pos - ch[0].s->ck_base,
+                                        ch[1].w, ch[1].left, &ch[1].r, &u1, ch[1].s->bits, ch[1].pos - ch[1].s->ck_base);
+        else
+            bppo_host::chain_walk2_nj(ch[0].w, ch[0].left, &ch[0].r, &u0, ch[1].w, ch[1].left, &ch[1].r, &u1);
         st.tsc_walk += __rdtsc() - t0;
         advance(ch[0], u0);
         advance(ch[1], u1);
@@ -557,7 +526,8 @@
         Chain &c = ch[k];
         while (c.live) {
             const uint64_t t0 = __rdtsc();
-            const size_t u = bppo_host::chain_walk_nj(c.w, c.left, &c.r);
+            const size_t u = rec(c) ? bppo_host::chain_walk_bits(c.w, c.left, &c.r, c.s->bits, c.pos - c.s->ck_base)
+                                    : bppo_host::chain_walk_nj(c.w, c.left, &c.r);
             st.tsc_walk += __rdtsc() - t0;
             advance(c, u);
         }
@@ -751,6 +721,9 @@
         bool cancelled = false;
         WalkStats tst;
         std::vector<std::pair<uint64_t, uint32_t>> tck;
+        struct BitRun { const uint64_t *src; size_t si0, cnt; };
+        std::vector<BitRun> runs;
+        std::vector<int> used_walks;
         for (int e = 0; e < epochs && !cancelled; e++) {
             auto t0 = std::chrono::steady_clock::now();
             if (ev_used[slot][e]) hip_note(hipEventSynchronize(ev[slot][e]), "hipEventSynchronize");
@@ -763,6 +736,33 @@
             if (e == 0 && cont0 && cont_valid[cs]) { c0 = ccp0; c1 = ccp0 + K; }
             tck.clear();
             tck.push_back({pos, r});
+            uint64_t *SB = bits_host[slot] + (size_t)e * maxseg * SEG_BITW;
+            bool bits_missing = false;
+            runs.clear();
+            used_walks.clear();
+            auto own_row = [&]() -> uint64_t * {
+                return tck.size() - 1 < (size_t)maxseg ? SB + (tck.size() - 1) * SEG_BITW : nullptr;
+            };
+            auto stage = [&](int src) {
+                const size_t si = tck.size() - 1;
+                if (si >= (size_t)maxseg) return;
+                const uint64_t p0 = tck.back().first / SHUF_CK * SHUF_CK;
+                const uint64_t *from = SB + si * SEG_BITW;
+                if (src >= 0) {
+                    const SpecWalk &t = spec[src];
+                    if (!t.bits || p0 < t.ck_base || (p0 - t.ck_base) / SHUF_CK >= t.bits_cap) { bits_missing = true; return; }
+                    from = t.bits + (p0 - t.ck_base) / SHUF_CK * SEG_BITW;
+                    if (used_walks.empty() || used_walks.back() != src) used_walks.push_back(src);
+                }
+                if (!runs.empty() && runs.back().si0 + runs.back().cnt == si && runs.back().src + runs.back().cnt * SEG_BITW == from)
+                    runs.back().cnt++;
+                else
+                    runs.push_back(BitRun{from, si, 1});
+            };
+            auto push = [&](uint64_t q, uint32_t rq, int src) {
+                stage(src);
+                tck.push_back({q, rq});
+            };
             int fin = -1;
             uint64_t endp = 0, chain_front = 0;
             auto frontier = [&](int i) -> uint64_t {
@@ -799,9 +799,10 @@
                     const bool chain_done = spec[f].done.load(std::memory_order_acquire) != 0 &&
                                             spec[f].merged_to.load(std::memory_order_acquire) < 0;
                     uint32_t rr = 0;
+                    int src = -1;
                     const bool recheck = keep_guess && s1 > s0 && met >= c0 && met < c1;
-                    for (uint64_t q = (pos / SHUF_CK + 1) * SHUF_CK; r >= 2 && peek(met, q, &rr) == 1; q += SHUF_CK) {
-                        tck.push_back({q, rr});
+                    for (uint64_t q = (pos / SHUF_CK + 1) * SHUF_CK; r >= 2 && peek(met, q, &rr, &src) == 1; q += SHUF_CK) {
+                        push(q, rr, src);
                         pos = q;
                         r = rr;
                         if (recheck && try_switch(q, rr)) break;
@@ -819,10 +820,10 @@
                     }
                 }
                 const uint64_t q = (pos / SHUF_CK + 1) * SHUF_CK;
-                pos = walk_piece(b, pos, &r, scratch, tst, true);
+                pos = walk_piece(b, pos, &r, scratch, tst, true, own_row(), pos / SHUF_CK * SHUF_CK, 1);
                 if (cancel.load(std::memory_order_relaxed)) { cancelled = true; break; }
                 if (pos != q || r < 2) continue;
-                tck.push_back({q, r});
+                push(q, r, -1);
                 if (s0 == s1 && c0 == c1) continue;
                 if (met < 0) walked++;
                 try_switch(q, r);
@@ -839,7 +840,9 @@
             };
             for (size_t i = 0; i + 1 < tck.size(); i++) add(tck[i].first, tck[i + 1].first, tck[i].second);
             if (fin >= 0) pos = endp;
+            if (pos > tck.back().first && tck.back().second >= 2) stage(fin);
             add(tck.back().first, pos, tck.back().second);
+            overflow = overflow || bits_missing;
             coalesced[slot][e] = met >= 0 ? walked : -1;
             auto prune = [&](int g0, int g1, uint64_t x) {
                 int lo = -1, hi = -1, exact = -1;
@@ -898,16 +901,24 @@
                         wr.n++;
                     }
                 Seg *dS = d_seg[slot] + (size_t)e * maxseg;
+                uint64_t *dB = d_bits[slot] + (size_t)e * maxseg * SEG_BITW;
                 hip_note(hipMemcpyAsync(dS, S, sizeof(Seg) * (size_t)std::max(ns, 1), hipMemcpyHostToDevice, copy), "hipMemcpyAsync");
-                xj_gate_wait(e);
-                hipLaunchKernelGGL(k_expand_J, dim3((unsigned)((std::max(ns, 1) + XJ_WAVES - 1) / XJ_WAVES)),
-                                   dim3(64 * XJ_WAVES), 0, copy, key, stream, (const Seg *)dS, ns, wr,
-                                   d_J[slot] + (size_t)e * n);
-                hip_note(hipGetLastError(), "k_expand_J launch");
+                for (const BitRun &rn : runs)
+                    if (rn.si0 + rn.cnt <= (size_t)ns)
+                        hip_note(hipMemcpyAsync(dB + rn.si0 * SEG_BITW, rn.src, sizeof(uint64_t) * SEG_BITW * rn.cnt,
+                                                hipMemcpyHostToDevice, copy), "hipMemcpyAsync");
+                hipLaunchKernelGGL(k_expand_bits, dim3((unsigned)((std::max(ns, 1) + XJ_WAVES - 1) / XJ_WAVES)),
+                                   dim3(64 * XJ_WAVES), 0, copy, key, stream, (const Seg *)dS, (const uint64_t *)dB, ns, wr,
+                                   n, d_J[slot] + (size_t)e * n);
+                hip_note(hipGetLastError(), "k_expand_bits launch");
             }
             end_pos[slot][e] = pos;
             hip_note(hipEventRecord(ev[slot][e], copy), "hipEventRecord");
             ev_used[slot][e] = true;
+            if (!used_walks.empty()) {
+                std::lock_guard<std::mutex> lk(mu);
+                for (int i : used_walks) spec[i].bits_ev = ev[slot][e];
+            }
             walk_ms[slot][e] = std::chrono::duration<double, std::milli>(std::chrono::steady_clock::now() - t0).count();
             SHUF_LOG("[shuf] epoch %d end=%llu met=%d segs=%d (%.2f ms)\n", e, (unsigned long long)pos,
                      coalesced[slot][e], ns, walk_ms[slot][e]);
@@ -985,6 +996,8 @@
     if (!(W.gpu && W.made_for == start)) make_words(W, start, order);
     else regions(W, start, order);
     if (W.gpu) make_words(wb[b ^ 1], start + (uint64_t)epochs * win + gap, next_order);
+    for (int e = 0; e < epochs; e++)
+        if (ev_used[slot][e]) hip_note(hipEventSynchronize(ev[slot][e]), "hipEventSynchronize");
     {
         std::unique_lock<std::mutex> lk(mu);
         cv.wait(lk, [&] { return gen_active == 0 || quit; });
@@ -997,7 +1010,9 @@
         gen_buf = &W;
         gen_next.store(0, std::memory_order_relaxed);
         gen_job++;
-        for (int e = 0; e < epochs; e++) launch_walk(e, start + (uint64_t)e * win, b);
+        for (int e = 0; e < epochs; e++)
+            launch_walk(e, start + (uint64_t)e * win, b, bits_host[slot] + (size_t)e * maxseg * SEG_BITW,
+                        std::min<uint64_t>((uint64_t)maxseg, spec[e].ck.size()));
     }
     cv.notify_all();
     for (int e = 0; e < epochs; e++) {
@@ -1034,12 +1049,14 @@
             WordRegions wr{};
             wr.ptr[0] = W.d + W.reg[e].off; wr.base[0] = W.reg[e].base; wr.len[0] = W.reg[e].len; wr.n = 1;
             Seg *dS = d_seg[slot] + (size_t)e * maxseg;
+            const size_t bo = (size_t)e * maxseg * SEG_BITW;
             hip_note(hipMemcpyAsync(dS, S, sizeof(Seg) * (size_t)std::max(ns, 1), hipMemcpyHostToDevice, copy), "hipMemcpyAsync");
-            xj_gate_wait(e);
-            hipLaunchKernelGGL(k_expand_J, dim3((unsigned)((std::max(ns, 1) + XJ_WAVES - 1) / XJ_WAVES)),
-                               dim3(64 * XJ_WAVES), 0, copy, key, stream, (const Seg *)dS, ns, wr,
-                               d_J[slot] + (size_t)e * n);
-            hip_note(hipGetLastError(), "k_expand_J launch");
+            hip_note(hipMemcpyAsync(d_bits[slot] + bo, bits_host[slot] + bo, sizeof(uint64_t) * SEG_BITW * (size_t)std::max(ns, 1),
+                                    hipMemcpyHostToDevice, copy), "hipMemcpyAsync");
+            hipLaunchKernelGGL(k_expand_bits, dim3((unsigned)((std::max(ns, 1) + XJ_WAVES - 1) / XJ_WAVES)),
+                               dim3(64 * XJ_WAVES), 0, copy, key, stream, (const Seg *)dS, (const uint64_t *)(d_bits[slot] + bo),
+                               ns, wr, n, d_J[slot] + (size_t)e * n);
+            hip_note(hipGetLastError(), "k_expand_bits launch");
         }
         end_pos[slot][e] = pend;
         coalesced[slot][e] = -1;
@@ -1073,11 +1090,14 @@
     if (copy) { (void)hipStreamSynchronize(copy); (void)hipStreamDestroy(copy); copy = nullptr; }
     if (d2h) { (void)hipStreamSynchronize(d2h); (void)hipStreamDestroy(d2h); d2h = nullptr; }
     if (words_made) { (void)hipEventDestroy(words_made); words_made = nullptr; }
+    if (spec_bits) { (void)hipHostFree(spec_bits); spec_bits = nullptr; }
     for (int s = 0; s < 2; s++) {
         if (consumed[s]) { (void)hipEventDestroy(consumed[s]); consumed[s] = nullptr; }
         for (int e = 0; e < epochs; e++) if (ev[s][e]) { (void)hipEventDestroy(ev[s][e]); ev[s][e] = nullptr; }
         if (seg_host[s]) { (void)hipHostFree(seg_host[s]); seg_host[s] = nullptr; }
         if (d_seg[s]) { (void)hipFree(d_seg[s]); d_seg[s] = nullptr; }
+        if (bits_host[s]) { (void)hipHostFree(bits_host[s]); bits_host[s] = nullptr; }
+        if (d_bits[s]) { (void)hipFree(d_bits[s]); d_bits[s] = nullptr; }
         if (d_J[s]) { (void)hipFree(d_J[s]); d_J[s] = nullptr; }
     }
     for (int b = 0; b < 2; b++) {
@@ -1112,3 +1132,58 @@
 }
 
 }
+
+extern "C" bppo_status bppo_debug_walk_bits(const uint32_t *words, size_t nw, uint32_t *r_inout, uint64_t *bits,
+                                            uint64_t bit0, int32_t isa, size_t *used) {
+    if (!words || !r_inout || !bits || !used || (isa != 1 && isa != 2)) return BPPO_ERR_ARG;
+    *used = bppo_host::chain_walk_bits_isa(isa, words, nw, r_inout, bits, bit0);
+    return BPPO_OK;
+}
+
+extern "C" bppo_status bppo_debug_walk2_bits(const uint32_t *words_a, size_t na, uint32_t *ra_inout, uint64_t *bits_a,
+                                             uint64_t bit0_a, size_t *used_a, const uint32_t *words_b, size_t nb,
+                                             uint32_t *rb_inout, uint64_t *bits_b, uint64_t bit0_b, size_t *used_b,
+                                             int32_t isa) {
+    if (!words_a || !words_b || !ra_inout || !rb_inout || !bits_a || !bits_b || !used_a || !used_b ||
+        (isa != 1 && isa != 2))
+        return BPPO_ERR_ARG;
+    bppo_host::chain_walk2_bits_isa(isa, words_a, na, ra_inout, used_a, bits_a, bit0_a, words_b, nb, rb_inout, used_b,
+                                    bits_b, bit0_b);
+    return BPPO_OK;
+}
+
+extern "C" bppo_status bppo_debug_expand_bits(int32_t device, const uint32_t *words, uint64_t word_base, size_t nw,
+                                              const uint64_t *pos0, const uint64_t *pos1, const uint32_t *r0,
+                                              const uint64_t *bits, int32_t ns, uint32_t n, uint32_t *J) {
+    using namespace bppo;
+    if (!words || !pos0 || !pos1 || !r0 || !bits || !J || ns < 1 || n < 1 || nw < 1) return BPPO_ERR_ARG;
+    std::vector<ShuffleEngine::Seg> segs((size_t)ns);
+    for (int i = 0; i < ns; i++) {
+        if (pos1[i] <= pos0[i] || pos1[i] > (pos0[i] & ~(SHUF_CK - 1)) + SHUF_CK || pos0[i] < word_base ||
+            pos1[i] > word_base + nw || r0[i] < 2 || r0[i] > n)
+            return BPPO_ERR_ARG;
+        segs[(size_t)i] = ShuffleEngine::Seg{pos0[i], pos1[i], r0[i], 0};
+    }
+    if (hipSetDevice(device) != hipSuccess) return BPPO_ERR_HIP;
+    uint32_t *dW = nullptr, *dJ = nullptr;
+    uint64_t *dB = nullptr;
+    ShuffleEngine::Seg *dS = nullptr;
+    const size_t bb = sizeof(uint64_t) * ShuffleEngine::SEG_BITW * (size_t)ns;
+    bppo_status s = BPPO_ERR_HIP;
+    if (hipMalloc((void **)&dW, 4 * nw) == hipSuccess && hipMalloc((void **)&dJ, 4ull * n) == hipSuccess &&
+        hipMalloc((void **)&dB, bb) == hipSuccess && hipMalloc((void **)&dS, sizeof(ShuffleEngine::Seg) * (size_t)ns) == hipSuccess &&
+        hipMemcpy(dW, words, 4 * nw, hipMemcpyHostToDevice) == hipSuccess &&
+        hipMemcpy(dJ, J, 4ull * n, hipMemcpyHostToDevice) == hipSuccess &&
+        hipMemcpy(dB, bits, bb, hipMemcpyHostToDevice) == hipSuccess &&
+        hipMemcpy(dS, segs.data(), sizeof(ShuffleEngine::Seg) * (size_t)ns, hipMemcpyHostToDevice) == hipSuccess) {
+        WordRegions wr{};
+        wr.ptr[0] = dW; wr.base[0] = word_base; wr.len[0] = nw; wr.n = 1;
+        hipLaunchKernelGGL(k_expand_bits, dim3((unsigned)((ns + XJ_WAVES - 1) / XJ_WAVES)), dim3(64 * XJ_WAVES), 0, 0,
+                           Key8{}, 0ull, (const ShuffleEngine::Seg *)dS, (const uint64_t *)dB, (int)ns, wr, n, dJ);
+        if (hipGetLastError() == hipSuccess && hipDeviceSynchronize() == hipSuccess &&
+            hipMemcpy(J, dJ, 4ull * n, hipMemcpyDeviceToHost) == hipSuccess)
+            s = BPPO_OK;
+    }
+    (void)hipFree(dW); (void)hipFree(dJ); (void)hipFree(dB); (void)hipFree(dS);
+    return s;
+}
diff --git a/burn-ppo_amd/csrc/shuffle_host.cpp b/burn-ppo_amd/csrc/shuffle_host.cpp
--- a/burn-ppo_amd/csrc/shuffle_host.cpp
+++ b/burn-ppo_amd/csrc/shuffle_host.cpp
@@ -209,9 +209,53 @@
     return p;
 }
 
-static inline size_t walk_scalar_nj(const u32 *w, size_t nw, u32 *rp) {
+template <bool BITS>
+struct BitAcc {
+    u64 *p = nullptr;
+    u64 acc = 0;
+    u32 n = 0;
+    inline void open(u64 *bits, u64 bit0) {
+        if (!BITS) return;
+        p = bits + (bit0 >> 6);
+        n = (u32)(bit0 & 63);
+        acc = n ? *p & ((1ull << n) - 1ull) : 0ull;
+    }
+    inline void put(u64 v, u32 k) {
+        if (!BITS) return;
+        acc |= v << n;
+        *p = acc;
+        const u32 m = n + k;
+        const u64 spill = (v >> 1) >> (63 - n);
+        acc = m >= 64 ? spill : acc;
+        p += m >> 6;
+        n = m & 63;
+    }
+    u64 one_v = 0;
+    u32 one_k = 0;
+    inline void one(u32 a) {
+        if (!BITS) return;
+        one_v |= (u64)a << one_k;
+        if (++one_k == 32) ones();
+    }
+    inline void ones() {
+        if (!BITS || !one_k) return;
+        put(one_v, one_k);
+        one_v = 0;
+        one_k = 0;
+    }
+    inline void flush() {
+        if (!BITS) return;
+        ones();
+        if (n) *p = acc;
+    }
+};
+
+template <bool BITS>
+static inline size_t walk_scalar_nj(const u32 *w, size_t nw, u32 *rp, u64 *bits, u64 bit0) {
     u32 r = *rp;
     size_t p = 0;
+    BitAcc<BITS> ba;
+    ba.open(bits, bit0);
     while (r >= 2 && p < nw) {
         const int lz = __builtin_clz(r);
         const u32 lowr = 1u << (31 - lz), s = 1u << lz;
@@ -219,19 +263,23 @@
         while (r >= lowr && r >= 2 && p < nw) {
             const u32 lo = w[p++] * r;
             const u32 acc = lo <= z;
+            ba.one(acc);
             r -= acc;
             z -= acc ? s : 0u;
         }
     }
+    ba.flush();
     *rp = r;
     return p;
 }
 
-template <int NH>
+template <int NH, bool BITS>
 __attribute__((target("avx512f,avx512bw,avx512vl,avx512dq,bmi,bmi2,popcnt")))
-static size_t walk_avx512_nj_t(const u32 *w, size_t nw, u32 *rp) {
+static size_t walk_avx512_nj_t(const u32 *w, size_t nw, u32 *rp, u64 *bits, u64 bit0) {
     u32 r = *rp;
     size_t p = 0;
+    BitAcc<BITS> ba;
+    ba.open(bits, bit0);
     const __m512i kidx = _mm512_setr_epi32(0, 1, 2, 3, 4, 5, 6, 7, 8, 9, 10, 11, 12, 13, 14, 15);
     const __m512i kidx16 = _mm512_add_epi32(kidx, _mm512_set1_epi32(16));
     while (r >= 2 && p < nw) {
@@ -239,6 +287,7 @@
         const u32 lowr = 1u << (31 - lz), s = 1u << lz;
         const __m512i sv = _mm512_set1_epi32((int)s);
         const __m512i kz = _mm512_slli_epi32(kidx, lz), kz16 = _mm512_slli_epi32(kidx16, lz);
+        ba.ones();
         while (r >= lowr + 48 && p + 32 <= nw) {
             const u32 z = (r << lz) - 1u;
             const __m512i w0 = _mm512_loadu_si512((const void *)(w + p));
@@ -254,29 +303,36 @@
                 lo0 = _mm512_add_epi32(lo0, w0); lo1 = _mm512_add_epi32(lo1, w1);
                 zz0 = _mm512_add_epi32(zz0, sv); zz1 = _mm512_add_epi32(zz1, sv);
             }
-            u64 L = 0;
-            for (int j = 0; j < NH; j++) L = _blsmsk_u64(Z[j] & ~L);
+            u64 L = 0, R = 0;
+            for (int j = 0; j < NH; j++) {
+                L = _blsmsk_u64(Z[j] & ~L);
+                if (BITS) R += L;
+            }
+            if (BITS) R = (R + NH) >> 1;
             const u32 P = (u32)__builtin_popcountll(L);
+            const u32 used = P < 32 ? P : 32;
+            ba.put(_bzhi_u64(~R, used), used);
             r -= P - NH;
-            p += P < 32 ? P : 32;
+            p += used;
         }
         u32 z = (r << lz) - 1u;
         while (r >= lowr && r >= 2 && p < nw) {
             const u32 lo = w[p++] * r;
             const u32 a = lo <= z;
+            ba.one(a);
             r -= a;
             z -= a ? s : 0u;
             if (r >= lowr + 48 && p + 32 <= nw) break;
         }
     }
+    ba.flush();
     *rp = r;
     return p;
 }
-static size_t walk_avx512_nj(const u32 *w, size_t nw, u32 *rp) { return walk_avx512_nj_t<10>(w, nw, rp); }
-
-template <int NH>
+
+template <int NH, bool BITS>
 __attribute__((target("avx512f,avx512bw,avx512vl,avx512dq,bmi,bmi2,popcnt"), always_inline))
-static inline u32 block32(const u32 *w, u32 &r) {
+static inline u32 block32(const u32 *w, u32 &r, BitAcc<BITS> &ba) {
     const int lz = __builtin_clz(r);
     const u32 z = (r << lz) - 1u;
     const __m512i kidx = _mm512_setr_epi32(0, 1, 2, 3, 4, 5, 6, 7, 8, 9, 10, 11, 12, 13, 14, 15);
@@ -296,11 +352,17 @@
         lo0 = _mm512_add_epi32(lo0, w0); lo1 = _mm512_add_epi32(lo1, w1);
         zz0 = _mm512_add_epi32(zz0, sv); zz1 = _mm512_add_epi32(zz1, sv);
     }
-    u64 L = 0;
-    for (int j = 0; j < NH; j++) L = _blsmsk_u64(Z[j] & ~L);
+    u64 L = 0, R = 0;
+    for (int j = 0; j < NH; j++) {
+        L = _blsmsk_u64(Z[j] & ~L);
+        if (BITS) R += L;
+    }
+    if (BITS) R = (R + NH) >> 1;
     const u32 P = (u32)__builtin_popcountll(L);
+    const u32 used = P < 32 ? P : 32;
+    ba.put(_bzhi_u64(~R, used), used);
     r -= P - NH;
-    return P < 32 ? P : 32;
+    return used;
 }
 
 static inline bool block_ok(u32 r, size_t p, size_t nw) {
@@ -308,31 +370,42 @@
     return r >= lowr + 48 && p + 32 <= nw;
 }
 
-static inline void steps_until_block(const u32 *w, size_t nw, size_t &p, u32 &r) {
+template <bool BITS>
+static inline void steps_until_block(const u32 *w, size_t nw, size_t &p, u32 &r, BitAcc<BITS> &ba) {
     while (r >= 2 && p < nw) {
         if (r >= 2 && block_ok(r, p, nw)) return;
         const int lz = __builtin_clz(r);
         const u32 lo = w[p++] * r;
-        r -= lo <= (r << lz) - 1u;
-    }
-}
-
+        const u32 a = lo <= (r << lz) - 1u;
+        ba.one(a);
+        r -= a;
+    }
+}
+
+template <bool BITS>
 __attribute__((target("avx512f,avx512bw,avx512vl,avx512dq,bmi,bmi2,popcnt")))
 static void walk2_avx512_nj(const u32 *wa, size_t na, u32 *rap, size_t *ua, const u32 *wb, size_t nb, u32 *rbp,
-                            size_t *ub) {
+                            size_t *ub, u64 *bits_a, u64 bit0_a, u64 *bits_b, u64 bit0_b) {
     u32 ra = *rap, rb = *rbp;
     size_t pa = 0, pb = 0;
+    BitAcc<BITS> ba, bb;
+    ba.open(bits_a, bit0_a);
+    bb.open(bits_b, bit0_b);
     for (;;) {
+        ba.ones();
+        bb.ones();
         while (block_ok(ra, pa, na) && block_ok(rb, pb, nb)) {
-            pa += block32<10>(wa + pa, ra);
-            pb += block32<10>(wb + pb, rb);
-        }
-        steps_until_block(wa, na, pa, ra);
-        steps_until_block(wb, nb, pb, rb);
+            pa += block32<10, BITS>(wa + pa, ra, ba);
+            pb += block32<10, BITS>(wb + pb, rb, bb);
+        }
+        steps_until_block<BITS>(wa, na, pa, ra, ba);
+        steps_until_block<BITS>(wb, nb, pb, rb, bb);
         const bool da = ra < 2 || pa >= na || !block_ok(ra, pa, na);
         const bool db = rb < 2 || pb >= nb || !block_ok(rb, pb, nb);
         if (da || db) break;
     }
+    ba.flush();
+    bb.flush();
     *rap = ra; *rbp = rb; *ua = pa; *ub = pb;
 }
 
@@ -349,14 +422,39 @@
 int chain_walk_isa() { return isa_level(); }
 
 size_t chain_walk_nj(const u32 *w, size_t nw, u32 *r) {
-    if (isa_level() == 2) return walk_avx512_nj(w, nw, r);
-    return walk_scalar_nj(w, nw, r);
+    if (isa_level() == 2) return walk_avx512_nj_t<10, false>(w, nw, r, nullptr, 0);
+    return walk_scalar_nj<false>(w, nw, r, nullptr, 0);
 }
 
 void chain_walk2_nj(const u32 *wa, size_t na, u32 *ra, size_t *ua, const u32 *wb, size_t nb, u32 *rb, size_t *ub) {
-    if (isa_level() == 2) return walk2_avx512_nj(wa, na, ra, ua, wb, nb, rb, ub);
-    *ua = walk_scalar_nj(wa, na, ra);
-    *ub = walk_scalar_nj(wb, nb, rb);
+    if (isa_level() == 2) return walk2_avx512_nj<false>(wa, na, ra, ua, wb, nb, rb, ub, nullptr, 0, nullptr, 0);
+    *ua = walk_scalar_nj<false>(wa, na, ra, nullptr, 0);
+    *ub = walk_scalar_nj<false>(wb, nb, rb, nullptr, 0);
+}
+
+size_t chain_walk_bits(const u32 *w, size_t nw, u32 *r, u64 *bits, u64 bit0) {
+    if (isa_level() == 2) return walk_avx512_nj_t<10, true>(w, nw, r, bits, bit0);
+    return walk_scalar_nj<true>(w, nw, r, bits, bit0);
+}
+
+void chain_walk2_bits(const u32 *wa, size_t na, u32 *ra, size_t *ua, u64 *bits_a, u64 bit0_a,
+                      const u32 *wb, size_t nb, u32 *rb, size_t *ub, u64 *bits_b, u64 bit0_b) {
+    if (isa_level() == 2) return walk2_avx512_nj<true>(wa, na, ra, ua, wb, nb, rb, ub, bits_a, bit0_a, bits_b, bit0_b);
+    *ua = walk_scalar_nj<true>(wa, na, ra, bits_a, bit0_a);
+    *ub = walk_scalar_nj<true>(wb, nb, rb, bits_b, bit0_b);
+}
+
+size_t chain_walk_bits_isa(int isa, const u32 *w, size_t nw, u32 *r, u64 *bits, u64 bit0) {
+    if (isa == 2 && isa_level() == 2) return walk_avx512_nj_t<10, true>(w, nw, r, bits, bit0);
+    return walk_scalar_nj<true>(w, nw, r, bits, bit0);
+}
+
+void chain_walk2_bits_isa(int isa, const u32 *wa, size_t na, u32 *ra, size_t *ua, u64 *bits_a, u64 bit0_a,
+                          const u32 *wb, size_t nb, u32 *rb, size_t *ub, u64 *bits_b, u64 bit0_b) {
+    if (isa == 2 && isa_level() == 2)
+        return walk2_avx512_nj<true>(wa, na, ra, ua, wb, nb, rb, ub, bits_a, bit0_a, bits_b, bit0_b);
+    *ua = walk_scalar_nj<true>(wa, na, ra, bits_a, bit0_a);
+    *ub = walk_scalar_nj<true>(wb, nb, rb, bits_b, bit0_b);
 }
 
 size_t chain_walk(const u32 *w, size_t nw, u32 *r, u32 *J) {
diff --git a/burn-ppo_amd/csrc/shuffle_host.h b/burn-ppo_amd/csrc/shuffle_host.h
--- a/burn-ppo_amd/csrc/shuffle_host.h
+++ b/burn-ppo_amd/csrc/shuffle_host.h
@@ -13,6 +13,14 @@
 void chain_walk2_nj(const uint32_t *wa, size_t na, uint32_t *ra, size_t *ua,
                     const uint32_t *wb, size_t nb, uint32_t *rb, size_t *ub);
 
+size_t chain_walk_bits(const uint32_t *w, size_t nw, uint32_t *r, uint64_t *bits, uint64_t bit0);
+void chain_walk2_bits(const uint32_t *wa, size_t na, uint32_t *ra, size_t *ua, uint64_t *bits_a, uint64_t bit0_a,
+                      const uint32_t *wb, size_t nb, uint32_t *rb, size_t *ub, uint64_t *bits_b, uint64_t bit0_b);
+size_t chain_walk_bits_isa(int isa, const uint32_t *w, size_t nw, uint32_t *r, uint64_t *bits, uint64_t bit0);
+void chain_walk2_bits_isa(int isa, const uint32_t *wa, size_t na, uint32_t *ra, size_t *ua, uint64_t *bits_a,
+                          uint64_t bit0_a, const uint32_t *wb, size_t nb, uint32_t *rb, size_t *ub, uint64_t *bits_b,
+                          uint64_t bit0_b);
+
 int chain_walk_isa();
 
 }
diff --git a/include/bppo.h b/include/bppo.h
--- a/include/bppo.h
+++ b/include/bppo.h
@@ -169,6 +169,15 @@
                                       uint64_t gap, int32_t jobs, int32_t windows, uint32_t *J, uint64_t *ends,
                                       int32_t *met);
 
+bppo_status bppo_debug_walk_bits(const uint32_t *words, size_t nw, uint32_t *r_inout, uint64_t *bits, uint64_t bit0,
+                                 int32_t isa, size_t *used);
+bppo_status bppo_debug_walk2_bits(const uint32_t *words_a, size_t na, uint32_t *ra_inout, uint64_t *bits_a,
+                                  uint64_t bit0_a, size_t *used_a, const uint32_t *words_b, size_t nb,
+                                  uint32_t *rb_inout, uint64_t *bits_b, uint64_t bit0_b, size_t *used_b, int32_t isa);
+bppo_status bppo_debug_expand_bits(int32_t device, const uint32_t *words, uint64_t word_base, size_t nw,
+                                   const uint64_t *pos0, const uint64_t *pos1, const uint32_t *r0, const uint64_t *bits,
+                                   int32_t ns, uint32_t n, uint32_t *J);
+
 bppo_status bppo_debug_sample(int32_t A, int32_t B, const float *logits, const uint8_t *masks, uint64_t seed,
                               uint64_t stream, uint64_t word_pos, int32_t *actions, float *log_probs);
 
```

After: 610.3 million. 6.8% lower.
